# erturklab/delivr_cfos

Hardware: AMD Instinct MI355X
Metric: voxels/sec sliding-window 3D U-Net inference, 2048x2048x1024 vol @1/2/4/8 GPU (higher is better)
Workload: dtype f16; 1 GPU; c3: 1024x2048x2048 (Z,Y,X) uint16 synthetic brain, windows 128x128x128, overlap 0.5, 1 pass (no TTA), trained-like BasicUNet(32,32,64,128,256,32) weights, fp16 operands / fp32 accumulate, ellipsoid brain (background skipped); tta=False, windows=14415, windows_skipped=5400, lanes=3, mask_voxels=16658615, mask_checksum=17887483292235547, parallelism=1 GPU

## Files before the change

### delivr_cfos_amd/_lib.py

```python
from __future__ import annotations

import ctypes as C
import os

_HERE = os.path.dirname(os.path.abspath(__file__))
LIB_PATH = os.path.join(_HERE, "lib", "libdelivr_hip.so")
if os.environ.get("DLV_LIB"):
    _name = os.environ["DLV_LIB"]
    if os.path.basename(_name) != _name or not (_name.startswith("libdelivr_hip") and _name.endswith(".so")):
        raise ImportError(f"DLV_LIB={_name!r}: expected the bare name of a libdelivr_hip*.so under {os.path.dirname(LIB_PATH)}")
    if "_abl" in _name and os.environ.get("DLV_ALLOW_WRONG_RESULTS") != "1":
        raise ImportError(f"DLV_LIB={_name!r} is a timing-only ablation build (wrong results); set DLV_ALLOW_WRONG_RESULTS=1 "
                          "to time it (profiles/tools/zreg_abl.sh does)")
    LIB_PATH = os.path.join(os.path.dirname(LIB_PATH), _name)



def build_fingerprint(lib_path: str | None = None) -> dict:
    import glob
    import hashlib

    lib_path = lib_path or LIB_PATH
    out = {"lib": os.path.basename(lib_path), "lib_sha256": None, "src_sha256": None}
    if os.path.isfile(lib_path):
        h = hashlib.sha256()
        with open(lib_path, "rb") as f:
            for blk in iter(lambda: f.read(1 << 20), b""):
                h.update(blk)
        out["lib_sha256"] = h.hexdigest()
    csrc = os.path.join(_HERE, "csrc")
    files = sorted(glob.glob(os.path.join(csrc, "*.hip")) + glob.glob(os.path.join(csrc, "*.h")) + [os.path.join(csrc, "Makefile")]
                   + glob.glob(os.path.join(os.path.dirname(_HERE), "include", "*.h")))
    h = hashlib.sha256()
    for fn in files:
        if os.path.isfile(fn):
            h.update(os.path.basename(fn).encode() + b"\0")
            with open(fn, "rb") as f:
                h.update(f.read())
    out["src_sha256"] = h.hexdigest()
    return out


DLV_OK, DLV_EINVAL, DLV_EHIP, DLV_ENOMEM, DLV_ESTATE, DLV_EUNSUP, DLV_ERANGE = 0, -1, -2, -3, -4, -5, -6
ABI_VERSION = 2
PREC_F32, PREC_BF16, PREC_F16, PREC_BF16_ALL = 0, 1, 2, 3
N_CONV, N_DECONV = 18, 4
PROF_MAX = 64


class DelivrHipError(RuntimeError):
    def __init__(self, code: int, msg: str):
        super().__init__(f"libdelivr_hip error {code}: {msg}")
        self.code = code


class UnetWeights(C.Structure):
    _fields_ = [
        ("features", C.c_int * 6),
        ("conv_w", C.c_void_p * N_CONV),
        ("conv_b", C.c_void_p * N_CONV),
        ("norm_g", C.c_void_p * N_CONV),
        ("norm_b", C.c_void_p * N_CONV),
        ("deconv_w", C.c_void_p * N_DECONV),
        ("deconv_b", C.c_void_p * N_DECONV),
        ("final_w", C.c_void_p),
        ("final_b", C.c_void_p),
    ]


class DebugLayerArgs(C.Structure):
    _fields_ = [
        ("kind", C.c_int), ("op", C.c_int), ("index", C.c_int),
        ("in1", C.c_void_p), ("c1", C.c_int), ("ss1", C.c_void_p),
        ("in2", C.c_void_p), ("c2", C.c_int),
        ("vol", C.c_void_p), ("flip_dim", C.c_int),
        ("out", C.c_void_p),
        ("B", C.c_int), ("D", C.c_int), ("H", C.c_int), ("W", C.c_int),
        ("ran_zreg", C.c_int), ("ran_upconv", C.c_int), ("ran_stem", C.c_int), ("drops_bias", C.c_int),
        ("drops_fold_const", C.c_int), ("raw_scale", C.c_float),
    ]


PLAN_MAX_LABELS = 96
PLAN_CONV_KERNELS = ("ZREG", "DEEP", "ZMARCH", "GENERIC", "STEM_MFMA", "STEM_VALU")
PLAN_DECONV_KERNELS = ("DEEP", "REGW", "WST", "ROWS", "PARITY")


class PlanConv(C.Structure):
    _fields_ = [("kernel", C.c_int), ("level", C.c_int), ("cin", C.c_int), ("cout", C.c_int), ("folded", C.c_int),
                ("tile_rows", C.c_int), ("act_on_load", C.c_int), ("tx", C.c_int), ("ncb", C.c_int), ("wlds", C.c_int),
                ("max_parts", C.c_longlong)]


class PlanDeconv(C.Structure):
    _fields_ = [("kernel", C.c_int), ("norm_first", C.c_int), ("padded", C.c_int)]


class PlanPool(C.Structure):
    _fields_ = [("rows", C.c_int), ("writeback", C.c_int), ("norm_after", C.c_int), ("nt", C.c_int)]


class LayerPlan(C.Structure):
    _fields_ = [("conv", PlanConv * N_CONV), ("deconv", PlanDeconv * N_DECONV), ("pool", PlanPool * 4), ("n_labels", C.c_int),
                ("labels", (C.c_char * 48) * PLAN_MAX_LABELS), ("flops", C.c_double * PLAN_MAX_LABELS),
                ("bytes", C.c_double * PLAN_MAX_LABELS)]


class SwParams(C.Structure):
    _fields_ = [
        ("Zp", C.c_int), ("Yp", C.c_int), ("Xp", C.c_int),
        ("roi", C.c_int * 3),
        ("overlap", C.c_float),
        ("flip_dim", C.c_int),
        ("skip_threshold", C.c_int),
        ("precision", C.c_int),
        ("sw_batch", C.c_int),
        ("win_begin", C.c_int64),
        ("win_end", C.c_int64),
        ("z0", C.c_int), ("nz", C.c_int),
        ("repeat", C.c_int),
        ("blend_mode", C.c_int),
        ("sigma_scale", C.c_float),
        ("wsum_dev", C.c_void_p),
    ]


class SwStats(C.Structure):
    _fields_ = [("n_windows", C.c_int64), ("n_skipped", C.c_int64), ("n_forward_launches", C.c_int64)]


MAX_RANKS = 16


class ShardPlanC(C.Structure):
    _fields_ = [("world", C.c_int), ("n_windows", C.c_int64),
                ("win_begin", C.c_int64 * MAX_RANKS), ("win_end", C.c_int64 * MAX_RANKS),
                ("z_comp_lo", C.c_int * MAX_RANKS), ("z_comp_hi", C.c_int * MAX_RANKS),
                ("z_own_lo", C.c_int * MAX_RANKS), ("z_own_hi", C.c_int * MAX_RANKS)]


class ProfEntry(C.Structure):
    _fields_ = [("name", C.c_char * 48), ("launches", C.c_int64), ("total_ms", C.c_double),
                ("flops", C.c_double), ("bytes", C.c_double)]


_P = C.c_void_p
SIGNATURES = {
    "dlv_abi_version": (C.c_int, []),
    "dlv_ctx_create": (C.c_int, [C.c_int, _P, C.POINTER(_P)]),
    "dlv_ctx_destroy": (C.c_int, [_P]),
    "dlv_last_error": (C.c_char_p, [_P]),
    "dlv_sync": (C.c_int, [_P]),
    "dlv_stream": (_P, [_P]),
    "dlv_malloc": (C.c_int, [_P, C.c_size_t, C.POINTER(_P)]),
    "dlv_free": (C.c_int, [_P, _P]),
    "dlv_memset_dev": (C.c_int, [_P, _P, C.c_int, C.c_size_t]),
    "dlv_copy_h2d": (C.c_int, [_P, _P, _P, C.c_size_t]),
    "dlv_copy_d2h": (C.c_int, [_P, _P, _P, C.c_size_t]),
    "dlv_unet_load": (C.c_int, [_P, C.POINTER(UnetWeights)]),
    "dlv_unet_blob_size": (C.c_int, [_P, C.POINTER(C.c_size_t)]),
    "dlv_unet_blob_dev": (C.c_int, [_P, C.POINTER(_P)]),
    "dlv_unet_alloc_blob": (C.c_int, [_P, C.POINTER(C.c_int)]),
    "dlv_unet_forward_dev": (C.c_int, [_P, _P, _P, C.c_int, C.c_int, C.c_int, C.c_int, C.c_int]),
    "dlv_sw_num_windows": (C.c_int, [C.POINTER(SwParams), C.POINTER(C.c_int64)]),
    "dlv_sw_window_starts": (C.c_int, [C.POINTER(SwParams), C.POINTER(C.c_int64), C.c_int64]),
    "dlv_sw_window_max_dev": (C.c_int, [_P, C.POINTER(SwParams), _P, C.POINTER(C.c_int32), C.c_int64]),
    "dlv_sw_infer_dev": (C.c_int, [_P, C.POINTER(SwParams), _P, _P, _P, C.POINTER(SwStats)]),
    "dlv_shard_plan_make": (C.c_int, [C.POINTER(SwParams), C.c_int, C.POINTER(C.c_float), C.POINTER(ShardPlanC)]),
    "dlv_shard_slab": (C.c_int, [C.POINTER(ShardPlanC), C.c_int, C.c_int, C.c_int, C.c_int, C.POINTER(C.c_int), C.POINTER(C.c_int)]),
    "dlv_comm_init_all": (C.c_int, [C.c_int, C.POINTER(C.c_int), C.POINTER(_P)]),
    "dlv_comm_destroy": (C.c_int, [_P]),
    "dlv_comm_size": (C.c_int, [_P]),
    "dlv_comm_uses_rccl": (C.c_int, [_P]),
    "dlv_comm_selftest": (C.c_int, [_P, C.c_size_t]),
    "dlv_comm_ctx": (_P, [_P, C.c_int]),
    "dlv_comm_last_error": (C.c_char_p, [_P]),
    "dlv_bcast_weights": (C.c_int, [_P, C.c_int]),
    "dlv_sw_infer_sharded": (C.c_int, [_P, C.POINTER(SwParams), C.POINTER(ShardPlanC), C.POINTER(C.c_int), C.POINTER(C.c_int),
                                       C.POINTER(_P), C.POINTER(_P), C.POINTER(_P), C.POINTER(SwStats)]),
    "dlv_sw_infer_sharded_wsum": (C.c_int, [_P, C.POINTER(SwParams), C.POINTER(ShardPlanC), C.POINTER(C.c_int), C.POINTER(C.c_int),
                                            C.POINTER(_P), C.POINTER(_P), C.POINTER(_P), C.POINTER(_P), C.POINTER(SwStats)]),
    "dlv_finalize_slab_dev": (C.c_int, [_P, _P, _P, _P, C.c_int, C.c_int, C.c_int, C.c_int, C.c_int, C.c_int, C.c_float, C.c_int,
                                        C.c_int, _P, _P]),
    "dlv_finalize_dev": (C.c_int, [_P, _P, _P, _P, C.c_int, C.c_int, C.c_int, C.c_int, C.c_int, C.c_float, C.c_int,
                                   C.c_int, _P, _P]),
    "dlv_ccl26_dev": (C.c_int, [_P, _P, C.c_int, C.c_int, C.c_int, _P, C.POINTER(C.c_uint64)]),
    "dlv_cc_stats_dev": (C.c_int, [_P, _P, C.c_int, C.c_int, C.c_int, C.c_uint64, _P, _P, _P]),
    "dlv_block_mean_u16_dev": (C.c_int, [_P, _P, C.c_int, C.c_int, C.c_int, C.c_int, C.c_int, C.c_int, _P]),
    "dlv_zoom_spline2_u8_dev": (C.c_int, [_P, _P, C.c_int, C.c_int, C.c_int, _P, C.c_int, C.c_int, C.c_int]),
    "dlv_mask_pad_u16_dev": (C.c_int, [_P, _P, _P, C.c_int, C.c_int, C.c_int, C.c_int, _P, C.c_int, C.c_int, C.c_int]),
    "dlv_trilinear_u16_dev": (C.c_int, [_P, _P, C.c_int, C.c_int, C.c_int, _P, C.c_int, C.c_int, C.c_int]),
    "dlv_affine_warp_u16_dev": (C.c_int, [_P, _P, C.c_int, C.c_int, C.c_int, C.POINTER(C.c_double), _P, C.c_int, C.c_int, C.c_int]),
    "dlv_seam_pairs_dev": (C.c_int, [_P, _P, _P, C.c_int, C.c_int, _P, C.c_uint64, C.POINTER(C.c_uint64)]),
    "dlv_relabel_u32_dev": (C.c_int, [_P, _P, C.c_uint64, _P, C.c_uint64]),
    "dlv_cc_stats_raw_dev": (C.c_int, [_P, _P, C.c_int, C.c_int, C.c_int, C.c_uint64, _P, _P, _P, _P]),
    "dlv_cc_counts_dev": (C.c_int, [_P, _P, C.c_uint64, C.c_uint64, _P]),
    "dlv_cc_size_filter_dev": (C.c_int, [_P, _P, C.c_uint64, C.c_uint64, _P, C.c_int64, C.c_int64, C.POINTER(C.c_uint64)]),
    "dlv_cc_intensity_dev": (C.c_int, [_P, _P, _P, C.c_int, C.c_int, C.c_int, C.c_int64, C.c_int64, C.c_uint64, _P, _P, _P, _P]),
    "dlv_cc_shell_dev": (C.c_int, [_P, _P, _P, C.c_int, C.c_int, C.c_int, C.c_int64, C.c_int64, C.c_int, _P, _P]),
    "dlv_paint_owner_dev": (C.c_int, [_P, _P, C.c_int, C.c_int, C.c_int, _P, _P, C.c_uint64, _P]),
    "dlv_paint_apply_dev": (C.c_int, [_P, _P, _P, C.c_uint64, _P, C.c_int, _P]),
    "dlv_edt_u16_dev": (C.c_int, [_P, _P, C.c_int, C.c_int, C.c_int, C.POINTER(C.c_double), _P]),
    "dlv_heatmap_counts_dev": (C.c_int, [_P, _P, C.c_uint64, C.c_int, C.c_int, C.c_int, _P]),
    "dlv_gauss_blur_f32_dev": (C.c_int, [_P, _P, C.c_int, C.c_int, C.c_int, _P, C.c_int, _P]),
    "dlv_tiff_last_error": (C.c_char_p, []),
    "dlv_tiff_plane_size": (C.c_int, [C.c_char_p, C.POINTER(C.c_int), C.POINTER(C.c_int), C.POINTER(C.c_int)]),
    "dlv_tiff_read_plane_u16": (C.c_int, [C.c_char_p, _P, C.c_int, C.c_int]),
    "dlv_tiff_write_plane": (C.c_int, [C.c_char_p, _P, C.c_int, C.c_int, C.c_int, C.c_int]),
    "dlv_tiff_stack_to_device": (C.c_int, [_P, C.POINTER(C.c_char_p), C.c_int, C.c_int, C.c_int, _P, C.c_longlong,
                                            C.c_longlong, C.c_int]),
    "dlv_diag_set": (C.c_int, [_P, C.c_char_p, C.c_int]),
    "dlv_diag_plan": (C.c_int, [C.POINTER(C.c_int), C.POINTER(C.c_char_p), C.POINTER(C.c_int), C.c_int, C.c_int, C.c_int, C.c_int,
                                C.c_int, C.c_int, C.POINTER(LayerPlan)]),
    "dlv_cells_csv": (C.c_int, [_P, _P, C.c_uint64, _P, C.c_size_t, C.POINTER(C.c_size_t)]),
    "dlv_reserve_dev": (C.c_int, [_P, _P, C.c_int, C.c_int, C.c_int]),
    "dlv_debug_stamps": (C.c_int, [_P, _P]),
    "dlv_debug_set_zm_variant": (C.c_int, [_P, C.c_int]),
    "dlv_debug_set_format": (C.c_int, [_P, C.c_int]),
    "dlv_debug_layer_bf16": (C.c_int, [_P, C.c_int, C.c_int, _P, C.c_int, _P, C.c_int, _P, C.c_int, C.c_int, C.c_int,
                                       C.c_int]),
    "dlv_debug_layer16": (C.c_int, [_P, C.POINTER(DebugLayerArgs)]),
    "dlv_unet_set_conv_shift": (C.c_int, [_P, C.c_int, C.c_int]),
    "dlv_unet_get_conv_shift": (C.c_int, [_P, C.c_int, C.POINTER(C.c_int)]),
    "dlv_unet_note_conv_shifts": (C.c_int, [_P, C.POINTER(C.c_int)]),
    "dlv_range_report": (C.c_int, [_P, C.POINTER(C.c_int), C.POINTER(C.c_float)]),
    "dlv_range_next_shifts": (C.c_int, [C.c_int, C.POINTER(C.c_float), C.POINTER(C.c_int), C.POINTER(C.c_int)]),
    "dlv_range_recover": (C.c_int, [_P, C.POINTER(C.c_int)]),
    "dlv_comm_range_recover": (C.c_int, [_P, C.POINTER(C.c_int)]),
    "dlv_set_lanes": (C.c_int, [_P, C.c_int]),
    "dlv_prof_enable": (C.c_int, [_P, C.c_int]),
    "dlv_prof_reset": (C.c_int, [_P]),
    "dlv_prof_report": (C.c_int, [_P, C.POINTER(ProfEntry), C.c_int, C.POINTER(C.c_int)]),
}

_lib = None


def load() -> C.CDLL:
    global _lib
    if _lib is not None:
        return _lib
    if not os.path.isfile(LIB_PATH):
        raise ImportError(
            f"{LIB_PATH} not found - build it with `python -c 'import __graft_entry__ as g; g.build()'` "
            "or `make -C delivr_cfos_amd/csrc` (hipcc, --offload-arch=gfx950). There is no CPU fallback.")
    try:
        import torch
    except ImportError:
        pass
    lib = C.CDLL(LIB_PATH)
    for name, (res, args) in SIGNATURES.items():
        fn = getattr(lib, name)
        fn.restype = res
        fn.argtypes = args
    if lib.dlv_abi_version() != ABI_VERSION:
        raise ImportError(f"libdelivr_hip.so reports ABI version {lib.dlv_abi_version()}, this package binds version {ABI_VERSION} "
                          "(include/delivr_hip.h: DLV_ABI_VERSION): rebuild with make -C delivr_cfos_amd/csrc")
    _lib = lib
    return lib
```

### delivr_cfos_amd/csrc/api.hip

```cpp
#include <dlfcn.h>

#include <algorithm>
#include <charconv>
#include <cmath>
#include <cstdlib>
#include <mutex>

#include "common.h"

int dlv_fail(dlv_ctx* ctx, int code, const char* fmt, ...) {
    char buf[1024];
    va_list ap;
    va_start(ap, fmt);
    vsnprintf(buf, sizeof(buf), fmt, ap);
    va_end(ap);
    if (ctx) ctx->err = buf;
    return code;
}

int dlv_ws_get(dlv_ctx* ctx, int slot, size_t bytes, void** out) {
    if (slot < 0 || slot >= WS_N_SLOTS) return dlv_fail(ctx, DLV_EINVAL, "bad scratch slot %d", slot);
    if (ctx->ws_bytes[slot] < bytes) {
        if (ctx->ws[slot]) {
            DLV_TRY(dlv_sync_all(ctx));
// ... 559 lines not shown
    if (std::isnan(v)) return p + snprintf(p, (size_t)(end - p), "nan");
    if (std::isinf(v)) return p + snprintf(p, (size_t)(end - p), v < 0 ? "-inf" : "inf");
    const double a = std::fabs(v);
    if (a != 0.0 && (a < 1e-4 || a >= 1e16)) {
        const auto r = std::to_chars(p, end, v, std::chars_format::scientific);
        return r.ptr;
    }
    const auto r = std::to_chars(p, end, v, std::chars_format::fixed);
    char* q = r.ptr;
    bool dot = false;
    for (char* c = p; c < q; ++c) dot |= (*c == '.');
    if (!dot && q + 2 <= end) {
        *q++ = '.';
        *q++ = '0';
    }
    return q;
}

int dlv_cells_csv(const uint32_t* voxel_counts, const double* centroids, uint64_t n, char* out, size_t cap, size_t* len_out) {
    if (!voxel_counts || !centroids || !out || !len_out) return DLV_EINVAL;
    static const char header[] = ",Blob,Coords,Size\n";
    if (cap < sizeof(header)) return DLV_EINVAL;
    char* p = out;
    char* const end = out + cap;
    memcpy(p, header, sizeof(header) - 1);
    p += sizeof(header) - 1;
    for (uint64_t i = 1; i < n; ++i) {
        if ((size_t)(end - p) < 128) return DLV_EINVAL;
        p += snprintf(p, (size_t)(end - p), "0,%llu,\"[", (unsigned long long)i);
        for (int k = 0; k < 3; ++k) {
            p = py_float_repr(p, end, centroids[3 * i + k]);
            if (k < 2) {
                *p++ = ',';
                *p++ = ' ';
            }
        }
        p += snprintf(p, (size_t)(end - p), "]\",%u\n", voxel_counts[i]);
    }
    *len_out = (size_t)(p - out);
    return DLV_OK;
}

int dlv_diag_set(dlv_ctx* ctx, const char* name, int value) {
    if (!ctx || !name) return DLV_EINVAL;
    const std::string n(name);
    if (n == "zm_variant") return dlv_debug_set_zm_variant(ctx, value);
    if (dlv_plan_switch_set(ctx->sw, name, value)) return DLV_OK;
    if (n == "upconv_simple") ctx->upconv_simple = value ? 1 : 0;
    else if (n == "zreg_dbg") ctx->zreg_dbg = value;
    else if (n == "erode_xy_split") ctx->erode_xy_split = value != 0;
    else if (n == "erode_z_two_sweeps") ctx->erode_z_two_sweeps = value != 0;
    else if (n == "ccl_simple") ctx->ccl_simple = value != 0;
    else if (n == "resample_simple") ctx->resample_simple = value != 0;
    else if (n == "resample_run16") ctx->resample_run16 = value != 0;
    else if (n == "tiff_chunk") ctx->tiff_chunk = value > 0 ? value : 0;
    else return dlv_fail(ctx, DLV_EINVAL, "dlv_diag_set: unknown switch '%s'", name);
    return DLV_OK;
}

int dlv_debug_set_zm_variant(dlv_ctx* ctx, int variant) {
    if (!ctx) return DLV_EINVAL;
#ifndef DLV_DIAG
    if (variant != 0 && variant != 50 && variant != 51)
        return dlv_fail(ctx, DLV_EUNSUP, "z-march variant %d is a diagnostic build: load libdelivr_hip_diag.so (make -C delivr_cfos_amd/csrc diag)", variant);
#endif
    ctx->sw.zm_variant = variant;
    return DLV_OK;
}

int dlv_diag_plan(const int features[6], const char* const* names, const int* values, int n, int fmt16, int B, int d, int h, int w,
                  dlv_layer_plan* out) {
    if (!features || !out || n < 0 || (n > 0 && (!names || !values)) || fmt16 < 0 || fmt16 > 2) return DLV_EINVAL;
    DlvPlanSwitches sw;
    bool upconv_simple = false;
    for (int i = 0; i < n; ++i) {
        if (!names[i]) return DLV_EINVAL;
        if (strcmp(names[i], "upconv_simple") == 0) upconv_simple = values[i] != 0;
        else if (strcmp(names[i], "zreg_dbg") == 0) continue;
        else if (!dlv_plan_switch_set(sw, names[i], values[i])) return DLV_EINVAL;
    }
    return dlv_plan_forward(sw, upconv_simple, features, fmt16, B, d, h, w, out) ? DLV_OK : DLV_EUNSUP;
}

int dlv_debug_stamps(dlv_ctx* ctx, void* buf_dev) {
    if (!ctx) return DLV_EINVAL;
    ctx->stamp_buf = buf_dev;
    return DLV_OK;
}

int dlv_debug_set_format(dlv_ctx* ctx, int precision) {
    if (!ctx || (precision != DLV_PREC_BF16_ALL && precision != DLV_PREC_F16)) return DLV_EINVAL;
    ctx->debug_f16 = precision == DLV_PREC_F16;
    return DLV_OK;
}

int dlv_set_lanes(dlv_ctx* ctx, int lanes) {
    if (!ctx || lanes < 1 || lanes > DLV_MAX_LANES) return DLV_EINVAL;
    ctx->lanes_wanted = lanes;
    return DLV_OK;
}

int dlv_prof_enable(dlv_ctx* ctx, int on) {
    if (!ctx) return DLV_EINVAL;
    if (!on) DLV_TRY(prof_drain(ctx));
    ctx->prof_on = on != 0;
    return DLV_OK;
}
int dlv_prof_reset(dlv_ctx* ctx) {
    if (!ctx) return DLV_EINVAL;
    DLV_TRY(prof_drain(ctx));
    ctx->prof_slots.clear();
    return DLV_OK;
}
int dlv_prof_report(dlv_ctx* ctx, dlv_prof_entry* entries, int capacity, int* n_out) {
    if (!ctx || !n_out) return DLV_EINVAL;
    DLV_TRY(prof_drain(ctx));
    int n = (int)ctx->prof_slots.size();
    *n_out = n;
    for (int i = 0; i < n && i < capacity && entries; ++i) {
        memcpy(entries[i].name, ctx->prof_slots[i].name, sizeof(entries[i].name));
        entries[i].launches = ctx->prof_slots[i].launches;
        entries[i].total_ms = ctx->prof_slots[i].total_ms;
        entries[i].flops = ctx->prof_slots[i].flops;
        entries[i].bytes = ctx->prof_slots[i].bytes;
    }
    return DLV_OK;
}

}
```

### delivr_cfos_amd/csrc/common.h

```cpp
#pragma once
#include <hip/hip_runtime.h>

#include <atomic>
#include <cstdarg>
#include <cstdint>
#include <cstdio>
#include <cstring>
#include <string>
#include <vector>

#include "../../include/delivr_hip.h"
#include "../../include/delivr_hip_diag.h"
#include "layer_plan.h"

#define DLV_WAVE 64
#define DLV_MAX_LANES 6

struct DlvProfSlot {
    char name[48];
    int64_t launches = 0;
    double total_ms = 0.0, flops = 0.0, bytes = 0.0;
};
struct DlvProfPending {
    int slot;
    hipEvent_t a, b;
};

struct DlvConvLayer {
    int cin = 0, cout = 0;
    float* w_f32 = nullptr;
    float* bias = nullptr;
    float* bias16 = nullptr;
    int shift = 0;
    float* gamma = nullptr;
    float* beta = nullptr;
    uint16_t* w_bf16 = nullptr;
    uint16_t* w_f16 = nullptr;
    uint16_t* w16_bf16 = nullptr;
    uint16_t* w16_f16 = nullptr;
    uint16_t* wskip_bf16 = nullptr;
    uint16_t* wskip_f16 = nullptr;
    uint16_t* wup_bf16 = nullptr;
    uint16_t* wup_f16 = nullptr;
    float* up_corr = nullptr;
    int up_slices = 0;
};
struct DlvDeconvLayer {
    int cin = 0, cout = 0;
    float* w_f32 = nullptr;
    float* bias = nullptr;
    uint16_t* w_bf16 = nullptr;
    uint16_t* w_f16 = nullptr;
    uint16_t* w16_bf16 = nullptr;
    uint16_t* w16_f16 = nullptr;
};

enum DlvWsSlot {
    WS_F32_ACT = 0,
    WS_BF16_ACT,
    WS_STATS,
    WS_TILE_IN,
    WS_TILE_OUT,
    WS_TILE_META,
    WS_BLEND_W,
    WS_ERODE,
    WS_CCL,
    WS_MISC,
    WS_LANE_ACT0,
    WS_LANE_STATS0 = WS_LANE_ACT0 + DLV_MAX_LANES - 1,
    WS_N_SLOTS = WS_LANE_STATS0 + DLV_MAX_LANES - 1
};

struct dlv_ctx {
    int device = 0;
    hipStream_t stream = nullptr;
    hipStream_t main_stream = nullptr;
    hipStream_t aux_stream = nullptr;
    hipStream_t aux[DLV_MAX_LANES - 1] = {nullptr};
    hipEvent_t ev_lane[DLV_MAX_LANES + 1] = {nullptr};
    int lane = 0;
    int lanes_wanted = 3;
    bool own_stream = false;
    std::string err;
    bool weights_loaded = false;
    int features[6] = {0, 0, 0, 0, 0, 0};
    const float* blend_w = nullptr;
    float blend_min = 0.f;
    float* blend_wsum = nullptr;
    int upconv_dbg = 0;
    int upconv_simple = 0;
    void* stamp_buf = nullptr;
    int* range_flag = nullptr;
    int range_last = -1;
    float range_peak[DLV_N_CONV] = {0};
    bool range_seq = false;
    int range_base[DLV_N_CONV] = {0};
    int range_blind_layer = -1;
    void* zero_page = nullptr;
    void* blob = nullptr;
    size_t blob_bytes = 0;
    DlvConvLayer conv[DLV_N_CONV];
    DlvDeconvLayer deconv[DLV_N_DECONV];
    float* final_w = nullptr;
    float* final_b = nullptr;
    void* ws[WS_N_SLOTS] = {nullptr};
    size_t ws_bytes[WS_N_SLOTS] = {0};
    bool debug_f16 = false;
    DlvPlanSwitches sw;
    int zreg_dbg = 0;
    int ran_zreg = 0, ran_upconv = 0;
    bool erode_xy_split = false, erode_z_two_sweeps = false, ccl_simple = false;
    bool resample_simple = false, resample_run16 = false;
    int tiff_chunk = 0;
    bool prof_on = false;
    std::vector<DlvProfSlot> prof_slots;
    std::vector<DlvProfPending> prof_pending;
    std::vector<hipEvent_t> prof_free;
};

int dlv_fail(dlv_ctx* ctx, int code, const char* fmt, ...);

#define DLV_HIP(ctx, expr)                                                                          \
    do {                                                                                            \
        hipError_t _e = (expr);                                                                     \
        if (_e != hipSuccess)                                                                       \
            return dlv_fail((ctx), _e == hipErrorOutOfMemory ? DLV_ENOMEM : DLV_EHIP, "%s failed: %s (%s:%d)", \
                            #expr, hipGetErrorString(_e), __FILE__, __LINE__);                      \
    } while (0)

#define DLV_LAUNCH_CHECK(ctx, what)                                                                 \
    do {                                                                                            \
        hipError_t _e = hipGetLastError();                                                          \
        if (_e != hipSuccess)                                                                       \
            return dlv_fail((ctx), DLV_EHIP, "launch of %s failed: %s", (what), hipGetErrorString(_e)); \
    } while (0)

#define DLV_TRY(expr)                \
    do {                             \
        int _rc = (expr);            \
        if (_rc != DLV_OK) return _rc; \
    } while (0)

int dlv_ws_get(dlv_ctx* ctx, int slot, size_t bytes, void** out);
int dlv_sync_all(dlv_ctx* ctx);

struct DlvProf {
    dlv_ctx* ctx;
    int idx = -1;
    bool ranged = false;
    DlvProf(dlv_ctx* c, const char* name, double flops, double bytes);
    ~DlvProf();
    void end();
};

typedef std::atomic<unsigned long long> dlv_attr_bits;
static inline bool dlv_attr_is_set(const dlv_attr_bits& bits, int device) { return (bits.load(std::memory_order_acquire) >> (device & 63)) & 1ull; }
static inline void dlv_attr_mark(dlv_attr_bits& bits, int device) { bits.fetch_or(1ull << (device & 63), std::memory_order_release); }

#ifdef __HIPCC__
#ifndef DLV_NT
#define DLV_NT 1
#endif
typedef unsigned dlv_u32x4_t __attribute__((ext_vector_type(4)));
typedef unsigned dlv_u32x2_t __attribute__((ext_vector_type(2)));
template <bool NT>
__device__ __forceinline__ uint4 dlv_ld16(const uint4* p) {
    if constexpr (NT && DLV_NT) {
        const dlv_u32x4_t t = __builtin_nontemporal_load(reinterpret_cast<const dlv_u32x4_t*>(p));
        return make_uint4(t.x, t.y, t.z, t.w);
    } else {
        return *p;
    }
}
template <bool NT>
__device__ __forceinline__ void dlv_st16(uint4* p, uint4 v) {
    if constexpr (NT && DLV_NT) __builtin_nontemporal_store(dlv_u32x4_t{v.x, v.y, v.z, v.w}, reinterpret_cast<dlv_u32x4_t*>(p));
    else *p = v;
}
template <bool NT>
__device__ __forceinline__ void dlv_st8(uint2* p, uint2 v) {
    if constexpr (NT && DLV_NT) __builtin_nontemporal_store(dlv_u32x2_t{v.x, v.y}, reinterpret_cast<dlv_u32x2_t*>(p));
    else *p = v;
}
__device__ __forceinline__ int dlv_xcd_tile(unsigned bx, unsigned gx) {
    return (gx % 8 == 0) ? (int)((bx % 8) * (gx / 8) + bx / 8) : (int)bx;
}
#endif

int dlv_unet_forward_f32(dlv_ctx* ctx, const float* x, float* logits, int B, int d, int h, int w);
static inline int dlv_fmt16(int precision) { return precision == DLV_PREC_F16 ? 1 : (precision == DLV_PREC_BF16 ? 2 : 0); }
int dlv_unet_forward_bf16(dlv_ctx* ctx, const float* x, float* logits, int B, int d, int h, int w, int fmt16);
int dlv_unet_tiles_bf16(dlv_ctx* ctx, const uint16_t* vol, int Yp, int Xp, const int* starts_dev, int B, int d,
                        int h, int w, int flip_dim, float scale, float* acc, int fmt16);
int dlv_pack_weights_bf16(dlv_ctx* ctx);
int dlv_unet_reserve_16(dlv_ctx* ctx, int B, int d, int h, int w, int lanes);
int dlv_conv3_zmarch_launch(dlv_ctx* ctx, bool f16, int cin, int cout, const void* in1, int c1, const void* in2, int c2,
                            const void* wpk, const float* bias, void* out, float* partials, int B, int D, int H, int W,
                            int* nparts);
int dlv_conv3_deep_launch(dlv_ctx* ctx, bool f16, int cin, int cout, const void* in1, int c1, const void* in2, int c2, const void* wpk16,
                          void* out, float* partials, int B, int D, int H, int W, int* nparts);
int dlv_pack_deconv_w16(dlv_ctx* ctx, bool f16, const float* w_f32, uint16_t* out, int cin, int cout);
int dlv_deconv2_deep_launch(dlv_ctx* ctx, bool f16, int cin, int cout, const void* in, const void* wpk16, const float* bias, void* out, int B,
                            int D, int H, int W);
int dlv_conv3_zreg_launch(dlv_ctx* ctx, bool f16, int cin, int cout, const void* in1, int c1, const void* ss1, const void* in2,
                          int c2, const void* ss2, const void* wpk16, void* out, float* partials, int B, int D, int H, int W,
                          int* nparts, const void* addend = nullptr);
int dlv_pack_conv_w16(dlv_ctx* ctx, bool f16, const float* w_f32, uint16_t* out, int cout, int cin, int ctot = 0, int c0 = 0, float wscale = 1.f);
int dlv_pack_upconv(dlv_ctx* ctx, bool f16, const float* wc, int ctot, int cs, const float* wd, const float* bd, uint16_t* wpk, float* corr,
                    int ci0 = 0, int with_corr = 1, float wscale = 1.f);
bool dlv_upconv2_persistent(const dlv_ctx* ctx, int Dc, int Hc, int Wc);
int dlv_upconv2_launch(dlv_ctx* ctx, bool f16, const void* in, const void* wpk, const float* corr, void* out, int B, int Dc, int Hc, int Wc,
                       int cstride = 4, int c0 = 0);
int dlv_range_reset(dlv_ctx* ctx);
int dlv_range_check(dlv_ctx* ctx, int fmt16);
int dlv_unet_apply_conv_shifts(dlv_ctx* ctx, const int* shifts);
int dlv_range_step(dlv_ctx* ctx, int layer, const float* peaks, int* n_changed, const int* force_next );
int dlv_range_plan(dlv_ctx* ctx, int layer, const float* peaks, int* nxt, bool* blind);
size_t dlv_bf16_pack_bytes(const int features[6]);
#if defined(__HIPCC__)
__device__ __forceinline__ float dlv_half_sum32(float v) {
#define DLV_DPP_ADD(ctrl, rmask)                                                                                      \
    v += __builtin_bit_cast(float, __builtin_amdgcn_update_dpp(0, __builtin_bit_cast(int, v), ctrl, rmask, 0xf, true))
    DLV_DPP_ADD(0xB1, 0xf);
    DLV_DPP_ADD(0x4E, 0xf);
    DLV_DPP_ADD(0x141, 0xf);
    DLV_DPP_ADD(0x140, 0xf);
    DLV_DPP_ADD(0x142, 0xa);
#undef DLV_DPP_ADD
    return v;
}
#endif
```

### delivr_cfos_amd/csrc/layer_plan.h

```cpp
#pragma once
#include <cstdio>
#include <cstring>

#include "../../include/delivr_hip_diag.h"

struct DlvPlanSwitches {
    bool no_zmarch = false;
    int zm_variant = 0;
    int zreg_mask = 3;
    int deep_mask = 2;
    int deep_small = 1;
    int generic_ncb = 0;
    int fuse_layers = 1 << 17;
    int fuse_levels = 0;
    int fold_up = 1;
    bool pool_rows_off = false;
};

inline bool dlv_plan_switch_set(DlvPlanSwitches& s, const char* name, int value) {
    const auto is = [&](const char* n) { return strcmp(name, n) == 0; };
    if (is("no_zmarch")) s.no_zmarch = value != 0;
    else if (is("no_upconv")) s.fold_up = value ? 0 : 1;
    else if (is("zm_variant")) s.zm_variant = value;
    else if (is("fuse_levels")) s.fuse_levels = value;
    else if (is("fuse_layers")) s.fuse_layers = value;
    else if (is("zreg_mask")) s.zreg_mask = value;
    else if (is("deep_mask")) s.deep_mask = value;
    else if (is("generic_ncb")) s.generic_ncb = value;
    else if (is("deep_small")) s.deep_small = value;
    else if (is("pool_rows_off")) s.pool_rows_off = value != 0;
    else return false;
    return true;
}

static inline int dlv_cdiv(long long a, long long b) { return (int)((a + b - 1) / b); }

constexpr int kDlvConvLevel[DLV_N_CONV] = {0, 0, 1, 1, 2, 2, 3, 3, 4, 4, 3, 3, 2, 2, 1, 1, 0, 0};

inline void dlv_unet_channels(const int f[6], int cin[DLV_N_CONV], int cout[DLV_N_CONV], int dcin[DLV_N_DECONV], int dcout[DLV_N_DECONV]) {
    const int ci[DLV_N_CONV] = {1, f[0], f[0], f[1], f[1], f[2], f[2], f[3], f[3], f[4],
                                f[3] + f[4] / 2, f[3], f[2] + f[3] / 2, f[2], f[1] + f[2] / 2, f[1], f[0] + f[1], f[5]};
    const int co[DLV_N_CONV] = {f[0], f[0], f[1], f[1], f[2], f[2], f[3], f[3], f[4], f[4],
                                f[3], f[3], f[2], f[2], f[1], f[1], f[5], f[5]};
    const int di[DLV_N_DECONV] = {f[4], f[3], f[2], f[1]};
    const int dco[DLV_N_DECONV] = {f[4] / 2, f[3] / 2, f[2] / 2, f[1]};
    for (int i = 0; i < DLV_N_CONV; ++i) {
        cin[i] = ci[i];
        cout[i] = co[i];
    }
    for (int j = 0; j < DLV_N_DECONV; ++j) {
        dcin[j] = di[j];
        dcout[j] = dco[j];
    }
}
inline bool dlv_window_supported(int d, int h, int w) {
    return d >= 16 && h >= 16 && w >= 16 && (long long)(d >> 4) * (h >> 4) * (w >> 4) >= 2;
}

inline bool dlv_conv_has_fold_pack(int li, int cin, int cout, int dcin3, int dcout3) {
    return li == 16 && cin == 64 && cout == 32 && dcin3 == 32 && dcout3 == 32;
}
inline bool dlv_deconv_has_w16_pack(int cin) { return cin >= 128; }

inline bool dlv_conv3_zreg_supports(int cin, int cout, int c1, int c2, int W) {
    return cout % 32 == 0 && cout > 0 && W >= 32 &&
           ((cin == 32 && c1 == 32 && c2 == 0) || (cin == 64 && ((c1 == 32 && c2 == 32) || (c1 == 64 && c2 == 0))));
}
inline int dlv_conv3_zreg_tile_rows(int cin, int cout, int D, int H, int W) {
    return (cin == 32 && H % 16 == 0 && (long long)(H / 16) * dlv_cdiv(W, 32) * (cout / 32) * dlv_cdiv(D, 64) >= 16) ? 16 : 8;
}
inline bool dlv_conv3_deep_supports(int cin, int cout, int c1, int c2, int D, int H, int W) {
    return cin % 32 == 0 && c1 % 32 == 0 && c2 % 32 == 0 && c1 + c2 == cin && cout % 32 == 0 && cout >= 32 && W >= 2 && H >= 2 && D >= 2 &&
           (long long)D * H * W <= 32768;
}
inline bool dlv_deconv2_deep_supports(int cin, int cout, int D, int H, int W) {
    return (cin == 128 || cin == 256) && cout % 64 == 0 && cout > 0 && (long long)D * H * W <= 32768 && W >= 1;
}
inline bool dlv_upconv2_persistent_shape(int Dc, int Hc, int Wc) {
    return Dc > 0 && Dc % 4 == 0 && Hc % 8 == 0 && Wc % 16 == 0 && ((long long)5 * Hc + 10) * Wc * 16 < (1 << 24) &&
           (long long)Dc * Hc * Wc * 8 * 16 * 2 < (1LL << 31);
}

struct DlvConvPlan {
    int kernel = DLV_PLAN_GENERIC;
    int cin = 0, cout = 0;
    bool folded = false;
    int tile_rows = 0;
    int tx = 0, ncb = 0;
    bool wlds = false;
    bool act_on_load = false;
    bool norm_first = false;
    long long max_parts = 0;
};

inline bool dlv_plan_zreg_runs(const DlvPlanSwitches& sw, int cin, int cout, int c1, int c2, int D, int H, int W) {
    return (sw.zm_variant == 0 || sw.zm_variant == 50) && !sw.no_zmarch && (long long)D * H * W > 32768 &&
           dlv_conv3_zreg_supports(cin, cout, c1, c2, W) && ((cin == 32 ? 1 : 2) & sw.zreg_mask);
}
inline bool dlv_plan_fuses_first_input(const DlvPlanSwitches& sw, int li, int cin, int cout, int c1, int c2, int D, int H, int W) {
    return (((sw.fuse_levels >> kDlvConvLevel[li]) & 1) || ((sw.fuse_layers >> li) & 1)) && c1 == 32 &&
           dlv_plan_zreg_runs(sw, cin, cout, c1, c2, D, H, W);
}

inline DlvConvPlan plan_conv(const DlvPlanSwitches& sw, int li, int cin, int cout, int c1, int c2, bool raw1, int B, int D, int H, int W) {
    DlvConvPlan p;
    p.cin = cin;
    p.cout = cout;
    p.act_on_load = raw1 && dlv_plan_fuses_first_input(sw, li, cin, cout, c1, c2, D, H, W);
    p.norm_first = raw1 && !p.act_on_load;
    const long long zm_parts = (long long)dlv_cdiv(H, 8) * dlv_cdiv(W, 32) * dlv_cdiv(D, 16);
    if (dlv_plan_zreg_runs(sw, cin, cout, c1, c2, D, H, W)) {
        p.kernel = DLV_PLAN_ZREG;
        p.tile_rows = dlv_conv3_zreg_tile_rows(cin, cout, D, H, W);
        p.max_parts = zm_parts;
        return p;
    }
    const bool zmarch_ok = (cout == 32 || cout == 64) && (cin == 32 || cin == 64) && W >= 32;
    const bool deep_full = cout >= 64 && W >= 8 && H >= 8 && D >= 4;
    if (!sw.no_zmarch && ((zmarch_ok ? 1 : 2) & sw.deep_mask) && (deep_full || sw.deep_small) && dlv_conv3_deep_supports(cin, cout, c1, c2, D, H, W)) {
        p.kernel = DLV_PLAN_DEEP;
        p.max_parts = (long long)dlv_cdiv(D, 4) * dlv_cdiv(H, 8) * dlv_cdiv(W, 8);
        return p;
    }
    if (zmarch_ok && !sw.no_zmarch) {
        p.kernel = DLV_PLAN_ZMARCH;
        p.max_parts = zm_parts;
        return p;
    }
    p.kernel = DLV_PLAN_GENERIC;
    p.tx = W >= 16 ? 16 : 8;
    const long long ntiles = (long long)dlv_cdiv(D, 4) * dlv_cdiv(H, 64 / p.tx) * dlv_cdiv(W, p.tx);
    p.wlds = (long long)D * H * W <= 1024;
    p.ncb = p.wlds ? (cout >= 64 ? 2 : 1) : (cout >= 128 ? 4 : (cout >= 64 ? 2 : 1));
    while (p.ncb > 1 && (long long)B * ntiles * (cout / (32 * p.ncb)) < 512) p.ncb >>= 1;
    if (const int want = sw.generic_ncb)
        if ((want == 1 || want == 2 || (want == 4 && !p.wlds)) && cout % (32 * want) == 0) p.ncb = want;
    p.max_parts = ntiles;
    return p;
}

inline bool plan_folds_up(const DlvPlanSwitches& sw, bool has_pack, int cskip, int cout, int D, int H, int W) {
    return sw.fold_up && has_pack && cskip == 32 && (sw.zm_variant == 0 || sw.zm_variant == 50) && !sw.no_zmarch && (long long)D * H * W > 32768 &&
           dlv_conv3_zreg_supports(32, cout, 32, 0, W) && D % 2 == 0 && H % 2 == 0 && W % 2 == 0;
}
inline DlvConvPlan plan_conv_folded(const DlvPlanSwitches& sw, int li, int cout, bool raw1, int D, int H, int W) {
    DlvConvPlan p;
    p.kernel = DLV_PLAN_ZREG;
    p.folded = true;
    p.cin = 32;
    p.cout = cout;
    p.tile_rows = dlv_conv3_zreg_tile_rows(32, cout, D, H, W);
    p.act_on_load = raw1 && dlv_plan_fuses_first_input(sw, li, 64, cout, 32, 32, D, H, W);
    p.norm_first = raw1 && !p.act_on_load;
    p.max_parts = (long long)dlv_cdiv(H, 8) * dlv_cdiv(W, 32) * dlv_cdiv(D, 16);
    return p;
}

struct DlvDeconvPlan {
    int kernel = DLV_PLAN_DC_PARITY;
    bool norm_first = false;
};
constexpr int DLV_DC_IPW = 8;

inline DlvDeconvPlan plan_deconv(const DlvPlanSwitches& sw, int cin, int cout, bool raw, int D, int H, int W) {
    DlvDeconvPlan p;
    const bool rows = !sw.no_zmarch;
    p.norm_first = raw && (!rows || cin >= 128);
    const long long segs = dlv_cdiv(W, 16), vox = (long long)D * H * W;
    if (rows && sw.deep_mask != 0 && dlv_deconv_has_w16_pack(cin) && dlv_deconv2_deep_supports(cin, cout, D, H, W)) p.kernel = DLV_PLAN_DC_DEEP;
    else if (cin != 32 && cin != 64 && cin != 128 && cin != 256) p.kernel = DLV_PLAN_NONE;
    else if (!rows) p.kernel = DLV_PLAN_DC_PARITY;
    else if (cin >= 128) p.kernel = DLV_PLAN_DC_WST;
    else if (cout == 32 && (long long)D * H * segs >= 4 * DLV_DC_IPW * 64 && vox * 8 * 4 * 16 < (1ll << 32)) p.kernel = DLV_PLAN_DC_REGW;
    else p.kernel = DLV_PLAN_DC_ROWS;
    return p;
}

struct DlvNormPlan {
    bool rows = false;
    bool nt = false;
};
inline DlvNormPlan plan_norm_pass(const DlvPlanSwitches& sw, bool pooled, int B, int C, int D, int H, int W) {
    DlvNormPlan p;
    p.nt = (double)D * H * W * B * C * 2 > 768.0 * (1 << 20);
    p.rows = pooled && W % 64 == 0 && !sw.pool_rows_off;
    return p;
}
inline bool plan_stem_mfma(const DlvPlanSwitches& sw, bool from_volume) { return from_volume && !sw.no_zmarch; }

struct DlvLabel {
    char name[48];
    double flops, bytes;
};
inline const char* dlv_fmt_name(bool f16) { return f16 ? "f16" : "bf16"; }

inline DlvLabel dlv_label_conv(const DlvConvPlan& p, bool f16, int B, int D, int H, int W) {
    static const char* const family[4] = {"zreg", "deep", "zmarch", "mfma"};
    DlvLabel l;
    const double vox = (double)((long long)D * H * W);
    snprintf(l.name, sizeof(l.name), "conv3_%s_%s_c%dx%d_d%d%s%s", family[p.kernel], dlv_fmt_name(f16), p.cin, p.cout, D, p.folded ? "_add" : "",
             p.act_on_load ? "_act" : "");
    l.flops = 2.0 * 27 * p.cin * p.cout * vox * B;
    l.bytes = 2.0 * vox * B * (p.cin + (p.folded ? 2 : 1) * p.cout);
    if (p.kernel == DLV_PLAN_DEEP) l.bytes += 2.0 * 27 * p.cin * p.cout;
    return l;
}
inline DlvLabel dlv_label_upconv(bool persistent, bool f16, int B, int D, int H, int W) {
    DlvLabel l;
    const double vox = (double)((long long)D * H * W), voxc = (double)((long long)(D / 2) * (H / 2) * (W / 2));
    snprintf(l.name, sizeof(l.name), "upconv2%s_%s_c32x32_d%d", persistent ? "m" : "", dlv_fmt_name(f16), D / 2);
    l.flops = 2.0 * 8 * 32 * 32 * vox * B;
    l.bytes = 2.0 * 32 * (voxc + vox) * B;
    return l;
}
inline DlvLabel dlv_label_deconv(const DlvDeconvPlan& p, bool f16, int cin, int cout, int B, int D, int H, int W) {
    DlvLabel l;
    const double vox = (double)((long long)D * H * W);
    snprintf(l.name, sizeof(l.name), "deconv2_%s_%s_c%dx%d_d%d", p.kernel == DLV_PLAN_DC_DEEP ? "deep" : "mfma", dlv_fmt_name(f16), cin, cout, D);
    l.flops = 2.0 * 8 * cin * cout * vox * B;
    l.bytes = 2.0 * vox * B * (cin + 8.0 * cout);
    return l;
}
inline DlvLabel dlv_label_norm(bool pooled, bool writeback, bool f16, bool seam, int B, int C, int D, int H, int W) {
    DlvLabel l;
    const double vox = (double)((long long)D * H * W);
    snprintf(l.name, sizeof(l.name), "%s", pooled ? (writeback ? (f16 ? (seam ? "norm_mish_pool_f16_to_bf16" : "norm_mish_pool_f16") : "norm_mish_pool_bf16")
                                                               : (f16 ? "pool_act_f16" : "pool_act_bf16"))
                                                  : (f16 ? "norm_mish_f16" : (seam ? "norm_mish_bf16_to_f16" : "norm_mish_bf16")));
    l.flops = 0.0;
    l.bytes = vox * B * C * 2 * (writeback ? 2 : 1) + (pooled ? vox / 8 * B * C * 2 : 0.0);
    return l;
}
inline DlvLabel dlv_label_pad(bool f16, int cout, int B, long long vox_up, long long vox_skip) {
    DlvLabel l;
    snprintf(l.name, sizeof(l.name), "%s", f16 ? "replicate_pad_f16" : "replicate_pad_bf16");
    l.flops = 0.0;
    l.bytes = 16.0 * B * (cout / 8) * ((double)vox_up + (double)vox_skip);
    return l;
}
inline DlvLabel dlv_label_stem(bool mfma, int B, int D, int H, int W) {
    DlvLabel l;
    const double vox = (double)((long long)D * H * W);
    snprintf(l.name, sizeof(l.name), "%s", mfma ? "stem_mfma_u16" : "stem_conv_f32");
    l.flops = 2.0 * 27 * 32 * vox * B;
    l.bytes = vox * B * (2 + 64);
    return l;
}
inline DlvLabel dlv_label_final(bool blend, int B, int D, int H, int W) {
    DlvLabel l;
    const double vox = (double)((long long)D * H * W);
    snprintf(l.name, sizeof(l.name), "%s", blend ? "final_conv_blend" : "final_conv_logits");
    l.flops = 2.0 * 32 * vox * B;
    l.bytes = vox * B * (64 + (blend ? 8 : 4));
    return l;
}

inline bool dlv_plan_forward(const DlvPlanSwitches& sw, bool upconv_simple, const int f[6], int fmt16, int B, int d, int h, int w, dlv_layer_plan* out) {
    memset(out, 0, sizeof(*out));
    if (f[0] != 32 || f[5] != 32 || B < 1 || !dlv_window_supported(d, h, w)) return false;
    for (int i = 0; i < 6; ++i)
        if (f[i] <= 0 || f[i] % 32 || f[i] > 256) return false;
    int cin[DLV_N_CONV], cout[DLV_N_CONV], dcin[DLV_N_DECONV], dcout[DLV_N_DECONV];
    dlv_unet_channels(f, cin, cout, dcin, dcout);
    struct Dm {
        int D, H, W;
        long long vox() const { return (long long)D * H * W; }
    } dm[5];
    for (int l = 0; l < 5; ++l) dm[l] = Dm{d >> l, h >> l, w >> l};
    const bool mixed = fmt16 == 2;
    const auto f16_at = [&](int level) { return level == 0 ? fmt16 != 0 : fmt16 == 1; };
    const auto emit = [&](const DlvLabel& l) {
        if (out->n_labels >= DLV_PLAN_MAX_LABELS) return;
        memcpy(out->labels[out->n_labels], l.name, sizeof(l.name));
        out->flops[out->n_labels] = l.flops;
        out->bytes[out->n_labels] = l.bytes;
        ++out->n_labels;
    };
    struct T {
        int C;
        bool raw;
    };
    const auto materialise = [&](T& t, int level, int fl, bool seam) {
        if (!t.raw) return;
        emit(dlv_label_norm(false, true, f16_at(fl), seam, B, t.C, dm[level].D, dm[level].H, dm[level].W));
        t.raw = false;
    };
    const auto record = [&](int li, const DlvConvPlan& p, int level) {
        dlv_plan_conv& c = out->conv[li];
        c.kernel = p.kernel;
        c.level = level;
        c.cin = p.cin;
        c.cout = p.cout;
        c.folded = p.folded;
        c.tile_rows = p.tile_rows;
        c.act_on_load = p.act_on_load;
        c.tx = p.tx;
        c.ncb = p.ncb;
        c.wlds = p.wlds;
        c.max_parts = p.max_parts;
        emit(dlv_label_conv(p, f16_at(level), B, dm[level].D, dm[level].H, dm[level].W));
    };
    const auto conv = [&](int li, T& a1, int c2, int level) {
        const DlvConvPlan p = plan_conv(sw, li, cin[li], cout[li], a1.C, c2, a1.raw, B, dm[level].D, dm[level].H, dm[level].W);
        if (p.norm_first) materialise(a1, level, level, false);
        record(li, p, level);
        return T{cout[li], true};
    };
    const auto deconv_to = [&](int j, T& a, int l, int fl) {
        const Dm din = dm[l + 1], sk = dm[l];
        const DlvDeconvPlan p = plan_deconv(sw, dcin[j], dcout[j], a.raw, din.D, din.H, din.W);
        if (p.norm_first) materialise(a, l + 1, fl, false);
        out->deconv[j].kernel = p.kernel;
        out->deconv[j].norm_first = p.norm_first;
        emit(dlv_label_deconv(p, f16_at(fl), dcin[j], dcout[j], B, din.D, din.H, din.W));
        out->deconv[j].padded = 2 * din.D != sk.D || 2 * din.H != sk.H || 2 * din.W != sk.W;
        if (out->deconv[j].padded) emit(dlv_label_pad(f16_at(fl), dcout[j], B, 8 * din.vox(), sk.vox()));
    };

    const bool stem_mfma = plan_stem_mfma(sw, true);
    out->conv[0].kernel = stem_mfma ? DLV_PLAN_STEM_MFMA : DLV_PLAN_STEM_VALU;
    out->conv[0].cin = 1;
    out->conv[0].cout = 32;
    emit(dlv_label_stem(stem_mfma, B, d, h, w));
    T x0{32, !stem_mfma};
    T skip[5];
    skip[0] = conv(1, x0, 0, 0);
    for (int l = 1; l <= 4; ++l) {
        T& up = skip[l - 1];
        const int li_cat = 18 - 2 * l, c_up = dcout[4 - l];
        const Dm dp = dm[l - 1];
        const bool keep_raw = plan_conv(sw, li_cat, cin[li_cat], cout[li_cat], up.C, c_up, true, B, dp.D, dp.H, dp.W).act_on_load;
        const bool odd = ((dp.D | dp.H | dp.W) & 1) != 0;
        const DlvNormPlan np = plan_norm_pass(sw, true, B, up.C, dp.D, dp.H, dp.W);
        dlv_plan_pool& pl = out->pool[l - 1];
        pl.rows = np.rows;
        pl.nt = np.nt;
        pl.writeback = !keep_raw && !odd;
        pl.norm_after = odd && !keep_raw;
        emit(dlv_label_norm(true, pl.writeback, f16_at(l - 1), l == 1 && mixed, B, up.C, dp.D, dp.H, dp.W));
        if (pl.norm_after) emit(dlv_label_norm(false, true, f16_at(l - 1), false, B, up.C, dp.D, dp.H, dp.W));
        up.raw = keep_raw;
        T a{l == 1 ? 32 : f[l - 1], false};
        T b = conv(2 * l, a, 0, l);
        skip[l] = conv(2 * l + 1, b, 0, l);
    }
    T cur = skip[4];
    for (int j = 0; j < 4; ++j) {
        const int l = 3 - j, li = 10 + 2 * j;
        T b;
        if (l == 0 && mixed) materialise(cur, 1, 1, true);
        if (l == 0 && plan_folds_up(sw, dlv_conv_has_fold_pack(li, cin[li], cout[li], dcin[3], dcout[3]), skip[0].C, cout[li], d, h, w)) {
            const DlvConvPlan p = plan_conv_folded(sw, li, cout[li], skip[0].raw, d, h, w);
            materialise(cur, 1, 0, false);
            if (p.norm_first) materialise(skip[0], 0, 0, false);
            emit(dlv_label_upconv(!upconv_simple && dlv_upconv2_persistent_shape(dm[1].D, dm[1].H, dm[1].W), f16_at(0), B, d, h, w));
            record(li, p, 0);
            out->deconv[j].kernel = DLV_PLAN_NONE;
            b = T{cout[li], true};
        } else {
            deconv_to(j, cur, l, l);
            b = conv(li, skip[l], dcout[j], l);
        }
        cur = conv(li + 1, b, 0, l);
    }
    emit(dlv_label_final(true, B, d, h, w));
    return true;
}
```

### delivr_cfos_amd/csrc/sw_infer.hip

```cpp
#include <algorithm>

#include "common.h"
#include <cmath>

namespace {

struct Tiler {
    int n[3], roi[3], iv[3];
    std::vector<int> st[3];
    int ncol[3];
    std::vector<int> col[3];
    int64_t count() const { return (int64_t)st[0].size() * st[1].size() * st[2].size(); }
};

int build_tiler(dlv_ctx* ctx, const dlv_sw_params* p, Tiler& t) {
    t.n[0] = p->Zp;
    t.n[1] = p->Yp;
    t.n[2] = p->Xp;
    if (!(p->overlap >= 0.f && p->overlap < 1.f)) return dlv_fail(ctx, DLV_EINVAL, "overlap must be >= 0 and < 1");
    for (int k = 0; k < 3; ++k) {
        if (t.n[k] <= 0) return dlv_fail(ctx, DLV_EINVAL, "empty volume");
        int r = p->roi[k] > 0 ? p->roi[k] : t.n[k];
        if (r > t.n[k])
            return dlv_fail(ctx, DLV_EUNSUP, "roi[%d]=%d exceeds the padded volume (%d): pad the volume first "
                            "(downsample_and_mask.py:390-396 does)", k, r, t.n[k]);
        t.roi[k] = r;
        int iv = r == t.n[k] ? r : (int)((double)r * (1.0 - (double)p->overlap));
        if (iv <= 0) iv = 1;
        t.iv[k] = iv;
        const int num = (t.n[k] + iv - 1) / iv;
        int scan = num - 1;
        for (int dd = 0; dd < num; ++dd)
            if ((long long)dd * iv + r >= t.n[k]) {
                scan = dd;
                break;
            }
        t.st[k].clear();
        for (int i = 0; i <= scan; ++i) {
            int s = i * iv;
            s -= std::max(s + r - t.n[k], 0);
            t.st[k].push_back(s);
        }
        const int c = (r + iv - 1) / iv;
        const int kk = (int)t.st[k].size();
        t.col[k].assign(kk, 0);
        int ncol = std::min(c, kk);
        for (int i = 0; i < kk; ++i) t.col[k][i] = i % c;
        if (kk > 1 && t.st[k][kk - 1] != (kk - 1) * iv && kk > c) {
            t.col[k][kk - 1] = c;
            ncol = c + 1;
        }
        t.ncol[k] = ncol;
    }
    return DLV_OK;
}


__global__ void __launch_bounds__(256) window_max_kernel(const uint16_t* __restrict__ vol, int Yp, int Xp,
                                                         const int* __restrict__ starts, int d, int h, int w,
                                                         int* __restrict__ wmax) {
    const int win = blockIdx.y;
    const int z0 = starts[3 * win], y0 = starts[3 * win + 1], x0 = starts[3 * win + 2];
    const uint16_t* base = vol + ((long long)z0 * Yp + y0) * Xp + x0;
    unsigned m = 0;
    const bool vec = (w % 8 == 0) && (Xp % 8 == 0) && (x0 % 8 == 0);
    if (vec) {
        const int w8 = w / 8;
        const long long n8 = (long long)d * h * w8;
        for (long long i = (long long)blockIdx.x * blockDim.x + threadIdx.x; i < n8; i += (long long)gridDim.x * blockDim.x) {
            const int xx = (int)(i % w8), yy = (int)((i / w8) % h), zz = (int)(i / ((long long)w8 * h));
            const uint4 v = *reinterpret_cast<const uint4*>(base + ((long long)zz * Yp + yy) * Xp + xx * 8);
            const unsigned a = max(max(v.x & 0xffffu, v.x >> 16), max(v.y & 0xffffu, v.y >> 16));
            const unsigned b = max(max(v.z & 0xffffu, v.z >> 16), max(v.w & 0xffffu, v.w >> 16));
            m = max(m, max(a, b));
        }
    } else {
        const long long n = (long long)d * h * w;
        for (long long i = (long long)blockIdx.x * blockDim.x + threadIdx.x; i < n; i += (long long)gridDim.x * blockDim.x) {
            const int xx = (int)(i % w), yy = (int)((i / w) % h), zz = (int)(i / ((long long)w * h));
            m = max(m, (unsigned)base[((long long)zz * Yp + yy) * Xp + xx]);
        }
    }
    for (int o = 32; o > 0; o >>= 1) m = max(m, __shfl_down(m, o, 64));
    if ((threadIdx.x & 63) == 0 && m > 0) atomicMax(wmax + win, (int)m);
}

__global__ void __launch_bounds__(256) cell_max_kernel(const uint16_t* __restrict__ vol, int Yp, int Xp, int z_lo,
                                                       const int* __restrict__ zcell, const int* __restrict__ ybound, int ncy,
                                                       const int* __restrict__ xcell, int x_lo8, int x_hi8, int ncx,
                                                       int* __restrict__ cellmax) {
    extern __shared__ int lmax[];
    const int cy = blockIdx.x % ncy, z = z_lo + blockIdx.x / ncy;
    const int cz = zcell[z];
    if (cz < 0) return;
    for (int i = threadIdx.x; i < ncx; i += blockDim.x) lmax[i] = 0;
    __syncthreads();
    const int y0 = ybound[cy], y1 = ybound[cy + 1];
    for (int c = x_lo8 + threadIdx.x; c < x_hi8; c += blockDim.x) {
        unsigned m = 0;
        const uint16_t* col = vol + ((long long)z * Yp + y0) * Xp + 8 * c;
        for (int y = y0; y < y1; ++y, col += Xp) {
            const uint4 v = *reinterpret_cast<const uint4*>(col);
            const unsigned a = max(max(v.x & 0xffffu, v.x >> 16), max(v.y & 0xffffu, v.y >> 16));
            const unsigned b = max(max(v.z & 0xffffu, v.z >> 16), max(v.w & 0xffffu, v.w >> 16));
            m = max(m, max(a, b));
        }
        if (m) atomicMax(&lmax[xcell[c]], (int)m);
    }
    __syncthreads();
    for (int i = threadIdx.x; i < ncx; i += blockDim.x)
        if (lmax[i]) atomicMax(&cellmax[((long long)cz * ncy + cy) * ncx + i], lmax[i]);
// ... 150 lines not shown
        pr.end();
    }
    DLV_LAUNCH_CHECK(ctx, "window_max_kernel");
    DLV_HIP(ctx, hipMemcpyAsync(wmax, meta + n * 3, (size_t)n * sizeof(int), hipMemcpyDeviceToHost, ctx->stream));
    DLV_HIP(ctx, hipStreamSynchronize(ctx->stream));
    return DLV_OK;
}

extern "C" {

int dlv_sw_num_windows(const dlv_sw_params* p, int64_t* n_windows) {
    if (!p || !n_windows) return DLV_EINVAL;
    Tiler t;
    DLV_TRY(build_tiler(nullptr, p, t));
    *n_windows = t.count();
    return DLV_OK;
}

int dlv_sw_window_starts(const dlv_sw_params* p, int64_t* starts, int64_t capacity) {
    if (!p || !starts) return DLV_EINVAL;
    Tiler t;
    DLV_TRY(build_tiler(nullptr, p, t));
    if (capacity < t.count()) return DLV_EINVAL;
    int64_t i = 0;
    for (int z : t.st[0])
        for (int y : t.st[1])
            for (int x : t.st[2]) {
                starts[3 * i] = z;
                starts[3 * i + 1] = y;
                starts[3 * i + 2] = x;
                ++i;
            }
    return DLV_OK;
}

int dlv_sw_window_max_dev(dlv_ctx* ctx, const dlv_sw_params* p, const uint16_t* vol_dev, int32_t* wmax, int64_t capacity) {
    if (!ctx || !p || !vol_dev || !wmax) return DLV_EINVAL;
    DLV_HIP(ctx, hipSetDevice(ctx->device));
    Tiler t;
    DLV_TRY(build_tiler(ctx, p, t));
    const int64_t total = t.count();
    const int64_t wb = std::max<int64_t>(p->win_begin, 0);
    const int64_t we = p->win_end > 0 ? std::min<int64_t>(p->win_end, total) : total;
    const int64_t n = std::max<int64_t>(we - wb, 0);
    if (capacity < n) return dlv_fail(ctx, DLV_EINVAL, "wmax capacity %lld < %lld windows", (long long)capacity, (long long)n);
    if (n == 0) return DLV_OK;
    if (n > (int64_t)1 << 30) return dlv_fail(ctx, DLV_EUNSUP, "too many windows");
    const int z0 = p->nz > 0 ? p->z0 : 0, nz = p->nz > 0 ? p->nz : p->Zp;
    const int ny = (int)t.st[1].size(), nx = (int)t.st[2].size();
    std::vector<int> starts((size_t)n * 3);
    for (int64_t g = wb; g < we; ++g) {
        const int iz = (int)(g / ((int64_t)ny * nx)), iy = (int)((g / nx) % ny), ix = (int)(g % nx);
        const int z = t.st[0][iz];
        if (z < z0 || z + t.roi[0] > z0 + nz) return dlv_fail(ctx, DLV_EINVAL, "window %lld outside the slab", (long long)g);
        const int64_t i = g - wb;
        starts[3 * i] = z - z0;
        starts[3 * i + 1] = t.st[1][iy];
        starts[3 * i + 2] = t.st[2][ix];
    }
    return window_maxima(ctx, vol_dev, p->Yp, p->Xp, t.roi, starts, n, wmax);
}

static int default_sw_batch(long long tile_vox) {
    return (int)std::min<long long>(std::max<long long>(((long long)1 << 25) / tile_vox, 1), 64);
}

int dlv_reserve_dev(dlv_ctx* ctx, const dlv_sw_params* p, int Z, int Y, int X) {
    if (!ctx || !p) return DLV_EINVAL;
    if (p->roi[0] <= 0 || p->roi[1] <= 0 || p->roi[2] <= 0) return dlv_fail(ctx, DLV_EINVAL, "dlv_reserve_dev: window dimensions");
    DLV_HIP(ctx, hipSetDevice(ctx->device));
    const long long tile_vox = (long long)p->roi[0] * p->roi[1] * p->roi[2];
    const int B = p->sw_batch > 0 ? p->sw_batch : default_sw_batch(tile_vox);
    if (p->precision != DLV_PREC_F32) {
        const int lanes = ctx->aux[0] != nullptr ? std::max(1, std::min(ctx->lanes_wanted, DLV_MAX_LANES)) : 1;
        DLV_TRY(dlv_unet_reserve_16(ctx, B, p->roi[0], p->roi[1], p->roi[2], lanes));
    }
    if (Z > 0 && Y > 0 && X > 0) {
        void* q;
        DLV_TRY(dlv_ws_get(ctx, WS_ERODE, (size_t)Z * Y * X, &q));
    }
    return DLV_OK;
}

int dlv_sw_infer_dev(dlv_ctx* ctx, const dlv_sw_params* p, const uint16_t* vol_dev, float* acc_dev, uint8_t* cnt_dev,
                     dlv_sw_stats* stats) {
    if (!ctx || !p || !vol_dev || !acc_dev) return DLV_EINVAL;
    if (!ctx->weights_loaded) return dlv_fail(ctx, DLV_ESTATE, "dlv_sw_infer_dev before dlv_unet_load");
    if (p->precision != DLV_PREC_F32 && p->precision != DLV_PREC_BF16 && p->precision != DLV_PREC_F16 && p->precision != DLV_PREC_BF16_ALL)
        return dlv_fail(ctx, DLV_EINVAL, "unknown precision %d", p->precision);
    if (!(p->flip_dim == -1 || (p->flip_dim >= 2 && p->flip_dim <= 4)))
        return dlv_fail(ctx, DLV_EINVAL, "flip_dim must be -1, 2, 3 or 4");
    DLV_HIP(ctx, hipSetDevice(ctx->device));
    Tiler t;
    DLV_TRY(build_tiler(ctx, p, t));
    const int d = t.roi[0], h = t.roi[1], w = t.roi[2];
    if (!dlv_window_supported(d, h, w))
        return dlv_fail(ctx, DLV_EUNSUP, "window %dx%dx%d: every dimension must be at least 16 and level 4 (each dimension / 16, rounded down) must hold more "
                        "than one voxel - InstanceNorm3d has no statistics of a single value and torch raises there; any size from there on: "
                        "levels with an odd size are pooled and padded like MONAI's MaxPool3d / UpCat", d, h, w);
    const int64_t total = t.count();
    const int64_t wb = std::max<int64_t>(p->win_begin, 0);
    const int64_t we = p->win_end > 0 ? std::min<int64_t>(p->win_end, total) : total;
    const int z0 = p->nz > 0 ? p->z0 : 0;
    const int nz = p->nz > 0 ? p->nz : p->Zp;
    const int Yp = p->Yp, Xp = p->Xp;
    const int rep = p->repeat > 0 ? p->repeat : 1;
    ctx->blend_w = nullptr;
    ctx->blend_wsum = nullptr;
    ctx->blend_min = 0.f;
    if (p->blend_mode == DLV_BLEND_GAUSSIAN) {
        if (cnt_dev) return dlv_fail(ctx, DLV_EINVAL, "Gaussian blend: pass wsum_dev (fp32) instead of the uint8 count map");
        const float ss = p->sigma_scale > 0.f ? p->sigma_scale : 0.125f;
        std::vector<float> g((size_t)d + h + w);
        float gmin = 1.f;
        size_t off = 0;
        for (int k = 0; k < 3; ++k) {
            const int len = t.roi[k], center = len / 2;
            const float sigma = (float)len * ss;
            const int tail = (int)(std::max(sigma * 4.0f, 0.5f) + 0.5f);
            const float tt = 0.70710678f / std::fabs(sigma);
            float mx = 0.f, mn = 0.f;
            for (int i = 0; i < len; ++i) {
                const int x = i - center;
                float v = 0.f;
                if (x >= -tail && x <= tail) v = std::max(0.f, 0.5f * (std::erf(tt * ((float)x + 0.5f)) - std::erf(tt * ((float)x - 0.5f))));
                g[off + i] = v;
                mx = std::max(mx, v);
            }
            for (int i = 0; i < len; ++i) {
                g[off + i] /= mx;
                if (g[off + i] > 0.f && (mn == 0.f || g[off + i] < mn)) mn = g[off + i];
            }
            gmin *= mn;
            off += len;
        }
        float* gw;
        DLV_TRY(dlv_ws_get(ctx, WS_BLEND_W, g.size() * sizeof(float), (void**)&gw));
        DLV_HIP(ctx, hipMemcpyAsync(gw, g.data(), g.size() * sizeof(float), hipMemcpyHostToDevice, ctx->stream));
        DLV_HIP(ctx, hipStreamSynchronize(ctx->stream));
        ctx->blend_w = gw;
        ctx->blend_min = gmin;
        ctx->blend_wsum = p->wsum_dev;
    } else if (p->blend_mode != DLV_BLEND_CONSTANT) {
        return dlv_fail(ctx, DLV_EINVAL, "unknown blend_mode %d", p->blend_mode);
    }
    if (cnt_dev) {
        long long mult = 1;
        for (int k = 0; k < 3; ++k) {
            std::vector<int> cov((size_t)t.n[k] + 1, 0);
            for (int st : t.st[k]) {
                cov[st] += 1;
                cov[st + t.roi[k]] -= 1;
            }
            int run = 0, mx = 0;
            for (int i = 0; i < t.n[k]; ++i) {
                run += cov[i];
                mx = std::max(mx, run);
            }
            mult *= mx;
        }
        if (mult * rep > 255)
            return dlv_fail(ctx, DLV_EUNSUP, "uint8 count map would wrap: up to %lld windows cover a voxel, x repeat %d > 255", mult, rep);
    }
    if (stats) {
        stats->n_windows = std::max<int64_t>(we - wb, 0);
        stats->n_skipped = 0;
        stats->n_forward_launches = 0;
    }
    if (we <= wb) return DLV_OK;
    const int64_t nwin = we - wb;
    if (nwin > (int64_t)1 << 30) return dlv_fail(ctx, DLV_EUNSUP, "too many windows in one shard");

    const int ny = (int)t.st[1].size(), nx = (int)t.st[2].size();
    const int ncolors = t.ncol[0] * t.ncol[1] * t.ncol[2];
    std::vector<std::vector<int>> by_color(ncolors);
    std::vector<int> starts((size_t)nwin * 3);
    for (int64_t g = wb; g < we; ++g) {
        const int iz = (int)(g / ((int64_t)ny * nx)), iy = (int)((g / nx) % ny), ix = (int)(g % nx);
        const int i = (int)(g - wb);
        const int sz = t.st[0][iz], sy = t.st[1][iy], sx = t.st[2][ix];
        if (sz < z0 || sz + d > z0 + nz)
            return dlv_fail(ctx, DLV_EINVAL, "window %lld (z %d..%d) lies outside the slab [%d,%d)", (long long)g, sz,
                            sz + d, z0, z0 + nz);
        starts[3 * i] = sz - z0;
        starts[3 * i + 1] = sy;
        starts[3 * i + 2] = sx;
        const int c = (t.col[0][iz] * t.ncol[1] + t.col[1][iy]) * t.ncol[2] + t.col[2][ix];
        by_color[c].push_back(i);
    }

    int* meta;
    DLV_TRY(dlv_ws_get(ctx, WS_TILE_META, (size_t)nwin * 3 * sizeof(int), (void**)&meta));
    int* list_dev = meta;
    const long long tile_vox = (long long)d * h * w;
    std::vector<int> wmax((size_t)nwin);
    DLV_TRY(window_maxima(ctx, vol_dev, Yp, Xp, t.roi, starts, nwin, wmax.data()));

    std::vector<int> list;
    list.reserve((size_t)nwin * 3);
    struct Seg { size_t off; int n_active, n_skipped; };
    std::vector<Seg> segs;
    int64_t n_skipped = 0;
    for (int c = 0; c < ncolors; ++c) {
        Seg s{list.size() / 3, 0, 0};
        for (int pass = 0; pass < 2; ++pass)
            for (int i : by_color[c]) {
                const bool skip = wmax[i] <= p->skip_threshold;
                if ((pass == 0) == skip) continue;
                list.push_back(starts[3 * i]);
                list.push_back(starts[3 * i + 1]);
                list.push_back(starts[3 * i + 2]);
                if (skip) ++s.n_skipped; else ++s.n_active;
            }
        n_skipped += s.n_skipped;
        segs.push_back(s);
    }
    DLV_HIP(ctx, hipMemcpyAsync(list_dev, list.data(), list.size() * sizeof(int), hipMemcpyHostToDevice, ctx->stream));

    int sw_batch = p->sw_batch;
    if (sw_batch <= 0) sw_batch = default_sw_batch(tile_vox);
    int64_t launches = 0;
    const int bchunks = (int)std::min<long long>(std::max<long long>(tile_vox / (256 * 16), 1), 256);
    const int nlanes = (p->precision != DLV_PREC_F32 && ctx->aux[0] != nullptr) ? std::max(1, std::min(ctx->lanes_wanted, DLV_MAX_LANES)) : 1;
    const bool two_lanes = nlanes > 1;
    auto lane_stream = [&](int l) { return l == 0 ? ctx->main_stream : ctx->aux[l - 1]; };
    std::vector<hipStream_t> parts;
    for (int l = 0; l < nlanes; ++l) parts.push_back(lane_stream(l));
    auto join_lanes = [&]() -> int {
        if (!two_lanes) return DLV_OK;
        for (size_t l = 0; l < parts.size(); ++l) DLV_HIP(ctx, hipEventRecord(ctx->ev_lane[l], parts[l]));
        for (size_t l = 0; l < parts.size(); ++l)
            for (size_t m = 0; m < parts.size(); ++m)
                if (m != l) DLV_HIP(ctx, hipStreamWaitEvent(parts[l], ctx->ev_lane[m], 0));
        return DLV_OK;
    };
    if (p->precision != DLV_PREC_F32) DLV_TRY(dlv_range_reset(ctx));
    int rc = join_lanes();
    int lane = 0;
    for (const Seg& s : segs) {
        if (rc != DLV_OK) break;
        for (int b0 = 0; b0 < s.n_active && rc == DLV_OK; b0 += sw_batch) {
            const int B = std::min(sw_batch, s.n_active - b0);
            const int* st_dev = list_dev + (s.off + b0) * 3;
            if (p->precision != DLV_PREC_F32) {
                ctx->lane = two_lanes ? lane : 0;
                ctx->stream = lane_stream(ctx->lane);
                rc = dlv_unet_tiles_bf16(ctx, vol_dev, Yp, Xp, st_dev, B, d, h, w, p->flip_dim, (float)rep, acc_dev, dlv_fmt16(p->precision));
                if (rc == DLV_OK && cnt_dev) {
                    hipLaunchKernelGGL(fill_add_kernel, dim3(bchunks, B), dim3(256), 0, ctx->stream, st_dev, d, h, w, Yp,
                                       Xp, 0.0f, rep, acc_dev, cnt_dev, nullptr, 0.f, nullptr);
                    if (hipGetLastError() != hipSuccess) rc = dlv_fail(ctx, DLV_EHIP, "launch of fill_add_kernel(count) failed");
                }
                lane = (lane + 1) % nlanes;
            } else {
                float *tin, *tout;
                rc = dlv_ws_get(ctx, WS_TILE_IN, (size_t)sw_batch * tile_vox * 4, (void**)&tin);
                if (rc == DLV_OK) rc = dlv_ws_get(ctx, WS_TILE_OUT, (size_t)sw_batch * tile_vox * 4, (void**)&tout);
                if (rc != DLV_OK) break;
                hipLaunchKernelGGL(gather_f32_kernel, dim3(bchunks, B), dim3(256), 0, ctx->stream, vol_dev, Yp, Xp,
                                   st_dev, d, h, w, p->flip_dim, tin);
                rc = dlv_unet_forward_f32(ctx, tin, tout, B, d, h, w);
                if (rc != DLV_OK) break;
                hipLaunchKernelGGL(blend_add_kernel, dim3(bchunks, B), dim3(256), 0, ctx->stream, tout, st_dev, d, h, w,
                                   p->flip_dim, Yp, Xp, (float)rep, rep, acc_dev, cnt_dev, ctx->blend_w, ctx->blend_min, ctx->blend_wsum);
                if (hipGetLastError() != hipSuccess) rc = dlv_fail(ctx, DLV_EHIP, "launch of gather/blend kernel failed");
            }
            ++launches;
        }
        ctx->stream = ctx->main_stream;
        ctx->lane = 0;
        if (rc == DLV_OK && s.n_skipped > 0) {
            const int* st_dev = list_dev + (s.off + s.n_active) * 3;
            DlvProf pr(ctx, "skip_fill_f32", 0.0, 8.0 * tile_vox * s.n_skipped);
            hipLaunchKernelGGL(fill_add_kernel, dim3(bchunks, s.n_skipped), dim3(256), 0, ctx->stream, st_dev, d, h, w,
                               Yp, Xp, -1000.0f * rep, rep, acc_dev, cnt_dev, ctx->blend_w, ctx->blend_min, ctx->blend_wsum);
            pr.end();
            if (hipGetLastError() != hipSuccess) rc = dlv_fail(ctx, DLV_EHIP, "launch of fill_add_kernel failed");
        }
        if (rc == DLV_OK) rc = join_lanes();
    }
    ctx->stream = ctx->main_stream;
    ctx->lane = 0;
    if (rc != DLV_OK) return rc;
    if (stats) {
        stats->n_skipped = n_skipped;
        stats->n_forward_launches = launches;
    }
    if (p->precision != DLV_PREC_F32 && launches > 0) return dlv_range_check(ctx, dlv_fmt16(p->precision));
    return DLV_OK;
}

}
```

### delivr_cfos_amd/csrc/unet16_norm.h

```cpp
#pragma once
namespace {

__global__ void __launch_bounds__(64) stats_finalize_kernel(const float* __restrict__ partials, int nparts, int C,
                                                            double inv_count, float eps, const float* __restrict__ gamma,
                                                            const float* __restrict__ beta, float2* __restrict__ ss,
                                                            int* __restrict__ range_flag, int layer) {
    const int c = blockIdx.x % C, n = blockIdx.x / C;
    double s = 0.0, q = 0.0;
    for (int i = threadIdx.x; i < nparts; i += 64) {
        const float2 v = *reinterpret_cast<const float2*>(partials + (((long long)n * nparts + i) * C + c) * 2);
        s += v.x;
        q += v.y;
    }
    for (int o = 32; o > 0; o >>= 1) {
        s += __shfl_down(s, o, 64);
        q += __shfl_down(q, o, 64);
    }
    if (threadIdx.x == 0) {
        if (!(fabs(s) <= 1.0e300 && fabs(q) <= 1.0e300)) atomicMax(range_flag, 100 - layer);
        const double mean = s * inv_count;
        double var = q * inv_count - mean * mean;
        if (var < 0.0) var = 0.0;
        const float peak = (float)(fabs(mean) + 8.0 * sqrt(var));
        if (peak > 0.f && peak < 3.0e38f && __float_as_int(peak) > __builtin_nontemporal_load(range_flag + 1 + layer))
            atomicMax(range_flag + 1 + layer, __float_as_int(peak));
        const float rstd = (float)(1.0 / sqrt(var + (double)eps));
        const float sc = rstd * gamma[c];
        ss[n * C + c] = make_float2(sc, beta[c] - (float)mean * sc);
    }
}

template <class P, class PO = P>
__device__ __forceinline__ uint4 norm_mish8(uint4 u, const float* sc, const float* sh, float* mx) {
    float v[8] = {P::lo(u.x), P::hi(u.x), P::lo(u.y), P::hi(u.y), P::lo(u.z), P::hi(u.z), P::lo(u.w), P::hi(u.w)};
#pragma unroll
    for (int k = 0; k < 8; k += 2) {
        const f32x2_t m = mish_fast2(fma2(f32x2_t{v[k], v[k + 1]}, f32x2_t{sc[k], sc[k + 1]}, f32x2_t{sh[k], sh[k + 1]}));
        v[k] = m.x;
        v[k + 1] = m.y;
        if (mx) {
            mx[k] = fmaxf(mx[k], v[k]);
            mx[k + 1] = fmaxf(mx[k + 1], v[k + 1]);
        }
    }
    uint4 r;
    r.x = PO::pack2(v[0], v[1]);
    r.y = PO::pack2(v[2], v[3]);
    r.z = PO::pack2(v[4], v[5]);
    r.w = PO::pack2(v[6], v[7]);
    return r;
}

template <class P, bool POOL, bool WB, bool NT = false, class PW = P, class PQ = P>
__global__ void __launch_bounds__(256) norm_mish_kernel(uint4* __restrict__ x, const float2* __restrict__ ss, int C,
                                                        int D, int H, int W, uint4* __restrict__ pooled) {
    const int c8 = blockIdx.y, n = blockIdx.z;
    float sc[8], sh[8];
#pragma unroll
    for (int k = 0; k < 8; ++k) {
        const float2 v = ss[n * C + c8 * 8 + k];
        sc[k] = v.x;
        sh[k] = v.y;
    }
    const long long vox = (long long)D * H * W;
    uint4* p = x + ((long long)n * (C / 8) + c8) * vox;
    if (!POOL) {
        for (long long i = (long long)blockIdx.x * 256 + threadIdx.x; i < vox; i += (long long)gridDim.x * 256)
            dlv_st16<NT>(p + i, norm_mish8<P, PW>(dlv_ld16<NT>(p + i), sc, sh, nullptr));
    } else {
        const int d2 = D / 2, h2 = H / 2, w2 = W / 2;
        const long long pv = (long long)d2 * h2 * w2;
        uint4* q = pooled + ((long long)n * (C / 8) + c8) * pv;
        for (long long i = (long long)blockIdx.x * 256 + threadIdx.x; i < pv; i += (long long)gridDim.x * 256) {
            const int xx = (int)(i % w2), yy = (int)((i / w2) % h2), zz = (int)(i / ((long long)w2 * h2));
            float mx[8];
#pragma unroll
            for (int k = 0; k < 8; ++k) mx[k] = -INFINITY;
#pragma unroll
            for (int a = 0; a < 2; ++a)
#pragma unroll
                for (int b = 0; b < 2; ++b) {
                    const long long o = ((long long)(2 * zz + a) * H + (2 * yy + b)) * W + 2 * xx;
                    const uint4 r0 = norm_mish8<P, PW>(p[o], sc, sh, mx), r1 = norm_mish8<P, PW>(p[o + 1], sc, sh, mx);
                    if (WB) {
                        p[o] = r0;
                        p[o + 1] = r1;
                    }
                }
            uint4 r;
            r.x = PQ::pack2(mx[0], mx[1]);
            r.y = PQ::pack2(mx[2], mx[3]);
            r.z = PQ::pack2(mx[4], mx[5]);
            r.w = PQ::pack2(mx[6], mx[7]);
            q[i] = r;
        }
    }
}

template <class P, bool WB, bool NT, class PQ = P>
__global__ void __launch_bounds__(256) norm_mish_pool_rows_kernel(uint4* __restrict__ x, const float2* __restrict__ ss, int C, int D, int H,
                                                                  int W, uint4* __restrict__ pooled) {
    const int c8 = blockIdx.y, n = blockIdx.z;
    float sc[8], sh[8];
#pragma unroll
    for (int k = 0; k < 8; ++k) {
        const float2 v = ss[n * C + c8 * 8 + k];
        sc[k] = v.x;
        sh[k] = v.y;
    }
    const long long vox = (long long)D * H * W;
    const int d2 = D / 2, h2 = H / 2, w2 = W / 2, nseg = W / 64;
    uint4* p = x + ((long long)n * (C / 8) + c8) * vox;
// ... 32 lines not shown
```

### delivr_cfos_amd/csrc/unet16_stem.h

```cpp
#pragma once
namespace {

constexpr int STEM_ZR = 4;

template <class P, bool FROM_VOLUME>
__global__ void __launch_bounds__(256) stem_conv_kernel(const float* __restrict__ xf, const uint16_t* __restrict__ vol,
                                                        int Yp, int Xp, const int* __restrict__ starts, int flip_dim,
                                                        const float* __restrict__ w, const float* __restrict__ bias,
                                                        uint4* __restrict__ out, float* __restrict__ partials, int D,
                                                        int H, int W, float oscale) {
    __shared__ float wl[27 * 32];
    __shared__ float red[4][64];
    for (int i = threadIdx.x; i < 27 * 32; i += 256) {
        const int t = i >> 5, co = i & 31;
        wl[i] = w[co * 27 + t];
    }
    __syncthreads();
    const int n = blockIdx.z;
    const int hw = H * W;
    const int p = blockIdx.x * 256 + threadIdx.x;
    const bool pvalid = p < hw;
    const int y = pvalid ? p / W : 0, x = pvalid ? p % W : 0;
    const int zb = blockIdx.y * STEM_ZR;
    int z0 = 0, y0 = 0, x0 = 0;
// ... 13 lines not shown
        return xf[(long long)n * D * hw + ((long long)zz * H + yy) * W + xx];
    };
    float s[32], q[32];
#pragma unroll
    for (int c = 0; c < 32; ++c) s[c] = q[c] = 0.f;
#pragma unroll 1
    for (int zi = 0; zi < STEM_ZR; ++zi) {
        const int z = zb + zi;
        if (z >= D || !pvalid) continue;
        float acc[32];
#pragma unroll
        for (int c = 0; c < 32; ++c) acc[c] = bias[c];
#pragma unroll 1
        for (int dz = 0; dz < 3; ++dz)
#pragma unroll 1
            for (int dy = 0; dy < 3; ++dy)
#pragma unroll
                for (int dx = 0; dx < 3; ++dx) {
                    const float v = fetch(z + dz - 1, y + dy - 1, x + dx - 1);
                    const float4* wr = reinterpret_cast<const float4*>(wl + ((dz * 3 + dy) * 3 + dx) * 32);
#pragma unroll
                    for (int c4 = 0; c4 < 8; ++c4) {
                        const float4 ww = wr[c4];
                        acc[4 * c4 + 0] = fmaf(v, ww.x, acc[4 * c4 + 0]);
                        acc[4 * c4 + 1] = fmaf(v, ww.y, acc[4 * c4 + 1]);
                        acc[4 * c4 + 2] = fmaf(v, ww.z, acc[4 * c4 + 2]);
                        acc[4 * c4 + 3] = fmaf(v, ww.w, acc[4 * c4 + 3]);
                    }
                }
        if (oscale != 1.0f) {
#pragma unroll
            for (int c = 0; c < 32; ++c) acc[c] *= oscale;
        }
        const long long vox = (long long)D * hw;
        const long long o = (long long)z * hw + p;
#pragma unroll
        for (int c8 = 0; c8 < 4; ++c8) {
            uint4 u;
            u.x = P::pack2(acc[8 * c8 + 0], acc[8 * c8 + 1]);
            u.y = P::pack2(acc[8 * c8 + 2], acc[8 * c8 + 3]);
            u.z = P::pack2(acc[8 * c8 + 4], acc[8 * c8 + 5]);
            u.w = P::pack2(acc[8 * c8 + 6], acc[8 * c8 + 7]);
            out[((long long)n * 4 + c8) * vox + o] = u;
        }
#pragma unroll
        for (int c = 0; c < 32; ++c) {
            s[c] += acc[c];
            q[c] = fmaf(acc[c], acc[c], q[c]);
        }
    }
    const int lane = threadIdx.x & 63, wave = threadIdx.x >> 6;
#pragma unroll
    for (int c = 0; c < 32; ++c) {
        float a = s[c], b = q[c];
        for (int o = 32; o > 0; o >>= 1) {
            a += __shfl_xor(a, o, 64);
            b += __shfl_xor(b, o, 64);
        }
        if (lane == 0) {
            red[wave][2 * c] = a;
            red[wave][2 * c + 1] = b;
        }
    }
    __syncthreads();
    if (threadIdx.x < 64) {
        const float v = red[0][threadIdx.x] + red[1][threadIdx.x] + red[2][threadIdx.x] + red[3][threadIdx.x];
        const long long blk = (long long)blockIdx.y * gridDim.x + blockIdx.x;
        const long long nblk = (long long)gridDim.x * gridDim.y;
        partials[((long long)n * nblk + blk) * 64 + threadIdx.x] = v;
    }
}

constexpr int SM_TZ = 4, SM_TY = 8, SM_TX = 32, SM_HZ = 6, SM_HY = 10, SM_HX = 34;
constexpr int SM_ZC = 8;
constexpr int SM_NT = SM_HZ * SM_HY * SM_HX;
constexpr int SM_NS = (SM_NT + 255) / 256;

template <class P, int MODE>
__global__ void __launch_bounds__(256) stem_mfma_kernel(const uint16_t* __restrict__ vol, int Yp, int Xp,
                                                        const int* __restrict__ starts, int flip_dim,
                                                        const uint4* __restrict__ wpk, const float* __restrict__ bias,
                                                        uint4* __restrict__ out, float* __restrict__ partials,
                                                        const float2* __restrict__ ss, int D, int H, int W, int tilesY,
                                                        int tilesX) {
    __shared__ unsigned tile[2][SM_NT];
    __shared__ float red[4 * 64];
    const int n = blockIdx.z;
    const int t = dlv_xcd_tile(blockIdx.x, gridDim.x);
    const int tx = t % tilesX, ty = (t / tilesX) % tilesY, tg = t / (tilesX * tilesY);
    const int zbase = tg * (SM_ZC * SM_TZ), y0 = ty * SM_TY, x0 = tx * SM_TX;
    const int nzc = min(SM_ZC, (D - zbase + SM_TZ - 1) / SM_TZ);
    const int wz = starts[3 * n], wy = starts[3 * n + 1], wx = starts[3 * n + 2];
    int soff[SM_NS], szh[SM_NS];
#pragma unroll
    for (int k = 0; k < SM_NS; ++k) {
        const int i = threadIdx.x + 256 * k;
        const int xh = i % SM_HX, yh = (i / SM_HX) % SM_HY, zh = i / (SM_HX * SM_HY);
        int gy = y0 + yh - 1, gx = x0 + xh - 1;
        const bool ok = i < SM_NT && (unsigned)gy < (unsigned)H && (unsigned)gx < (unsigned)W;
        if (flip_dim == 3) gy = H - 1 - gy;
        if (flip_dim == 4) gx = W - 1 - gx;
        soff[k] = ok ? (wy + gy) * Xp + (wx + gx) : -1;
        szh[k] = zh - 1;
    }
    const long long plane = (long long)Yp * Xp;
    unsigned sv[SM_NS];
    auto stage_load = [&](int zc) __attribute__((always_inline)) {
#pragma unroll
        for (int k = 0; k < SM_NS; ++k) {
            int gz = zbase + zc * SM_TZ + szh[k];
            const bool ok = soff[k] >= 0 && (unsigned)gz < (unsigned)D;
            if (flip_dim == 2) gz = D - 1 - gz;
            sv[k] = ok ? (unsigned)vol[(long long)(wz + gz) * plane + soff[k]] : 0u;
        }
    };
    auto stage_store = [&](int buf) __attribute__((always_inline)) {
#pragma unroll
        for (int k = 0; k < SM_NS; ++k) {
            const int i = threadIdx.x + 256 * k;
            if (i < SM_NT) tile[buf][i] = P::pack2((float)(sv[k] & 255u), (float)(sv[k] >> 8));
        }
    };
    stage_load(0);
    const int lane = threadIdx.x & 63, wave = threadIdx.x >> 6;
    const int h = lane >> 5, col = lane & 31;
    uint4 a[4];
#pragma unroll
    for (int s = 0; s < 4; ++s) a[s] = AS_FRAG(wpk[s * 64 + lane]);
    const f32x16 bsv = {};
    float ssum[16], ssq[16];
#pragma unroll
    for (int r = 0; r < 16; ++r) ssum[r] = ssq[r] = 0.f;
    float nsc[16], nsh[16];
    if (MODE == 2) {
#pragma unroll
        for (int r = 0; r < 16; ++r) {
            const float2 v = ss[n * 32 + (r & 3) + 8 * (r >> 2) + 4 * h];
            nsc[r] = v.x;
            nsh[r] = v.y;
        }
    }
    stage_store(0);
    __syncthreads();
    const long long vox = (long long)D * H * W;
    int tap_off[16];
#pragma unroll
    for (int i = 0; i < 16; ++i) {
        const int tp = 8 * (i >> 2) + 4 * h + (i & 3);
        const int tt = tp < 27 ? tp : 0;
        tap_off[i] = (wave * SM_HY * SM_HX + col) + ((tt / 9) * SM_HY + (tt / 3) % 3) * SM_HX + tt % 3;
    }
#pragma unroll 1
    for (int zc = 0; zc < nzc; ++zc) {
        if (zc + 1 < nzc) stage_load(zc + 1);
        const unsigned* tl = tile[zc & 1];
        const int oz = zbase + zc * SM_TZ + wave;
#pragma unroll
        for (int row = 0; row < SM_TY; ++row) {
            unsigned b[16];
#pragma unroll
            for (int i = 0; i < 16; ++i) b[i] = tl[tap_off[i] + row * SM_HX];
            f32x16 acc = P::mfma(a[0], AS_FRAG(make_uint4(b[0], b[1], b[2], b[3])), bsv, 0, 0, 0);
            acc = P::mfma(a[1], AS_FRAG(make_uint4(b[4], b[5], b[6], b[7])), acc, 0, 0, 0);
            acc = P::mfma(a[2], AS_FRAG(make_uint4(b[8], b[9], b[10], b[11])), acc, 0, 0, 0);
            acc = P::mfma(a[3], AS_FRAG(make_uint4(b[12], b[13], b[14], b[15])), acc, 0, 0, 0);
            const int oy = y0 + row, ox = x0 + col;
            const bool ok = oz < D && oy < H && ox < W;
            float val[16];
#pragma unroll
            for (int r = 0; r < 16; ++r) val[r] = acc[r];
            if (MODE != 2 && ok) {
#pragma unroll
                for (int r = 0; r < 16; ++r) {
                    ssum[r] += val[r];
                    ssq[r] = fmaf(val[r], val[r], ssq[r]);
                }
            }
            if (MODE == 2) {
#pragma unroll
                for (int r = 0; r < 16; r += 2) {
                    const f32x2_t m = mish_fast2(fma2(f32x2_t{val[r], val[r + 1]}, f32x2_t{nsc[r], nsc[r + 1]}, f32x2_t{nsh[r], nsh[r + 1]}));
                    val[r] = m.x;
                    val[r + 1] = m.y;
                }
            }
            if (MODE != 1 && ok) {
                const long long o = ((long long)oz * H + oy) * W + ox;
#pragma unroll
                for (int g = 0; g < 4; ++g) {
                    uint2 u;
                    u.x = P::pack2(val[4 * g + 0], val[4 * g + 1]);
                    u.y = P::pack2(val[4 * g + 2], val[4 * g + 3]);
                    uint2* dst = reinterpret_cast<uint2*>(out + ((long long)n * 4 + g) * vox + o);
                    dlv_st8<true>(dst + h, u);
                }
            }
        }
        if (zc + 1 < nzc) stage_store((zc + 1) & 1);
        __syncthreads();
    }
    if (MODE == 2) return;
#pragma unroll
    for (int r = 0; r < 16; ++r) {
        float sa = ssum[r], sb = ssq[r];
        sa = dlv_half_sum32(sa);
        sb = dlv_half_sum32(sb);
        if (col == 31) {
            const int co = (r & 3) + 8 * (r >> 2) + 4 * h;
            red[(wave * 32 + co) * 2] = sa;
            red[(wave * 32 + co) * 2 + 1] = sb;
        }
    }
    __syncthreads();
    if (threadIdx.x < 64) {
        const int i = threadIdx.x;
        partials[((long long)n * gridDim.x + t) * 64 + i] = red[i] + red[64 + i] + red[128 + i] + red[192 + i];
    }
}

}
```

### delivr_cfos_amd/csrc/unet_bf16.hip

```cpp
#include <algorithm>
#include <type_traits>

#include "common.h"
#include "prec16.h"

namespace {

#define AS_FRAG(x) (x)

__device__ __forceinline__ float mish_fast(float y) {
    const float n = __builtin_amdgcn_exp2f(y * 1.44269504f);
    const float d = fmaf(n, n + 2.f, 2.f);
    return fmaf(-2.f * y, __builtin_amdgcn_rcpf(d), y);
}

__device__ __forceinline__ f32x2_t mish_fast2(f32x2_t y) {
    const f32x2_t l2e = {1.44269504f, 1.44269504f}, two = {2.f, 2.f}, m2 = {-2.f, -2.f};
    const f32x2_t e = y * l2e;
    const f32x2_t n = {__builtin_amdgcn_exp2f(e.x), __builtin_amdgcn_exp2f(e.y)};
    const f32x2_t d = __builtin_elementwise_fma(n, n + two, two);
    const f32x2_t r = {__builtin_amdgcn_rcpf(d.x), __builtin_amdgcn_rcpf(d.y)};
    return __builtin_elementwise_fma(m2 * y, r, y);
}
__device__ __forceinline__ f32x2_t fma2(f32x2_t a, f32x2_t b, f32x2_t c) { return __builtin_elementwise_fma(a, b, c); }
// ... 214 lines not shown
        }
        if (kernel == DLV_PLAN_DC_ROWS)
            hipLaunchKernelGGL((deconv2_rows_kernel<P, KP>), dim3(dlv_cdiv(rowsegs, 4), B), dim3(256), 0, ctx->stream, in, w, L.bias, out, L.cout, din.D, din.H,
                               din.W, segs, ssin);
        else
            hipLaunchKernelGGL((deconv2_mfma_kernel<P, KP>), dim3(dlv_cdiv(din.vox(), 128), B), dim3(256), 0, ctx->stream, in, w, L.bias, out, L.cout, din.D,
                               din.H, din.W);
        return DLV_OK;
    }

    int deconv(int j, Act& a, uint4* out, Dims din) {
        const DlvDeconvLayer& L = ctx->deconv[j];
        const DlvDeconvPlan plan = plan_deconv(ctx->sw, L.cin, L.cout, a.ss != nullptr, din.D, din.H, din.W);
        if (plan.kernel == DLV_PLAN_NONE) return dlv_fail(ctx, DLV_EUNSUP, "deconv %d: Cin=%d not in {32,64,128,256}", j, L.cin);
        if (plan.norm_first) DLV_TRY(materialise(a, din));
        const DlvLabel lb = dlv_label_deconv(plan, P::IS_F16, L.cin, L.cout, B, din.D, din.H, din.W);
        DlvProf pr(ctx, lb.name, lb.flops, lb.bytes);
        if (plan.kernel == DLV_PLAN_DC_DEEP) {
            DLV_TRY(dlv_deconv2_deep_launch(ctx, P::IS_F16, L.cin, L.cout, a.p, P::IS_F16 ? L.w16_f16 : L.w16_bf16, L.bias, out, B, din.D, din.H, din.W));
            pr.end();
            return DLV_OK;
        }
        switch (L.cin / 16) {
            case 2: DLV_TRY(launch_deconv<2>(plan.kernel, L, a.p, a.ss, out, din)); break;
            case 4: DLV_TRY(launch_deconv<4>(plan.kernel, L, a.p, a.ss, out, din)); break;
            case 8: DLV_TRY(launch_deconv<8>(plan.kernel, L, a.p, a.ss, out, din)); break;
            default: DLV_TRY(launch_deconv<16>(plan.kernel, L, a.p, a.ss, out, din)); break;
        }
        pr.end();
        DLV_LAUNCH_CHECK(ctx, "deconv2 kernel");
        return DLV_OK;
    }
};

struct Ws16 {
    size_t act, stats, pfloats;
};
static Ws16 ws16_bytes(const int* f, int B, int d, int h, int w, size_t (*offs)[4]) {
    const int lvlC[5] = {32, f[1], f[2], f[3], f[4]};
    size_t off = 0;
    for (int l = 0; l < 5; ++l)
        for (int k = 0; k < 4; ++k) {
            if (offs) offs[l][k] = off;
            off += (size_t)B * lvlC[l] * ((size_t)(d >> l) * (h >> l) * (w >> l)) * 2;
            off = (off + 255) & ~(size_t)255;
        }
    const long long max_tiles = (long long)dlv_cdiv(d, 4) * dlv_cdiv(h, 4) * dlv_cdiv(w, 8) + 64;
    const size_t pfloats = (size_t)B * max_tiles * 64 * 2;
    return Ws16{off, pfloats * 4 + (size_t)DLV_N_CONV * B * 256 * sizeof(float2) + 256, pfloats};
}

template <class P0, class PD = P0>
int forward_16(dlv_ctx* ctx, const float* xf, const uint16_t* vol, int Yp, int Xp, const int* starts_dev, int flip_dim,
                 float scale, float* logits, float* acc, int B, int d, int h, int w) {
    const int* f = ctx->features;
    if (f[0] != 32 || f[5] != 32)
        return dlv_fail(ctx, DLV_EUNSUP, "bf16 path: features[0] and features[5] must be 32 (got %d, %d)", f[0], f[5]);
    if ((long long)d * h * w >= (1ll << 31)) return dlv_fail(ctx, DLV_EUNSUP, "16-bit path: a window of %d x %d x %d voxels exceeds the 2^31 voxel index range", d, h, w);
    Dims dm[5];
    for (int l = 0; l < 5; ++l) dm[l] = Dims{d >> l, h >> l, w >> l};
    size_t offs[5][4];
    Ws16 wsz = ws16_bytes(f, B, d, h, w, offs);
    const size_t off = wsz.act, pfloats = wsz.pfloats;
    char* base;
    DLV_TRY(dlv_ws_get(ctx, ctx->lane ? WS_LANE_ACT0 + (ctx->lane - 1) : WS_BF16_ACT, off, (void**)&base));
    char* sbase;
    DLV_TRY(dlv_ws_get(ctx, ctx->lane ? WS_LANE_STATS0 + (ctx->lane - 1) : WS_STATS, wsz.stats, (void**)&sbase));
    Net16<P0> net{ctx, B, (float*)sbase, pfloats, (float2*)(sbase + ((pfloats * 4 + 255) & ~(size_t)255))};
    Net16<PD> netd{ctx, B, net.partials, pfloats, net.ss_base};
    constexpr bool mixed = !std::is_same<P0, PD>::value;
    using P = P0;
    using Act = Act16;
    auto buf = [&](int l, int k) { return (uint4*)(base + offs[l][k]); };
    enum { A = 0, Bf = 1, S = 2, U = 3 };

    Act x0{buf(0, A), 32, nullptr};
    {
        dim3 grid(dlv_cdiv((long long)h * w, 256), dlv_cdiv(d, STEM_ZR), B);
        int nblk = grid.x * grid.y;
        bool two_pass_stem = false;
        if ((size_t)B * nblk * 64 > pfloats) return dlv_fail(ctx, DLV_ESTATE, "partials buffer too small (stem)");
        const DlvConvLayer& L = ctx->conv[0];
        const bool stem_mfma = plan_stem_mfma(ctx->sw, vol != nullptr);
        const DlvLabel lb = dlv_label_stem(stem_mfma, B, d, h, w);
        DlvProf pr(ctx, lb.name, lb.flops, lb.bytes);
        if (stem_mfma) {
            const int tY = dlv_cdiv(h, SM_TY), tX = dlv_cdiv(w, SM_TX), tZ = dlv_cdiv(d, SM_TZ * SM_ZC);
            grid = dim3(tZ * tY * tX, 1, B);
            nblk = grid.x;
            if ((size_t)B * nblk * 64 > pfloats) return dlv_fail(ctx, DLV_ESTATE, "partials buffer too small (stem)");
            const uint4* wst = reinterpret_cast<const uint4*>(wpack<P>(L));
            hipLaunchKernelGGL((stem_mfma_kernel<P, 1>), grid, dim3(256), 0, ctx->stream, vol, Yp, Xp, starts_dev, flip_dim, wst,
                               L.bias16, buf(0, A), net.partials, (const float2*)nullptr, d, h, w, tY, tX);
            DLV_LAUNCH_CHECK(ctx, "stem_mfma_kernel<1>");
            DLV_TRY(net.stats(nblk, 0, dm[0]));
            hipLaunchKernelGGL((stem_mfma_kernel<P, 2>), grid, dim3(256), 0, ctx->stream, vol, Yp, Xp, starts_dev, flip_dim, wst,
                               L.bias16, buf(0, A), net.partials, (const float2*)net.ss_of(0), d, h, w, tY, tX);
            two_pass_stem = true;
        } else if (vol)
            hipLaunchKernelGGL((stem_conv_kernel<P, true>), grid, dim3(256), 0, ctx->stream, nullptr, vol, Yp, Xp, starts_dev,
                               flip_dim, L.w_f32, L.bias, buf(0, A), net.partials, d, h, w, P::STEM_SCALE * exp2f(-(float)L.shift));
        else
            hipLaunchKernelGGL((stem_conv_kernel<P, false>), grid, dim3(256), 0, ctx->stream, xf, nullptr, 0, 0, nullptr, -1,
                               L.w_f32, L.bias, buf(0, A), net.partials, d, h, w, P::STEM_SCALE * exp2f(-(float)L.shift));
        pr.end();
        DLV_LAUNCH_CHECK(ctx, "stem_conv_kernel");
        if (!two_pass_stem) {
            DLV_TRY(net.stats(nblk, 0, dm[0]));
            x0.ss = net.ss_of(0);
        }
    }
    const int encC[5] = {32, f[1], f[2], f[3], f[4]};
    Act skip[5];
    {
        Act s0{buf(0, S), 32, nullptr};
        DLV_TRY(net.conv(1, x0, nullptr, s0.p, dm[0]));
        s0.ss = net.ss_of(1);
        skip[0] = s0;
    }
    for (int l = 1; l <= 4; ++l) {
        Act& up = skip[l - 1];
        const int li_cat = 18 - 2 * l;
        const int c_up = ctx->deconv[4 - l].cout;
        const DlvConvLayer& Lcat = ctx->conv[li_cat];
        const bool keep_raw = plan_conv(ctx->sw, li_cat, Lcat.cin, Lcat.cout, up.C, c_up, true, B, dm[l - 1].D, dm[l - 1].H, dm[l - 1].W).act_on_load;
        const bool odd = ((dm[l - 1].D | dm[l - 1].H | dm[l - 1].W) & 1) != 0;
        if (l == 1) {
            DLV_TRY((net.template norm_mish<P0, PD>(up.p, up.C, dm[0], buf(1, A), up.ss, !keep_raw && !odd)));
            if (odd && !keep_raw) DLV_TRY(net.norm_mish(up.p, up.C, dm[0], nullptr, up.ss, true));
        } else {
            DLV_TRY(netd.norm_mish(up.p, up.C, dm[l - 1], buf(l, A), up.ss, !keep_raw && !odd));
            if (odd && !keep_raw) DLV_TRY(netd.norm_mish(up.p, up.C, dm[l - 1], nullptr, up.ss, true));
        }
        if (!keep_raw) up.ss = nullptr;
        Act a{buf(l, A), encC[l - 1], nullptr};
        Act b{buf(l, Bf), encC[l], nullptr};
        DLV_TRY(netd.conv(2 * l, a, nullptr, b.p, dm[l]));
        b.ss = net.ss_of(2 * l);
        Act s{buf(l, S), encC[l], nullptr};
        DLV_TRY(netd.conv(2 * l + 1, b, nullptr, s.p, dm[l]));
        s.ss = net.ss_of(2 * l + 1);
        skip[l] = s;
    }
    Act cur = skip[4];
    for (int j = 0; j < 4; ++j) {
        const int l = 3 - j;
        const int li = 10 + 2 * j;
        Act b{buf(l, Bf), ctx->conv[li].cout, nullptr};
        if (l >= 1) {
            DLV_TRY(netd.deconv_to(j, cur, buf(l, U), buf(l, A), dm[l + 1], dm[l]));
            Act u{buf(l, U), ctx->deconv[j].cout, nullptr};
            DLV_TRY(netd.conv(li, skip[l], &u, b.p, dm[l]));
            b.ss = net.ss_of(li);
            Act o{buf(l, A), ctx->conv[li + 1].cout, nullptr};
            DLV_TRY(netd.conv(li + 1, b, nullptr, o.p, dm[l]));
            o.ss = net.ss_of(li + 1);
            cur = o;
            continue;
        }
        if (mixed) DLV_TRY((netd.template materialise<P0>(cur, dm[1])));
        if (net.plan_fold(li, skip[l].C, dm[l])) {
            DLV_TRY(net.conv_folded(li, skip[l], cur, buf(l, U), b.p, dm[l], dm[l + 1]));
        } else {
            DLV_TRY(net.deconv_to(j, cur, buf(l, U), buf(l, A), dm[l + 1], dm[l]));
            Act u{buf(l, U), ctx->deconv[j].cout, nullptr};
            DLV_TRY(net.conv(li, skip[l], &u, b.p, dm[l]));
        }
        b.ss = net.ss_of(li);
        Act o{buf(l, A), ctx->conv[li + 1].cout, nullptr};
        DLV_TRY(net.conv(li + 1, b, nullptr, o.p, dm[l]));
        o.ss = net.ss_of(li + 1);
        cur = o;
    }
    {
        dim3 grid(std::min(net.grid1d(dm[0].vox()), 512), B);
        const DlvLabel lb = dlv_label_final(acc != nullptr, B, d, h, w);
        DlvProf pr(ctx, lb.name, lb.flops, lb.bytes);
        if (acc)
            hipLaunchKernelGGL((final_conv_kernel<P, true>), grid, dim3(256), 0, ctx->stream, cur.p, cur.ss, ctx->final_w,
                               ctx->final_b, nullptr, starts_dev, flip_dim, Yp, Xp, scale, acc, d, h, w, ctx->blend_w, ctx->blend_min,
// ... 41 lines not shown
}

template <class P>
int debug_layer_16(dlv_ctx* ctx, dlv_debug_layer_args& a) {
    const int B = a.B, D = a.D, H = a.H, W = a.W;
    const Dims d{D, H, W};
    const long long vox = d.vox();
    a.ran_zreg = a.ran_upconv = a.ran_stem = a.drops_bias = a.drops_fold_const = 0;
    a.raw_scale = 1.f;
    ctx->ran_zreg = ctx->ran_upconv = 0;
    if (B < 1 || D < 1 || H < 1 || W < 1) return dlv_fail(ctx, DLV_EINVAL, "debug layer: empty shape");
    const int kind = a.kind;
    if (kind == 1) {
        if (a.op != DLV_DBG_CONV) return dlv_fail(ctx, DLV_EINVAL, "kind 1 (deconv) runs as op 0 only");
        const int index = a.index, c1 = a.c1;
        if (index < 0 || index >= DLV_N_DECONV) return dlv_fail(ctx, DLV_EINVAL, "deconv index must be 0..3");
        const DlvDeconvLayer& L = ctx->deconv[index];
        if (!a.in1 || c1 != L.cin || a.c2 != 0 || a.ss1) return dlv_fail(ctx, DLV_EINVAL, "bad channels");
        const size_t b1 = (size_t)B * c1 * vox * 2, bo = (size_t)B * L.cout * vox * 8 * 2;
        char* base;
        DLV_TRY(dlv_ws_get(ctx, WS_BF16_ACT, b1 + bo + 1024, (void**)&base));
        uint4 *i1 = (uint4*)base, *o = (uint4*)(base + ((b1 + 255) & ~(size_t)255));
        Net16<P> net{ctx, B, nullptr, 0, nullptr};
        hipLaunchKernelGGL(f32_to_cp_kernel<P>, dim3(net.grid1d(vox), c1 / 8, B), dim3(256), 0, ctx->stream, a.in1, i1, c1, vox);
        typename Net16<P>::Act t1{i1, c1, nullptr};
        DLV_TRY(net.deconv(index, t1, o, d));
        hipLaunchKernelGGL(cp_to_f32_kernel<P>, dim3(net.grid1d(vox * 8), L.cout / 8, B), dim3(256), 0, ctx->stream, o, a.out,
                           L.cout, vox * 8);
        DLV_LAUNCH_CHECK(ctx, "debug deconv");
        return DLV_OK;
    }
    if (kind != 0 && kind != 2 && kind != 3) return dlv_fail(ctx, DLV_EINVAL, "kind must be 0 (final), 1 (deconv), 2 (raw) or 3 (scale/shift)");
    const int li = a.op == DLV_DBG_STEM ? 0 : a.index;
    if (a.op == DLV_DBG_FOLDED && li != 16) return dlv_fail(ctx, DLV_EINVAL, "the folded conv is block 16");
    if (a.op == DLV_DBG_CONV && (li < 1 || li >= DLV_N_CONV)) return dlv_fail(ctx, DLV_EINVAL, "conv index must be 1..17");
    if (a.op < DLV_DBG_CONV || a.op > DLV_DBG_STEM) return dlv_fail(ctx, DLV_EINVAL, "op must be 0 (conv), 1 (folded) or 2 (stem)");
    const DlvConvLayer& L = ctx->conv[li];
    int c1 = a.c1, c2 = a.c2;
    long long vox2 = vox;
    if (a.op == DLV_DBG_STEM) {
        if (!a.vol) return dlv_fail(ctx, DLV_EINVAL, "the stem reads vol");
        if (a.flip_dim != -1 && (a.flip_dim < 2 || a.flip_dim > 4)) return dlv_fail(ctx, DLV_EINVAL, "flip_dim must be -1 or 2..4");
        c1 = c2 = 0;
    } else {
        if (!a.in1) return dlv_fail(ctx, DLV_EINVAL, "in1 missing");
        if (a.op == DLV_DBG_FOLDED) {
            if (c1 != 32 || c2 != 32 || !a.in2 || D % 2 || H % 2 || W % 2) return dlv_fail(ctx, DLV_EINVAL, "folded conv: 32 fine + 32 coarse channels, even sizes");
            vox2 = vox / 8;
        } else if (c1 + c2 != L.cin || c1 % 32 || c2 % 32 || (c2 && !a.in2)) {
            return dlv_fail(ctx, DLV_EINVAL, "bad channel split");
        }
    }
    const bool folded = a.op == DLV_DBG_FOLDED;
    auto al = [](size_t b) { return (b + 255) & ~(size_t)255; };
    const size_t b1 = (size_t)B * c1 * vox * 2, b2 = (size_t)B * c2 * vox2 * 2, bp = folded ? (size_t)B * 32 * vox * 2 : 0,
                 bo = (size_t)B * L.cout * vox * 2, bst = (size_t)B * 3 * sizeof(int);
    const long long tiles = (long long)dlv_cdiv(D, 4) * dlv_cdiv(H, 4) * dlv_cdiv(W, 8) + 64;
    const size_t pf = (size_t)B * tiles * std::max(L.cout, 64) * 2;
    char* base;
    DLV_TRY(dlv_ws_get(ctx, WS_BF16_ACT, al(b1) + al(b2) + al(bp) + al(bo) + al(bst) + 1024, (void**)&base));
    char* sbase;
    DLV_TRY(dlv_ws_get(ctx, WS_STATS, al(pf * 4) + Net16<P>::ss_bytes(B) + 256, (void**)&sbase));
    uint4 *i1 = (uint4*)base, *i2 = (uint4*)(base + al(b1)), *pb = (uint4*)(base + al(b1) + al(b2)),
          *o = (uint4*)(base + al(b1) + al(b2) + al(bp));
    int* starts = (int*)(base + al(b1) + al(b2) + al(bp) + al(bo));
    Net16<P> net{ctx, B, (float*)sbase, pf, (float2*)(sbase + al(pf * 4))};
    const int g = net.grid1d(vox);
    if (c1) hipLaunchKernelGGL(f32_to_cp_kernel<P>, dim3(g, c1 / 8, B), dim3(256), 0, ctx->stream, a.in1, i1, c1, vox);
    if (c2) hipLaunchKernelGGL(f32_to_cp_kernel<P>, dim3(net.grid1d(vox2), c2 / 8, B), dim3(256), 0, ctx->stream, a.in2, i2, c2, vox2);
    DLV_LAUNCH_CHECK(ctx, "debug layer: f32_to_cp_kernel");
    bool final_written = false;
    if (a.op == DLV_DBG_STEM) {
        std::vector<int> st(3 * (size_t)B, 0);
        for (int n = 0; n < B; ++n) st[3 * n] = n * D;
        DLV_HIP(ctx, hipMemcpyAsync(starts, st.data(), bst, hipMemcpyHostToDevice, ctx->stream));
        DLV_HIP(ctx, hipStreamSynchronize(ctx->stream));
        const int tY = dlv_cdiv(H, SM_TY), tX = dlv_cdiv(W, SM_TX), tZ = dlv_cdiv(D, SM_TZ * SM_ZC);
        const dim3 grid(tZ * tY * tX, 1, B);
        if ((size_t)B * grid.x * 64 > pf) return dlv_fail(ctx, DLV_ESTATE, "partials buffer too small (stem)");
        const uint4* wst = reinterpret_cast<const uint4*>(wpack<P>(L));
        const uint16_t* vol = reinterpret_cast<const uint16_t*>(a.vol);
        if (kind == 2)
            hipLaunchKernelGGL((stem_mfma_kernel<P, 0>), grid, dim3(256), 0, ctx->stream, vol, H, W, starts, a.flip_dim, wst,
                               L.bias16, o, net.partials, (const float2*)nullptr, D, H, W, tY, tX);
        else
            hipLaunchKernelGGL((stem_mfma_kernel<P, 1>), grid, dim3(256), 0, ctx->stream, vol, H, W, starts, a.flip_dim, wst,
                               L.bias16, o, net.partials, (const float2*)nullptr, D, H, W, tY, tX);
        DLV_LAUNCH_CHECK(ctx, "debug stem_mfma_kernel");
        DLV_TRY(net.stats((int)grid.x, 0, d));
        if (kind == 0) {
            hipLaunchKernelGGL((stem_mfma_kernel<P, 2>), grid, dim3(256), 0, ctx->stream, vol, H, W, starts, a.flip_dim, wst,
                               L.bias16, o, net.partials, (const float2*)net.ss_of(0), D, H, W, tY, tX);
            DLV_LAUNCH_CHECK(ctx, "debug stem_mfma_kernel<2>");
            final_written = true;
        }
        a.ran_stem = 1;
        a.drops_bias = 1;
        a.raw_scale = P::STEM_SCALE * exp2f(-(float)L.shift);
    } else {
        typename Net16<P>::Act t1{i1, c1, reinterpret_cast<const float2*>(a.ss1)}, t2{i2, c2, nullptr};
        if (folded) {
            if (!net.plan_fold(16, 32, d)) return dlv_fail(ctx, DLV_EUNSUP, "debug layer: a forward does not fold block 16 at %dx%dx%d", D, H, W);
            DLV_TRY(net.conv_folded(16, t1, t2, pb, o, d, Dims{D / 2, H / 2, W / 2}));
            a.drops_fold_const = 1;
        } else {
            DLV_TRY(net.conv(li, t1, c2 ? &t2 : nullptr, o, d));
        }
        a.raw_scale = exp2f(-(float)L.shift);
    }
    a.ran_zreg = ctx->ran_zreg;
    a.ran_upconv = ctx->ran_upconv;
    a.drops_bias |= a.ran_zreg != 0;
    if (kind == 3) {
        DLV_HIP(ctx, hipMemcpyAsync(a.out, net.ss_of(li), (size_t)B * L.cout * sizeof(float2), hipMemcpyDeviceToDevice, ctx->stream));
        return DLV_OK;
    }
    if (kind == 0 && !final_written) DLV_TRY(net.norm_mish(o, L.cout, d, nullptr, net.ss_of(li), true));
    hipLaunchKernelGGL(cp_to_f32_kernel<P>, dim3(g, L.cout / 8, B), dim3(256), 0, ctx->stream, o, a.out, L.cout, vox);
    DLV_LAUNCH_CHECK(ctx, "debug layer");
    return DLV_OK;
}

}

int dlv_pack_weights_bf16(dlv_ctx* ctx) {
    DLV_TRY(pack_weights_16<PBf16>(ctx));
    return pack_weights_16<PF16>(ctx);
}

int dlv_unet_reserve_16(dlv_ctx* ctx, int B, int d, int h, int w, int lanes) {
    if (!ctx->weights_loaded && ctx->features[1] == 0) return DLV_OK;
    const Ws16 wsz = ws16_bytes(ctx->features, B, d, h, w, nullptr);
    void* p;
    for (int lane = 0; lane < std::max(1, std::min(lanes, DLV_MAX_LANES)); ++lane) {
        DLV_TRY(dlv_ws_get(ctx, lane ? WS_LANE_ACT0 + (lane - 1) : WS_BF16_ACT, wsz.act, &p));
        DLV_TRY(dlv_ws_get(ctx, lane ? WS_LANE_STATS0 + (lane - 1) : WS_STATS, wsz.stats, &p));
    }
    return DLV_OK;
}

int dlv_range_reset(dlv_ctx* ctx) {
    DLV_HIP(ctx, hipMemsetAsync(ctx->range_flag, 0, sizeof(int) * (1 + DLV_N_CONV), ctx->main_stream));
    return DLV_OK;
}

int dlv_range_check(dlv_ctx* ctx, int fmt16) {
    const bool f16 = fmt16 != 0;
    int words[1 + DLV_N_CONV] = {0};
    DLV_HIP(ctx, hipMemcpyAsync(words, ctx->range_flag, sizeof(words), hipMemcpyDeviceToHost, ctx->main_stream));
    DLV_HIP(ctx, hipStreamSynchronize(ctx->main_stream));
    const int flag = words[0];
    for (int i = 0; i < DLV_N_CONV; ++i) memcpy(&ctx->range_peak[i], &words[1 + i], sizeof(float));
    ctx->range_last = flag == 0 ? -1 : 100 - flag;
    if (flag == 0) {
        ctx->range_seq = false;
        ctx->range_blind_layer = -1;
        return DLV_OK;
    }
    const int layer = 100 - flag;
    static const char* const names[DLV_N_CONV] = {"conv_0.conv_0", "conv_0.conv_1", "down_1.conv_0", "down_1.conv_1", "down_2.conv_0",
                                                  "down_2.conv_1", "down_3.conv_0", "down_3.conv_1", "down_4.conv_0", "down_4.conv_1",
                                                  "upcat_4.conv_0", "upcat_4.conv_1", "upcat_3.conv_0", "upcat_3.conv_1", "upcat_2.conv_0",
                                                  "upcat_2.conv_1", "upcat_1.conv_0", "upcat_1.conv_1"};
    if (layer >= 0 && layer < DLV_N_CONV)
        return dlv_fail(ctx, DLV_ERANGE, "%s range exceeded: the InstanceNorm sums of conv block %d (%s) are not finite - a value of its input "
                        "(the block before it or the transposed conv feeding it) left the format%s", fmt16 == 2 ? "fp16 (level 0 of DLV_PREC_BF16)" : (f16 ? "fp16" : "bf16"), layer, names[layer],
                        f16 ? "; use dlv_unet_set_conv_shift on the producing block (dlv_range_report) or DLV_PREC_BF16_ALL (8 exponent bits) for this checkpoint" : "");
    return dlv_fail(ctx, DLV_ERANGE, "%s range exceeded: non-finite logits (raw output of the last conv block, upcat_1.conv_1)%s",
                    fmt16 == 2 ? "fp16 (level 0 of DLV_PREC_BF16)" : (f16 ? "fp16" : "bf16"), f16 ? "; use dlv_unet_set_conv_shift on upcat_1.conv_1 (dlv_range_report) or DLV_PREC_BF16_ALL (8 exponent bits) for this checkpoint" : "");
}

int dlv_unet_forward_bf16(dlv_ctx* ctx, const float* x, float* logits, int B, int d, int h, int w, int fmt16) {
    DLV_TRY(dlv_range_reset(ctx));
    if (fmt16 == 1) DLV_TRY(forward_16<PF16>(ctx, x, nullptr, 0, 0, nullptr, -1, 1.f, logits, nullptr, B, d, h, w));
    else if (fmt16 == 2) DLV_TRY((forward_16<PF16, PBf16>(ctx, x, nullptr, 0, 0, nullptr, -1, 1.f, logits, nullptr, B, d, h, w)));
    else DLV_TRY(forward_16<PBf16>(ctx, x, nullptr, 0, 0, nullptr, -1, 1.f, logits, nullptr, B, d, h, w));
    return dlv_range_check(ctx, fmt16);
}

int dlv_unet_tiles_bf16(dlv_ctx* ctx, const uint16_t* vol, int Yp, int Xp, const int* starts_dev, int B, int d, int h,
                        int w, int flip_dim, float scale, float* acc, int fmt16) {
    if (fmt16 == 1) return forward_16<PF16>(ctx, nullptr, vol, Yp, Xp, starts_dev, flip_dim, scale, nullptr, acc, B, d, h, w);
    if (fmt16 == 2) return forward_16<PF16, PBf16>(ctx, nullptr, vol, Yp, Xp, starts_dev, flip_dim, scale, nullptr, acc, B, d, h, w);
    return forward_16<PBf16>(ctx, nullptr, vol, Yp, Xp, starts_dev, flip_dim, scale, nullptr, acc, B, d, h, w);
}

extern "C" int dlv_debug_layer16(dlv_ctx* ctx, dlv_debug_layer_args* args) {
    if (!ctx || !args || !args->out) return DLV_EINVAL;
    if (!ctx->weights_loaded) return dlv_fail(ctx, DLV_ESTATE, "no weights");
    DLV_HIP(ctx, hipSetDevice(ctx->device));
    if (ctx->debug_f16) return debug_layer_16<PF16>(ctx, *args);
    return debug_layer_16<PBf16>(ctx, *args);
}

extern "C" int dlv_debug_layer_bf16(dlv_ctx* ctx, int kind, int index, const float* in1_dev, int c1, const float* in2_dev,
                                    int c2, float* out_dev, int B, int D, int H, int W) {
    if (!in1_dev) return DLV_EINVAL;
    dlv_debug_layer_args a{};
    a.kind = kind;
    a.op = DLV_DBG_CONV;
    a.index = index;
    a.in1 = in1_dev;
    a.c1 = c1;
    a.in2 = in2_dev;
    a.c2 = c2;
// ... 9 lines not shown
```

### delivr_cfos_amd/engine.py

```python
from __future__ import annotations

import ctypes as C
from typing import Dict, Optional, Sequence, Tuple

import numpy as np

from . import _lib
from ._lib import PREC_BF16, PREC_BF16_ALL, PREC_F16, PREC_F32, DelivrHipError

PRECISIONS = {"fp32": PREC_F32, "f32": PREC_F32, "bf16": PREC_BF16, "fp16": PREC_F16, "f16": PREC_F16, "bf16_all": PREC_BF16_ALL}
RANGE_GUARDED = ("fp16", "f16", "bf16")

CONV_BLOCKS = (
    ["conv_0.conv_0", "conv_0.conv_1"]
    + [f"down_{k}.convs.conv_{j}" for k in (1, 2, 3, 4) for j in (0, 1)]
    + [f"upcat_{k}.convs.conv_{j}" for k in (4, 3, 2, 1) for j in (0, 1)]
)
DECONV_BLOCKS = [f"upcat_{k}.upsample.deconv" for k in (4, 3, 2, 1)]


def strip_state_dict(checkpoint) -> Dict[str, "np.ndarray"]:
    sd = checkpoint
    if isinstance(sd, dict):
        for key in ("state_dict", "model_state"):
# ... 29 lines not shown

    def close(self):
        if getattr(self, "handle", None):
            self.lib.dlv_comm_destroy(self.handle)
            self.handle = None
            for e in self.engines:
                e.ctx = None

    def _check(self, rc: int):
        if rc != 0:
            raise DelivrHipError(rc, self.lib.dlv_comm_last_error(self.handle).decode(errors="replace"))

    @property
    def uses_rccl(self) -> bool:
        return bool(self.lib.dlv_comm_uses_rccl(self.handle))

    def selftest(self, nbytes: int = 64 << 20) -> None:
        self._check(self.lib.dlv_comm_selftest(self.handle, int(nbytes)))

    def bcast_weights(self, root: int = 0):
        self._check(self.lib.dlv_bcast_weights(self.handle, int(root)))
        for e in self.engines:
            e.features = self.engines[root].features

    def range_recover(self) -> int:
        n = C.c_int()
        self._check(self.lib.dlv_comm_range_recover(self.handle, C.byref(n)))
        return n.value

    def make_plan(self, params, weights=None):
        from .parallel import plan_from_params

        return plan_from_params(params, len(self.devices), weights)

    def sw_infer_sharded(self, params, plan, slabs, vols, accs, cnts=None, wsums=None):
        n = len(self.devices)
        pc = _lib.ShardPlanC()
        pc.world, pc.n_windows = n, plan.n_windows
        for r in range(n):
            pc.win_begin[r], pc.win_end[r] = plan.win_ranges[r]
            pc.z_comp_lo[r], pc.z_comp_hi[r] = plan.z_computed[r]
            pc.z_own_lo[r], pc.z_own_hi[r] = plan.z_owned[r]
        z0 = (C.c_int * n)(*[int(s[0]) for s in slabs])
        nz = (C.c_int * n)(*[int(s[1]) for s in slabs])
        torch = self.torch
        vp = (C.c_void_p * n)(*[self.engines[r]._dev(vols[r], torch.uint16, "vol").value for r in range(n)])
        ap = (C.c_void_p * n)(*[self.engines[r]._dev(accs[r], torch.float32, "acc").value for r in range(n)])
        cp = None
        if cnts is not None:
            cp = (C.c_void_p * n)(*[self.engines[r]._dev(cnts[r], torch.uint8, "cnt").value for r in range(n)])
        st = (_lib.SwStats * n)()
        for d in set(self.devices):
            torch.cuda.synchronize(d)
        if wsums is None:
            self._check(self.lib.dlv_sw_infer_sharded(self.handle, C.byref(params), C.byref(pc), z0, nz, vp, ap, cp, st))
        else:
            wp = (C.c_void_p * n)(*[self.engines[r]._dev(wsums[r], torch.float32, "wsum").value for r in range(n)])
            self._check(self.lib.dlv_sw_infer_sharded_wsum(self.handle, C.byref(params), C.byref(pc), z0, nz, vp, ap, cp, wp, st))
        return [{"n_windows": s.n_windows, "n_skipped": s.n_skipped, "n_forward_launches": s.n_forward_launches} for s in st]


_shared_engines: Dict[int, "HipEngine"] = {}
_shared_comms: Dict[Tuple[int, ...], HipComm] = {}


def shared_comm(devices: Sequence[int]) -> HipComm:
    key = tuple(int(d) for d in devices)
    comm = _shared_comms.get(key)
    if comm is None or comm.handle is None:
        comm = HipComm(key)
        _shared_comms[key] = comm
    return comm


def shared_engine(device: int = 0) -> "HipEngine":
    eng = _shared_engines.get(int(device))
    if eng is None or eng.ctx is None:
        eng = HipEngine(int(device))
        eng.shared = True
        _shared_engines[int(device)] = eng
    return eng


def layer_plan(window, switches=None, precision="fp16", batch=1, features=(32, 32, 64, 128, 256, 32)):
    lib = _lib.load()
    sw = dict(switches or {})
    names = (C.c_char_p * max(1, len(sw)))(*[k.encode() for k in sw])
    values = (C.c_int * max(1, len(sw)))(*[int(v) for v in sw.values()])
    out = _lib.LayerPlan()
    rc = lib.dlv_diag_plan((C.c_int * 6)(*features), names, values, len(sw), {"bf16_all": 0, "fp16": 1, "bf16": 2}[precision], int(batch),
                           *(int(v) for v in window), C.byref(out))
    if rc != 0:
        raise DelivrHipError(rc, f"dlv_diag_plan: window {tuple(window)}, switches {sw}")

    def fields(st, kernels):
        d = {name: getattr(st, name) for name, _ in st._fields_}
        d["kernel"] = None if st.kernel < 0 else kernels[st.kernel]
        return d

    return {"conv": [fields(c, _lib.PLAN_CONV_KERNELS) for c in out.conv],
            "deconv": [fields(c, _lib.PLAN_DECONV_KERNELS) for c in out.deconv],
            "pool": [{name: getattr(p, name) for name, _ in p._fields_} for p in out.pool],
            "labels": [(out.labels[i].value.decode(), out.flops[i], out.bytes[i]) for i in range(out.n_labels)]}


class HipEngine:
    shared = False

    def __init__(self, device: int = 0, _ctx=None):
        import torch

        if not torch.cuda.is_available():
            raise RuntimeError("delivr_cfos_amd needs an MI355X (torch.cuda.is_available() is False); "
                               "there is no CPU fallback for the HIP path")
        self.torch = torch
        self.lib = _lib.load()
        self.device_index = int(device)
        self.device = torch.device("cuda", self.device_index)
        self.features: Optional[Tuple[int, ...]] = None
        self._keep = []
        self._owns_ctx = _ctx is None
        if _ctx is not None:
            self.ctx = _ctx
            self.tstream = torch.cuda.ExternalStream(self.lib.dlv_stream(_ctx), device=self.device)
            return
        self.tstream = torch.cuda.Stream(device=self.device)
        ctx = C.c_void_p()
        rc = self.lib.dlv_ctx_create(self.device_index, C.c_void_p(self.tstream.cuda_stream), C.byref(ctx))
        if rc != 0:
            raise DelivrHipError(rc, "dlv_ctx_create failed")
        self.ctx = ctx

    def close(self):
        if getattr(self, "ctx", None) and getattr(self, "_owns_ctx", True):
            self.lib.dlv_ctx_destroy(self.ctx)
        self.ctx = None

    def __del__(self):
        try:
            self.close()
        except Exception:
            pass

    def _check(self, rc: int):
        if rc != 0:
            raise DelivrHipError(rc, self.lib.dlv_last_error(self.ctx).decode(errors="replace"))

    def _enter(self):
        self.tstream.wait_stream(self.torch.cuda.current_stream(self.device))

    def _leave(self):
        self.torch.cuda.current_stream(self.device).wait_stream(self.tstream)

    def sync(self):
        self._check(self.lib.dlv_sync(self.ctx))

    def _dev(self, t, dtype, name):
        torch = self.torch
        if not isinstance(t, torch.Tensor) or t.device != self.device:
            raise TypeError(f"{name}: expected a torch tensor on {self.device}, got {type(t)} on "
                            f"{getattr(t, 'device', None)}")
        if t.dtype != dtype:
            raise TypeError(f"{name}: expected dtype {dtype}, got {t.dtype}")
        if not t.is_contiguous():
            raise ValueError(f"{name}: tensor must be contiguous")
        return C.c_void_p(t.data_ptr())

    def to_device(self, arr, dtype=None):
        torch = self.torch
        if isinstance(arr, torch.Tensor):
            t = arr
        else:
            a = np.ascontiguousarray(arr)
            if not a.flags.writeable:
                a = np.array(a)
            t = torch.from_numpy(a)
        if dtype is not None and t.dtype != dtype:
            t = t.to(dtype)
        return t.to(self.device).contiguous()

    def upload_volume(self, arr, z_lo: int = 0, z_hi: Optional[int] = None, chunk_bytes: int = 64 << 20):
        from . import hostio

        a = arr if isinstance(arr, np.ndarray) else np.asarray(arr)
        lead = a.shape[:-3]
# ... 132 lines not shown
        a.B, a.D, a.H, a.W = int(B), int(D), int(H), int(W)
        self._check(self.lib.dlv_debug_set_format(self.ctx, PREC_F16 if precision in ("fp16", "f16") else PREC_BF16_ALL))
        self._enter()
        self._check(self.lib.dlv_debug_layer16(self.ctx, C.byref(a)))
        self._leave()
        zr = a.ran_zreg
        report = {
            "zreg": None if not zr else "{}_c{}_t{}_{}".format("f16" if zr & 2 else "bf16", 64 if zr & 4 else 32, 16 if zr & 8 else 8,
                                                              ("adda1" if zr & 16 else "add") if zr & 32 else ("a1" if zr & 16 else "a0")),
            "upconv": {0: None, 1: "upconv2", 2: "upconv2m"}[a.ran_upconv],
            "stem": bool(a.ran_stem),
            "drops_bias": bool(a.drops_bias),
            "drops_fold_const": bool(a.drops_fold_const),
            "raw_scale": float(a.raw_scale),
        }
        return out, report

    def make_sw_params(self, padded_shape, roi, overlap=0.5, flip_dim=None, skip_threshold=0, precision="fp16",
                       sw_batch=0, win_range=None, slab=None, repeat=1, blend="constant", sigma_scale=0.125,
                       wsum=None) -> _lib.SwParams:
        p = _lib.SwParams()
        p.Zp, p.Yp, p.Xp = (int(v) for v in padded_shape)
        for k in range(3):
            p.roi[k] = int(roi[k])
        p.overlap = float(overlap)
        p.flip_dim = -1 if flip_dim is None else int(flip_dim)
        p.skip_threshold = int(skip_threshold)
        p.precision = PRECISIONS[precision]
        p.sw_batch = int(sw_batch)
        p.win_begin, p.win_end = (0, 0) if win_range is None else (int(win_range[0]), int(win_range[1]))
        p.z0, p.nz = (0, 0) if slab is None else (int(slab[0]), int(slab[1]))
        p.repeat = int(repeat)
        p.blend_mode = {"constant": 0, "gaussian": 1}[blend]
        p.sigma_scale = float(sigma_scale)
        if wsum is not None:
            if blend != "gaussian":
                raise ValueError("wsum is the float count map of the Gaussian blend")
            p.wsum_dev = self._dev(wsum, self.torch.float32, "wsum").value
            p._keep = wsum
        return p

    def num_windows(self, params) -> int:
        n = C.c_int64()
        rc = self.lib.dlv_sw_num_windows(C.byref(params), C.byref(n))
        if rc != 0:
            raise DelivrHipError(rc, "dlv_sw_num_windows: bad geometry")
        return n.value

    def window_starts(self, params) -> np.ndarray:
        n = self.num_windows(params)
        buf = np.zeros((n, 3), dtype=np.int64)
        rc = self.lib.dlv_sw_window_starts(C.byref(params), buf.ctypes.data_as(C.POINTER(C.c_int64)), n)
        if rc != 0:
            raise DelivrHipError(rc, "dlv_sw_window_starts failed")
        return buf

    def window_max(self, params, vol) -> np.ndarray:
        n = self.num_windows(params)
        if params.win_end > 0 or params.win_begin > 0:
            n = max(min(int(params.win_end) if params.win_end > 0 else n, n) - max(int(params.win_begin), 0), 0)
        out = np.zeros(n, dtype=np.int32)
        if n == 0:
            return out
        self._enter()
        self._check(self.lib.dlv_sw_window_max_dev(self.ctx, C.byref(params), self._dev(vol, self.torch.uint16, "vol"),
                                                   out.ctypes.data_as(C.POINTER(C.c_int32)), n))
        self._leave()
        return out

    def reserve(self, params, stack_shape=None) -> None:
        Z, Y, X = (int(v) for v in stack_shape) if stack_shape is not None else (0, 0, 0)
        self._check(self.lib.dlv_reserve_dev(self.ctx, C.byref(params), Z, Y, X))

    def sw_infer(self, params, vol, acc, cnt=None) -> dict:
        torch = self.torch
        st = _lib.SwStats()
        self._enter()
        self._check(self.lib.dlv_sw_infer_dev(
            self.ctx, C.byref(params), self._dev(vol, torch.uint16, "vol"), self._dev(acc, torch.float32, "acc"),
            self._dev(cnt, torch.uint8, "cnt") if cnt is not None else None, C.byref(st)))
        self._leave()
        return {"n_windows": st.n_windows, "n_skipped": st.n_skipped, "n_forward_launches": st.n_forward_launches}

    def finalize(self, acc, cnt, raw, stack_shape, threshold=0.5, erode_iters=30, zblock=0, want_prob=False, out=None):
        torch = self.torch
        Z, Y, X = (int(v) for v in stack_shape)
        Yp, Xp = int(acc.shape[-2]), int(acc.shape[-1])
        if cnt is not None and cnt.dtype == torch.float32:
            acc = acc / cnt.clamp_min(torch.finfo(torch.float32).tiny)
            cnt = None
        if out is None:
            out = torch.empty((Z, Y, X), dtype=torch.uint8, device=self.device)
        elif tuple(out.shape) != (Z, Y, X):
            raise ValueError(f"finalize: out has shape {tuple(out.shape)}, the stack {(Z, Y, X)}")
        prob = torch.empty((Z, Y, X), dtype=torch.float32, device=self.device) if want_prob else None
        self._enter()
        self._check(self.lib.dlv_finalize_dev(
            self.ctx, self._dev(acc, torch.float32, "acc"),
            self._dev(cnt, torch.uint8, "cnt") if cnt is not None else None, self._dev(raw, torch.uint16, "raw"),
            Yp, Xp, Z, Y, X, float(threshold), int(erode_iters), int(zblock),
            self._dev(out, torch.uint8, "out"), self._dev(prob, torch.float32, "prob") if want_prob else None))
        self._leave()
        return (out, prob) if want_prob else out

    def finalize_slab(self, acc, cnt, raw, z_abs0: int, stack_yx, threshold=0.5, erode_iters=30, zblock=0, want_prob=False):
        torch = self.torch
        nz = int(acc.shape[0])
        Y, X = (int(v) for v in stack_yx)
        Yp, Xp = int(acc.shape[-2]), int(acc.shape[-1])
        if cnt is not None and cnt.dtype == torch.float32:
            acc = acc / cnt.clamp_min(torch.finfo(torch.float32).tiny)
            cnt = None
        out = torch.empty((nz, Y, X), dtype=torch.uint8, device=self.device)
        prob = torch.empty((nz, Y, X), dtype=torch.float32, device=self.device) if want_prob else None
        self._enter()
        self._check(self.lib.dlv_finalize_slab_dev(
            self.ctx, self._dev(acc, torch.float32, "acc"), self._dev(cnt, torch.uint8, "cnt") if cnt is not None else None,
            self._dev(raw, torch.uint16, "raw"), Yp, Xp, int(z_abs0), nz, Y, X, float(threshold), int(erode_iters), int(zblock),
            self._dev(out, torch.uint8, "out"), self._dev(prob, torch.float32, "prob") if want_prob else None))
        self._leave()
        return (out, prob) if want_prob else out

    def ccl26(self, mask):
        torch = self.torch
        Z, Y, X = (int(v) for v in mask.shape)
        labels = torch.empty((Z, Y, X), dtype=torch.int32, device=self.device)
        n = C.c_uint64()
        self._enter()
        self._check(self.lib.dlv_ccl26_dev(self.ctx, self._dev(mask, torch.uint8, "mask"), Z, Y, X,
                                           C.c_void_p(labels.data_ptr()), C.byref(n)))
        self._leave()
        return labels, int(n.value)

    def cc_stats(self, labels, n: int) -> dict:
        Z, Y, X = (int(v) for v in labels.shape)
        counts = np.zeros(n + 1, dtype=np.uint32)
        bbox = np.zeros((n + 1, 6), dtype=np.uint16)
        cent = np.zeros((n + 1, 3), dtype=np.float64)
        self._enter()
        self._check(self.lib.dlv_cc_stats_dev(self.ctx, C.c_void_p(labels.data_ptr()), Z, Y, X, n,
                                              counts.ctypes.data_as(C.c_void_p), bbox.ctypes.data_as(C.c_void_p),
                                              cent.ctypes.data_as(C.c_void_p)))
        self._leave()
        return {"voxel_counts": counts, "bounding_boxes": bbox, "centroids": cent}

    def cc_stats_raw(self, labels, n: int) -> dict:
        Z, Y, X = (int(v) for v in labels.shape)
        counts = np.zeros(n + 1, dtype=np.uint32)
        bbmin = np.zeros((n + 1, 3), dtype=np.uint32)
        bbmax = np.zeros((n + 1, 3), dtype=np.uint32)
        sums = np.zeros((n + 1, 3), dtype=np.uint64)
        self._enter()
        self._check(self.lib.dlv_cc_stats_raw_dev(self.ctx, C.c_void_p(labels.data_ptr()), Z, Y, X, n,
                                                  counts.ctypes.data_as(C.c_void_p), bbmin.ctypes.data_as(C.c_void_p),
                                                  bbmax.ctypes.data_as(C.c_void_p), sums.ctypes.data_as(C.c_void_p)))
        self._leave()
        return {"counts": counts, "bbmin": bbmin, "bbmax": bbmax, "sums": sums}

    def seam_pairs(self, plane_a, plane_b) -> np.ndarray:
        torch = self.torch
        Y, X = (int(v) for v in plane_a.shape)
        a = self._dev(plane_a, torch.int32, "plane_a")
        b = self._dev(plane_b, torch.int32, "plane_b")
        cnt = C.c_uint64()
        self._enter()
        self._check(self.lib.dlv_seam_pairs_dev(self.ctx, a, b, Y, X, None, 0, C.byref(cnt)))
# ... 290 lines not shown
```

### include/delivr_hip_diag.h

```cpp
#ifndef DELIVR_HIP_DIAG_H
#define DELIVR_HIP_DIAG_H
#include "delivr_hip.h"
#ifdef __cplusplus
extern "C" {
#endif

int dlv_diag_set(dlv_ctx* ctx, const char* name, int value);

int dlv_debug_set_zm_variant(dlv_ctx* ctx, int variant);
int dlv_debug_stamps(dlv_ctx* ctx, void* buf_dev);
int dlv_debug_set_format(dlv_ctx* ctx, int precision);
int dlv_debug_layer_bf16(dlv_ctx* ctx, int kind, int index, const float* in1_dev, int c1, const float* in2_dev,
                         int c2, float* out_dev, int B, int D, int H, int W);

#define DLV_DBG_CONV 0
#define DLV_DBG_FOLDED 1
#define DLV_DBG_STEM 2
#define DLV_DBG_ZR_RAN 1
#define DLV_DBG_ZR_F16 2
#define DLV_DBG_ZR_C64 4
#define DLV_DBG_ZR_T16 8
#define DLV_DBG_ZR_ACT 16
#define DLV_DBG_ZR_ADD 32
typedef struct dlv_debug_layer_args {
    int kind, op, index;
    const float* in1;
    int c1;
    const float* ss1;
    const float* in2;
    int c2;
    const unsigned short* vol;
    int flip_dim;
    float* out;
    int B, D, H, W;
    int ran_zreg, ran_upconv, ran_stem, drops_bias, drops_fold_const;
    float raw_scale;
} dlv_debug_layer_args;
int dlv_debug_layer16(dlv_ctx* ctx, dlv_debug_layer_args* args);

#define DLV_PLAN_NONE (-1)
#define DLV_PLAN_ZREG 0
#define DLV_PLAN_DEEP 1
#define DLV_PLAN_ZMARCH 2
#define DLV_PLAN_GENERIC 3
#define DLV_PLAN_STEM_MFMA 4
#define DLV_PLAN_STEM_VALU 5
#define DLV_PLAN_DC_DEEP 0
#define DLV_PLAN_DC_REGW 1
#define DLV_PLAN_DC_WST 2
#define DLV_PLAN_DC_ROWS 3
#define DLV_PLAN_DC_PARITY 4
#define DLV_PLAN_MAX_LABELS 96
typedef struct dlv_plan_conv {
    int kernel, level, cin, cout;
    int folded;
    int tile_rows;
    int act_on_load;
    int tx, ncb, wlds;
    long long max_parts;
} dlv_plan_conv;
typedef struct dlv_plan_deconv {
    int kernel;
    int norm_first;
    int padded;
} dlv_plan_deconv;
typedef struct dlv_plan_pool {
    int rows;
    int writeback;
    int norm_after;
    int nt;
} dlv_plan_pool;
typedef struct dlv_layer_plan {
    dlv_plan_conv conv[DLV_N_CONV];
    dlv_plan_deconv deconv[DLV_N_DECONV];
    dlv_plan_pool pool[4];
    int n_labels;
    char labels[DLV_PLAN_MAX_LABELS][48];
    double flops[DLV_PLAN_MAX_LABELS], bytes[DLV_PLAN_MAX_LABELS];
} dlv_layer_plan;
int dlv_diag_plan(const int features[6], const char* const* names, const int* values, int n, int fmt16, int B, int d, int h, int w,
                  dlv_layer_plan* out);

#ifdef __cplusplus
}
#endif
#endif
```

Baseline: 819.0 million voxels/s.

## Share stem norm statistics across overlapping windows via per-cell precomputed sums

Adds a pre-pass that splits the volume into scan-interval cells, computes the stem conv's per-channel sum and sum-of-squares once per cell, and lets each window assemble its instance-norm statistics from its cells. This replaces the separate per-window statistics pass of the two-pass MFMA stem. Windows overlap by half, so each cell is otherwise recomputed by up to eight windows. Window-boundary face voxels still need a small correction pass. The change adds host-side cell bookkeeping, a new scratch slot and a debug hook, and the double-precision reassembly risks small numeric differences.

```diff
diff --git a/delivr_cfos_amd/_lib.py b/delivr_cfos_amd/_lib.py
--- a/delivr_cfos_amd/_lib.py
+++ b/delivr_cfos_amd/_lib.py
@@ -103,7 +103,7 @@
 class LayerPlan(C.Structure):
     _fields_ = [("conv", PlanConv * N_CONV), ("deconv", PlanDeconv * N_DECONV), ("pool", PlanPool * 4), ("n_labels", C.c_int),
                 ("labels", (C.c_char * 48) * PLAN_MAX_LABELS), ("flops", C.c_double * PLAN_MAX_LABELS),
-                ("bytes", C.c_double * PLAN_MAX_LABELS)]
+                ("bytes", C.c_double * PLAN_MAX_LABELS), ("stem_stats_pass", C.c_int)]
 
 
 class SwParams(C.Structure):
@@ -212,6 +212,9 @@
     "dlv_diag_set": (C.c_int, [_P, C.c_char_p, C.c_int]),
     "dlv_diag_plan": (C.c_int, [C.POINTER(C.c_int), C.POINTER(C.c_char_p), C.POINTER(C.c_int), C.c_int, C.c_int, C.c_int, C.c_int,
                                 C.c_int, C.c_int, C.POINTER(LayerPlan)]),
+    "dlv_diag_plan_sw": (C.c_int, [C.POINTER(C.c_int), C.POINTER(C.c_char_p), C.POINTER(C.c_int), C.c_int, C.c_int, C.c_int, C.POINTER(C.c_int),
+                                   C.POINTER(C.c_int), C.c_float, C.POINTER(LayerPlan)]),
+    "dlv_debug_sw_stem_stats": (C.c_int, [_P, _P, _P, _P, C.POINTER(C.c_int)]),
     "dlv_cells_csv": (C.c_int, [_P, _P, C.c_uint64, _P, C.c_size_t, C.POINTER(C.c_size_t)]),
     "dlv_reserve_dev": (C.c_int, [_P, _P, C.c_int, C.c_int, C.c_int]),
     "dlv_debug_stamps": (C.c_int, [_P, _P]),
diff --git a/delivr_cfos_amd/csrc/api.hip b/delivr_cfos_amd/csrc/api.hip
--- a/delivr_cfos_amd/csrc/api.hip
+++ b/delivr_cfos_amd/csrc/api.hip
@@ -665,6 +665,21 @@
     return dlv_plan_forward(sw, upconv_simple, features, fmt16, B, d, h, w, out) ? DLV_OK : DLV_EUNSUP;
 }
 
+int dlv_diag_plan_sw(const int features[6], const char* const* names, const int* values, int n, int fmt16, int B, const int roi[3],
+                     const int volume[3], float overlap, dlv_layer_plan* out) {
+    if (!features || !out || !roi || !volume || n < 0 || (n > 0 && (!names || !values)) || fmt16 < 0 || fmt16 > 2) return DLV_EINVAL;
+    DlvPlanSwitches sw;
+    bool upconv_simple = false;
+    for (int i = 0; i < n; ++i) {
+        if (!names[i]) return DLV_EINVAL;
+        if (strcmp(names[i], "upconv_simple") == 0) upconv_simple = values[i] != 0;
+        else if (strcmp(names[i], "zreg_dbg") == 0) continue;
+        else if (!dlv_plan_switch_set(sw, names[i], values[i])) return DLV_EINVAL;
+    }
+    const bool shared = plan_stem_shared(sw, plan_stem_mfma(sw, true), volume, roi, overlap).on;
+    return dlv_plan_forward(sw, upconv_simple, features, fmt16, B, roi[0], roi[1], roi[2], out, shared) ? DLV_OK : DLV_EUNSUP;
+}
+
 int dlv_debug_stamps(dlv_ctx* ctx, void* buf_dev) {
     if (!ctx) return DLV_EINVAL;
     ctx->stamp_buf = buf_dev;
diff --git a/delivr_cfos_amd/csrc/common.h b/delivr_cfos_amd/csrc/common.h
--- a/delivr_cfos_amd/csrc/common.h
+++ b/delivr_cfos_amd/csrc/common.h
@@ -66,9 +66,19 @@
     WS_ERODE,
     WS_CCL,
     WS_MISC,
+    WS_STEM_SHARED,
     WS_LANE_ACT0,
     WS_LANE_STATS0 = WS_LANE_ACT0 + DLV_MAX_LANES - 1,
     WS_N_SLOTS = WS_LANE_STATS0 + DLV_MAX_LANES - 1
+};
+
+struct DlvStemShared {
+    const double* cell_sums = nullptr;
+    const int* win_cells = nullptr;
+    int ncw = 0;
+    int Zv = 0;
+    float2* capture = nullptr;
+    const int* capture_idx = nullptr;
 };
 
 struct dlv_ctx {
@@ -107,6 +117,7 @@
     size_t ws_bytes[WS_N_SLOTS] = {0};
     bool debug_f16 = false;
     DlvPlanSwitches sw;
+    DlvStemShared stem;
     int zreg_dbg = 0;
     int ran_zreg = 0, ran_upconv = 0;
     bool erode_xy_split = false, erode_z_two_sweeps = false, ccl_simple = false;
@@ -192,6 +203,9 @@
 int dlv_unet_forward_bf16(dlv_ctx* ctx, const float* x, float* logits, int B, int d, int h, int w, int fmt16);
 int dlv_unet_tiles_bf16(dlv_ctx* ctx, const uint16_t* vol, int Yp, int Xp, const int* starts_dev, int B, int d,
                         int h, int w, int flip_dim, float scale, float* acc, int fmt16);
+int dlv_stem_cell_stats(dlv_ctx* ctx, const uint16_t* vol, int Zv, int Yp, int Xp, const int* origins_dev, int ncells, const int cell[3],
+                        int flip_dim, int fmt16, float* scratch, size_t scratch_floats, double* sums_dev);
+size_t dlv_stem_cell_scratch_floats(int ncells, const int cell[3]);
 int dlv_pack_weights_bf16(dlv_ctx* ctx);
 int dlv_unet_reserve_16(dlv_ctx* ctx, int B, int d, int h, int w, int lanes);
 int dlv_conv3_zmarch_launch(dlv_ctx* ctx, bool f16, int cin, int cout, const void* in1, int c1, const void* in2, int c2,
diff --git a/delivr_cfos_amd/csrc/layer_plan.h b/delivr_cfos_amd/csrc/layer_plan.h
--- a/delivr_cfos_amd/csrc/layer_plan.h
+++ b/delivr_cfos_amd/csrc/layer_plan.h
@@ -15,6 +15,7 @@
     int fuse_levels = 0;
     int fold_up = 1;
     bool pool_rows_off = false;
+    bool stem_shared_stats = true;
 };
 
 inline bool dlv_plan_switch_set(DlvPlanSwitches& s, const char* name, int value) {
@@ -29,6 +30,7 @@
     else if (is("generic_ncb")) s.generic_ncb = value;
     else if (is("deep_small")) s.deep_small = value;
     else if (is("pool_rows_off")) s.pool_rows_off = value != 0;
+    else if (is("stem_shared_stats")) s.stem_shared_stats = value != 0;
     else return false;
     return true;
 }
@@ -188,6 +190,36 @@
 }
 inline bool plan_stem_mfma(const DlvPlanSwitches& sw, bool from_volume) { return from_volume && !sw.no_zmarch; }
 
+inline int dlv_sw_scan_interval(int roi, int n, float overlap) {
+    int iv = roi == n ? roi : (int)((double)roi * (1.0 - (double)overlap));
+    return iv <= 0 ? 1 : iv;
+}
+struct DlvStemSharedPlan {
+    bool on = false;
+    int cell[3] = {0, 0, 0};
+    int per_win[3] = {0, 0, 0};
+    int ncell[3] = {0, 0, 0};
+};
+inline DlvStemSharedPlan plan_stem_shared(const DlvPlanSwitches& sw, bool stem_mfma, const int n[3], const int roi[3], float overlap) {
+    DlvStemSharedPlan p;
+    if (!sw.stem_shared_stats || !stem_mfma) return p;
+    bool shared = false;
+    for (int k = 0; k < 3; ++k) {
+        if (roi[k] < 2 || n[k] < roi[k]) return p;
+        const int iv = dlv_sw_scan_interval(roi[k], n[k], overlap);
+        if (roi[k] % iv != 0 || (n[k] - roi[k]) % iv != 0) return p;
+        p.cell[k] = iv;
+        p.per_win[k] = roi[k] / iv;
+        p.ncell[k] = n[k] / iv;
+        shared = shared || (n[k] > roi[k] && iv < roi[k]);
+    }
+    p.on = shared;
+    return p;
+}
+inline long long dlv_window_face_voxels(int D, int H, int W) {
+    return (long long)D * H * W - (long long)(D - 2) * (H - 2) * (W - 2);
+}
+
 struct DlvLabel {
     char name[48];
     double flops, bytes;
@@ -246,6 +278,14 @@
     l.bytes = vox * B * (2 + 64);
     return l;
 }
+inline DlvLabel dlv_label_stem_faces(int B, int D, int H, int W) {
+    DlvLabel l;
+    const double fv = (double)dlv_window_face_voxels(D, H, W);
+    snprintf(l.name, sizeof(l.name), "stem_face_stats_u16");
+    l.flops = 2.0 * 2.0 * 27 * 32 * fv * B;
+    l.bytes = 2.0 * fv * B;
+    return l;
+}
 inline DlvLabel dlv_label_final(bool blend, int B, int D, int H, int W) {
     DlvLabel l;
     const double vox = (double)((long long)D * H * W);
@@ -255,7 +295,8 @@
     return l;
 }
 
-inline bool dlv_plan_forward(const DlvPlanSwitches& sw, bool upconv_simple, const int f[6], int fmt16, int B, int d, int h, int w, dlv_layer_plan* out) {
+inline bool dlv_plan_forward(const DlvPlanSwitches& sw, bool upconv_simple, const int f[6], int fmt16, int B, int d, int h, int w, dlv_layer_plan* out,
+                             bool stem_shared = false) {
     memset(out, 0, sizeof(*out));
     if (f[0] != 32 || f[5] != 32 || B < 1 || !dlv_window_supported(d, h, w)) return false;
     for (int i = 0; i < 6; ++i)
@@ -321,6 +362,8 @@
     out->conv[0].kernel = stem_mfma ? DLV_PLAN_STEM_MFMA : DLV_PLAN_STEM_VALU;
     out->conv[0].cin = 1;
     out->conv[0].cout = 32;
+    out->stem_stats_pass = !(stem_shared && stem_mfma);
+    if (!out->stem_stats_pass) emit(dlv_label_stem_faces(B, d, h, w));
     emit(dlv_label_stem(stem_mfma, B, d, h, w));
     T x0{32, !stem_mfma};
     T skip[5];
diff --git a/delivr_cfos_amd/csrc/sw_infer.hip b/delivr_cfos_amd/csrc/sw_infer.hip
--- a/delivr_cfos_amd/csrc/sw_infer.hip
+++ b/delivr_cfos_amd/csrc/sw_infer.hip
@@ -25,8 +25,7 @@
             return dlv_fail(ctx, DLV_EUNSUP, "roi[%d]=%d exceeds the padded volume (%d): pad the volume first "
                             "(downsample_and_mask.py:390-396 does)", k, r, t.n[k]);
         t.roi[k] = r;
-        int iv = r == t.n[k] ? r : (int)((double)r * (1.0 - (double)p->overlap));
-        if (iv <= 0) iv = 1;
+        const int iv = dlv_sw_scan_interval(r, t.n[k], p->overlap);
         t.iv[k] = iv;
         const int num = (t.n[k] + iv - 1) / iv;
         int scan = num - 1;
@@ -343,9 +342,10 @@
     return DLV_OK;
 }
 
-int dlv_sw_infer_dev(dlv_ctx* ctx, const dlv_sw_params* p, const uint16_t* vol_dev, float* acc_dev, uint8_t* cnt_dev,
-                     dlv_sw_stats* stats) {
-    if (!ctx || !p || !vol_dev || !acc_dev) return DLV_EINVAL;
+}
+
+static int sw_infer_pass(dlv_ctx* ctx, const dlv_sw_params* p, const uint16_t* vol_dev, float* acc_dev, uint8_t* cnt_dev, dlv_sw_stats* stats,
+                         float2* capture, int* shared_out) {
     if (!ctx->weights_loaded) return dlv_fail(ctx, DLV_ESTATE, "dlv_sw_infer_dev before dlv_unet_load");
     if (p->precision != DLV_PREC_F32 && p->precision != DLV_PREC_BF16 && p->precision != DLV_PREC_F16 && p->precision != DLV_PREC_BF16_ALL)
         return dlv_fail(ctx, DLV_EINVAL, "unknown precision %d", p->precision);
@@ -457,8 +457,9 @@
     std::vector<int> wmax((size_t)nwin);
     DLV_TRY(window_maxima(ctx, vol_dev, Yp, Xp, t.roi, starts, nwin, wmax.data()));
 
-    std::vector<int> list;
+    std::vector<int> list, list_win;
     list.reserve((size_t)nwin * 3);
+    list_win.reserve((size_t)nwin);
     struct Seg { size_t off; int n_active, n_skipped; };
     std::vector<Seg> segs;
     int64_t n_skipped = 0;
@@ -471,12 +472,85 @@
                 list.push_back(starts[3 * i]);
                 list.push_back(starts[3 * i + 1]);
                 list.push_back(starts[3 * i + 2]);
+                list_win.push_back(i);
                 if (skip) ++s.n_skipped; else ++s.n_active;
             }
         n_skipped += s.n_skipped;
         segs.push_back(s);
     }
     DLV_HIP(ctx, hipMemcpyAsync(list_dev, list.data(), list.size() * sizeof(int), hipMemcpyHostToDevice, ctx->stream));
+
+    struct StemReset {
+        dlv_ctx* c;
+        ~StemReset() { c->stem = DlvStemShared(); }
+    } stem_reset{ctx};
+    ctx->stem = DlvStemShared();
+    const bool stem16 = p->precision != DLV_PREC_F32 && plan_stem_mfma(ctx->sw, true);
+    const DlvStemSharedPlan ssp = plan_stem_shared(ctx->sw, stem16, t.n, t.roi, p->overlap);
+    if (capture && !stem16) return dlv_fail(ctx, DLV_EUNSUP, "the stem statistics hook needs the MFMA stem of a 16-bit precision");
+    if (shared_out) *shared_out = ssp.on ? 1 : 0;
+    const int ncw = ssp.on ? ssp.per_win[0] * ssp.per_win[1] * ssp.per_win[2] : 0;
+    const int* win_cells_dev = nullptr;
+    const int* list_win_dev = nullptr;
+    std::vector<int> stem_host;
+    if (ssp.on || capture) {
+        const size_t n_list = list_win.size();
+        std::vector<int> cell_id, origins;
+        std::vector<int> wcells(n_list * (size_t)ncw, 0);
+        int ncells = 0;
+        if (ssp.on) {
+            cell_id.assign((size_t)ssp.ncell[0] * ssp.ncell[1] * ssp.ncell[2], -1);
+            const auto cell_at = [&](size_t e, int a, int b, int c) {
+                const int cz = (list[3 * e] + z0) / ssp.cell[0] + a, cy = list[3 * e + 1] / ssp.cell[1] + b, cx = list[3 * e + 2] / ssp.cell[2] + c;
+                return ((size_t)cz * ssp.ncell[1] + cy) * ssp.ncell[2] + cx;
+            };
+            size_t e = 0;
+            for (const Seg& sg : segs)
+                for (int k = 0; k < sg.n_active + sg.n_skipped; ++k, ++e) {
+                    if (k >= sg.n_active) continue;
+                    for (int a = 0; a < ssp.per_win[0]; ++a)
+                        for (int b = 0; b < ssp.per_win[1]; ++b)
+                            for (int c = 0; c < ssp.per_win[2]; ++c) cell_id[cell_at(e, a, b, c)] = 0;
+                }
+            for (size_t i = 0; i < cell_id.size(); ++i)
+                if (cell_id[i] == 0) {
+                    cell_id[i] = ncells++;
+                    const int cx = (int)(i % ssp.ncell[2]), cy = (int)((i / ssp.ncell[2]) % ssp.ncell[1]), cz = (int)(i / ((size_t)ssp.ncell[2] * ssp.ncell[1]));
+                    origins.push_back(cz * ssp.cell[0] - z0);
+                    origins.push_back(cy * ssp.cell[1]);
+                    origins.push_back(cx * ssp.cell[2]);
+                }
+            e = 0;
+            for (const Seg& sg : segs)
+                for (int k = 0; k < sg.n_active + sg.n_skipped; ++k, ++e) {
+                    if (k >= sg.n_active) continue;
+                    int m = 0;
+                    for (int a = 0; a < ssp.per_win[0]; ++a)
+                        for (int b = 0; b < ssp.per_win[1]; ++b)
+                            for (int c = 0; c < ssp.per_win[2]; ++c) wcells[e * ncw + m++] = cell_id[cell_at(e, a, b, c)];
+                }
+        }
+        stem_host = origins;
+        stem_host.insert(stem_host.end(), wcells.begin(), wcells.end());
+        stem_host.insert(stem_host.end(), list_win.begin(), list_win.end());
+        const size_t sums_bytes = (size_t)ncells * 64 * sizeof(double);
+        const size_t scratch_floats = ncells ? dlv_stem_cell_scratch_floats(ncells, ssp.cell) : 0;
+        const size_t scratch_bytes = (scratch_floats * sizeof(float) + 255) & ~(size_t)255;
+        char* sb;
+        DLV_TRY(dlv_ws_get(ctx, WS_STEM_SHARED, sums_bytes + scratch_bytes + stem_host.size() * sizeof(int) + 256, (void**)&sb));
+        int* ints = (int*)(sb + sums_bytes + scratch_bytes);
+        DLV_HIP(ctx, hipMemcpyAsync(ints, stem_host.data(), stem_host.size() * sizeof(int), hipMemcpyHostToDevice, ctx->stream));
+        win_cells_dev = ints + origins.size();
+        list_win_dev = win_cells_dev + wcells.size();
+        if (ncells > 0) {
+            DLV_TRY(dlv_stem_cell_stats(ctx, vol_dev, nz, Yp, Xp, ints, ncells, ssp.cell, p->flip_dim, dlv_fmt16(p->precision),
+                                        (float*)(sb + sums_bytes), scratch_floats, (double*)sb));
+            ctx->stem.cell_sums = (const double*)sb;
+            ctx->stem.ncw = ncw;
+            ctx->stem.Zv = nz;
+        }
+        ctx->stem.capture = capture;
+    }
 
     int sw_batch = p->sw_batch;
     if (sw_batch <= 0) sw_batch = default_sw_batch(tile_vox);
@@ -506,6 +580,8 @@
             if (p->precision != DLV_PREC_F32) {
                 ctx->lane = two_lanes ? lane : 0;
                 ctx->stream = lane_stream(ctx->lane);
+                ctx->stem.win_cells = win_cells_dev ? win_cells_dev + (s.off + b0) * (size_t)ncw : nullptr;
+                ctx->stem.capture_idx = list_win_dev ? list_win_dev + (s.off + b0) : nullptr;
                 rc = dlv_unet_tiles_bf16(ctx, vol_dev, Yp, Xp, st_dev, B, d, h, w, p->flip_dim, (float)rep, acc_dev, dlv_fmt16(p->precision));
                 if (rc == DLV_OK && cnt_dev) {
                     hipLaunchKernelGGL(fill_add_kernel, dim3(bchunks, B), dim3(256), 0, ctx->stream, st_dev, d, h, w, Yp,
@@ -530,7 +606,7 @@
         }
         ctx->stream = ctx->main_stream;
         ctx->lane = 0;
-        if (rc == DLV_OK && s.n_skipped > 0) {
+        if (rc == DLV_OK && s.n_skipped > 0 && !capture) {
             const int* st_dev = list_dev + (s.off + s.n_active) * 3;
             DlvProf pr(ctx, "skip_fill_f32", 0.0, 8.0 * tile_vox * s.n_skipped);
             hipLaunchKernelGGL(fill_add_kernel, dim3(bchunks, s.n_skipped), dim3(256), 0, ctx->stream, st_dev, d, h, w,
@@ -551,4 +627,20 @@
     return DLV_OK;
 }
 
-}
+extern "C" {
+
+int dlv_sw_infer_dev(dlv_ctx* ctx, const dlv_sw_params* p, const uint16_t* vol_dev, float* acc_dev, uint8_t* cnt_dev,
+                     dlv_sw_stats* stats) {
+    if (!ctx || !p || !vol_dev || !acc_dev) return DLV_EINVAL;
+    return sw_infer_pass(ctx, p, vol_dev, acc_dev, cnt_dev, stats, nullptr, nullptr);
+}
+
+int dlv_debug_sw_stem_stats(dlv_ctx* ctx, const dlv_sw_params* p, const unsigned short* vol_dev, float* ss_dev, int* shared_out) {
+    if (!ctx || !p || !vol_dev || !ss_dev) return DLV_EINVAL;
+    if (p->precision == DLV_PREC_F32) return dlv_fail(ctx, DLV_EUNSUP, "the stem statistics hook runs the 16-bit precisions");
+    dlv_sw_params q = *p;
+    q.blend_mode = DLV_BLEND_CONSTANT;
+    return sw_infer_pass(ctx, &q, vol_dev, nullptr, nullptr, nullptr, reinterpret_cast<float2*>(ss_dev), shared_out);
+}
+
+}
diff --git a/delivr_cfos_amd/csrc/unet16_norm.h b/delivr_cfos_amd/csrc/unet16_norm.h
--- a/delivr_cfos_amd/csrc/unet16_norm.h
+++ b/delivr_cfos_amd/csrc/unet16_norm.h
@@ -1,5 +1,19 @@
 #pragma once
 namespace {
+
+__device__ __forceinline__ void stats_write(double s, double q, int c, double inv_count, float eps, const float* __restrict__ gamma,
+                                            const float* __restrict__ beta, float2* __restrict__ ss, int* __restrict__ range_flag, int layer) {
+    if (!(fabs(s) <= 1.0e300 && fabs(q) <= 1.0e300)) atomicMax(range_flag, 100 - layer);
+    const double mean = s * inv_count;
+    double var = q * inv_count - mean * mean;
+    if (var < 0.0) var = 0.0;
+    const float peak = (float)(fabs(mean) + 8.0 * sqrt(var));
+    if (peak > 0.f && peak < 3.0e38f && __float_as_int(peak) > __builtin_nontemporal_load(range_flag + 1 + layer))
+        atomicMax(range_flag + 1 + layer, __float_as_int(peak));
+    const float rstd = (float)(1.0 / sqrt(var + (double)eps));
+    const float sc = rstd * gamma[c];
+    *ss = make_float2(sc, beta[c] - (float)mean * sc);
+}
 
 __global__ void __launch_bounds__(64) stats_finalize_kernel(const float* __restrict__ partials, int nparts, int C,
                                                             double inv_count, float eps, const float* __restrict__ gamma,
@@ -16,18 +30,34 @@
         s += __shfl_down(s, o, 64);
         q += __shfl_down(q, o, 64);
     }
-    if (threadIdx.x == 0) {
-        if (!(fabs(s) <= 1.0e300 && fabs(q) <= 1.0e300)) atomicMax(range_flag, 100 - layer);
-        const double mean = s * inv_count;
-        double var = q * inv_count - mean * mean;
-        if (var < 0.0) var = 0.0;
-        const float peak = (float)(fabs(mean) + 8.0 * sqrt(var));
-        if (peak > 0.f && peak < 3.0e38f && __float_as_int(peak) > __builtin_nontemporal_load(range_flag + 1 + layer))
-            atomicMax(range_flag + 1 + layer, __float_as_int(peak));
-        const float rstd = (float)(1.0 / sqrt(var + (double)eps));
-        const float sc = rstd * gamma[c];
-        ss[n * C + c] = make_float2(sc, beta[c] - (float)mean * sc);
+    if (threadIdx.x == 0) stats_write(s, q, c, inv_count, eps, gamma, beta, ss + n * C + c, range_flag, layer);
+}
+
+__global__ void __launch_bounds__(64) stem_combine_kernel(const double* __restrict__ cell_sums, const int* __restrict__ win_cells, int ncw,
+                                                          const float* __restrict__ fparts, int nfp, double inv_count, float eps,
+                                                          const float* __restrict__ gamma, const float* __restrict__ beta,
+                                                          float2* __restrict__ ss, int* __restrict__ range_flag) {
+    const int c = blockIdx.x % 32, n = blockIdx.x / 32;
+    double s = 0.0, q = 0.0;
+    for (int k = threadIdx.x; k < ncw; k += 64) {
+        const double* v = cell_sums + ((long long)win_cells[(long long)n * ncw + k] * 32 + c) * 2;
+        s += v[0];
+        q += v[1];
     }
+    for (int i = threadIdx.x; i < nfp; i += 64) {
+        const float2 v = *reinterpret_cast<const float2*>(fparts + (((long long)n * nfp + i) * 32 + c) * 2);
+        s += v.x;
+        q += v.y;
+    }
+    for (int o = 32; o > 0; o >>= 1) {
+        s += __shfl_down(s, o, 64);
+        q += __shfl_down(q, o, 64);
+    }
+    if (threadIdx.x == 0) stats_write(s, q, c, inv_count, eps, gamma, beta, ss + n * 32 + c, range_flag, 0);
+}
+
+__global__ void __launch_bounds__(64) stem_capture_kernel(const float2* __restrict__ ss, const int* __restrict__ idx, float2* __restrict__ out) {
+    if (threadIdx.x < 32) out[(long long)idx[blockIdx.x] * 32 + threadIdx.x] = ss[blockIdx.x * 32 + threadIdx.x];
 }
 
 template <class P, class PO = P>
diff --git a/delivr_cfos_amd/csrc/unet16_stem.h b/delivr_cfos_amd/csrc/unet16_stem.h
--- a/delivr_cfos_amd/csrc/unet16_stem.h
+++ b/delivr_cfos_amd/csrc/unet16_stem.h
@@ -119,7 +119,7 @@
                                                         const uint4* __restrict__ wpk, const float* __restrict__ bias,
                                                         uint4* __restrict__ out, float* __restrict__ partials,
                                                         const float2* __restrict__ ss, int D, int H, int W, int tilesY,
-                                                        int tilesX) {
+                                                        int tilesX, int Zv) {
     __shared__ unsigned tile[2][SM_NT];
     __shared__ float red[4 * 64];
     const int n = blockIdx.z;
@@ -134,9 +134,10 @@
         const int i = threadIdx.x + 256 * k;
         const int xh = i % SM_HX, yh = (i / SM_HX) % SM_HY, zh = i / (SM_HX * SM_HY);
         int gy = y0 + yh - 1, gx = x0 + xh - 1;
-        const bool ok = i < SM_NT && (unsigned)gy < (unsigned)H && (unsigned)gx < (unsigned)W;
+        bool ok = i < SM_NT && (unsigned)gy < (unsigned)H && (unsigned)gx < (unsigned)W;
         if (flip_dim == 3) gy = H - 1 - gy;
         if (flip_dim == 4) gx = W - 1 - gx;
+        if (MODE == 3) ok = i < SM_NT && (unsigned)(wy + gy) < (unsigned)Yp && (unsigned)(wx + gx) < (unsigned)Xp;
         soff[k] = ok ? (wy + gy) * Xp + (wx + gx) : -1;
         szh[k] = zh - 1;
     }
@@ -146,8 +147,9 @@
 #pragma unroll
         for (int k = 0; k < SM_NS; ++k) {
             int gz = zbase + zc * SM_TZ + szh[k];
-            const bool ok = soff[k] >= 0 && (unsigned)gz < (unsigned)D;
+            bool ok = soff[k] >= 0 && (unsigned)gz < (unsigned)D;
             if (flip_dim == 2) gz = D - 1 - gz;
+            if (MODE == 3) ok = soff[k] >= 0 && (unsigned)(wz + gz) < (unsigned)Zv;
             sv[k] = ok ? (unsigned)vol[(long long)(wz + gz) * plane + soff[k]] : 0u;
         }
     };
@@ -221,7 +223,7 @@
                     val[r + 1] = m.y;
                 }
             }
-            if (MODE != 1 && ok) {
+            if (MODE != 1 && MODE != 3 && ok) {
                 const long long o = ((long long)oz * H + oy) * W + ox;
 #pragma unroll
                 for (int g = 0; g < 4; ++g) {
@@ -255,4 +257,140 @@
     }
 }
 
-}
+__global__ void __launch_bounds__(64) stem_cell_reduce_kernel(const float* __restrict__ partials, int nblk, double* __restrict__ sums) {
+    const long long cell = blockIdx.x;
+    double s = 0.0;
+    for (int b = 0; b < nblk; ++b) s += (double)partials[(cell * nblk + b) * 64 + threadIdx.x];
+    sums[cell * 64 + threadIdx.x] = s;
+}
+
+constexpr int SF_SEGS_PER_WAVE = 4;
+constexpr int SF_YSEG = 30;
+inline int stem_face_segments(int D, int H, int W) {
+    return 2 * H * ((W + 31) / 32) + 2 * (D - 2) * ((W + 31) / 32) + 2 * (D - 2) * ((H - 2 + SF_YSEG - 1) / SF_YSEG);
+}
+inline int stem_face_blocks(int D, int H, int W) { return (stem_face_segments(D, H, W) + 4 * SF_SEGS_PER_WAVE - 1) / (4 * SF_SEGS_PER_WAVE); }
+
+template <class P>
+__global__ void __launch_bounds__(256) stem_face_kernel(const uint16_t* __restrict__ vol, int Zv, int Yp, int Xp,
+                                                        const int* __restrict__ starts, int flip_dim,
+                                                        const uint4* __restrict__ wpk, float* __restrict__ partials, int D, int H,
+                                                        int W) {
+    const int n = blockIdx.y;
+    const int lane = threadIdx.x & 63, wave = threadIdx.x >> 6;
+    const int h = lane >> 5, col = lane & 31;
+    const int wz = starts[3 * n], wy = starts[3 * n + 1], wx = starts[3 * n + 2];
+    const long long plane = (long long)Yp * Xp;
+    uint4 a[4];
+#pragma unroll
+    for (int s = 0; s < 4; ++s) a[s] = AS_FRAG(wpk[s * 64 + lane]);
+    int toff[16], tbit[16];
+    const int fz = flip_dim == 2 ? -1 : 1, fy = flip_dim == 3 ? -1 : 1, fx = flip_dim == 4 ? -1 : 1;
+#pragma unroll
+    for (int i = 0; i < 16; ++i) {
+        const int tp = 8 * (i >> 2) + 4 * h + (i & 3);
+        const int tt = tp < 27 ? tp : 13;
+        const int oz = (tt / 9 - 1) * fz, oy = ((tt / 3) % 3 - 1) * fy, ox = (tt % 3 - 1) * fx;
+        toff[i] = (oz * Yp + oy) * Xp + ox;
+        tbit[i] = tp < 27 ? (oz + 1) | ((oy + 4) << 8) | ((ox + 7) << 16) : -1;
+    }
+    float ds[16], dq[16];
+#pragma unroll
+    for (int r = 0; r < 16; ++r) ds[r] = dq[r] = 0.f;
+    const int sx = (W + 31) / 32, sy = (H - 2 + SF_YSEG - 1) / SF_YSEG;
+    const int nA = 2 * H * sx, nB = 2 * (D - 2) * sx, nC = 2 * (D - 2) * sy;
+    const f32x16 zero = {};
+#pragma unroll 1
+    for (int j = blockIdx.x * 4 + wave; j < nA + nB + nC; j += gridDim.x * 4) {
+        unsigned bg[16], bz[16];
+        if (j < nA + nB) {
+            int z, y;
+            if (j < nA) {
+                const int r = j % (H * sx);
+                z = j / (H * sx) ? D - 1 : 0;
+                y = r / sx;
+            } else {
+                const int k = j - nA, r = k % ((D - 2) * sx);
+                y = k / ((D - 2) * sx) ? H - 1 : 0;
+                z = 1 + r / sx;
+            }
+            const int x = (j % sx) * 32 + col;
+            unsigned win = 0, hld = 0;
+#pragma unroll
+            for (int o = -1; o <= 1; ++o) {
+                win |= ((unsigned)(z + o) < (unsigned)D ? 1u : 0u) << (o + 1);
+                win |= ((unsigned)(y + o) < (unsigned)H ? 1u : 0u) << (o + 4);
+                win |= ((unsigned)(x + o) < (unsigned)W ? 1u : 0u) << (o + 7);
+                hld |= ((unsigned)(wz + z + o) < (unsigned)Zv ? 1u : 0u) << (o + 1);
+                hld |= ((unsigned)(wy + y + o) < (unsigned)Yp ? 1u : 0u) << (o + 4);
+                hld |= ((unsigned)(wx + x + o) < (unsigned)Xp ? 1u : 0u) << (o + 7);
+            }
+            if (x >= W) win = hld = 0;
+            const uint16_t* ctr = vol + ((long long)(wz + z) * plane + (long long)(wy + y) * Xp + (wx + x));
+#pragma unroll
+            for (int i = 0; i < 16; ++i) {
+                const int tb = tbit[i];
+                const unsigned m = tb < 0 ? 0u : (1u << (tb & 255)) | (1u << ((tb >> 8) & 255)) | (1u << (tb >> 16));
+                unsigned v = 0;
+                if ((hld & m) == m && tb >= 0) v = ctr[toff[i]];
+                bg[i] = P::pack2((float)(v & 255u), (float)(v >> 8));
+                bz[i] = (win & m) == m && tb >= 0 ? bg[i] : 0u;
+            }
+        } else {
+            const int k = j - nA - nB, r = k % ((D - 2) * sy);
+            const int x = k / ((D - 2) * sy) ? W - 1 : 0;
+            const int z = 1 + r / sy;
+            const int y = (r % sy) * SF_YSEG + col;
+            const bool on = col >= 1 && col <= SF_YSEG && y < H - 1;
+            unsigned nb[3][3];
+            bool cin[3];
+#pragma unroll
+            for (int c3 = 0; c3 < 3; ++c3) cin[c3] = (unsigned)(x + fx * (c3 - 1)) < (unsigned)W;
+#pragma unroll
+            for (int a3 = 0; a3 < 3; ++a3)
+#pragma unroll
+                for (int c3 = 0; c3 < 3; ++c3) {
+                    const int gz = wz + z + fz * (a3 - 1), gx = wx + x + fx * (c3 - 1);
+                    unsigned v = 0;
+                    if (y < H && (unsigned)gz < (unsigned)Zv && (unsigned)gx < (unsigned)Xp) v = vol[(long long)gz * plane + (long long)(wy + y) * Xp + gx];
+                    nb[a3][c3] = P::pack2((float)(v & 255u), (float)(v >> 8));
+                }
+#pragma unroll
+            for (int i = 0; i < 16; ++i) {
+                const int t0 = 8 * (i >> 2) + (i & 3) < 27 ? 8 * (i >> 2) + (i & 3) : 13;
+                const int t1 = 8 * (i >> 2) + 4 + (i & 3) < 27 ? 8 * (i >> 2) + 4 + (i & 3) : 13;
+                const unsigned mine = h ? nb[t1 / 9][t1 % 3] : nb[t0 / 9][t0 % 3];
+                const int oy = (h ? (t1 / 3) % 3 : (t0 / 3) % 3) - 1;
+                const unsigned v = (unsigned)__shfl((int)mine, lane + fy * oy, 64);
+                bg[i] = on ? v : 0u;
+                bz[i] = on && (h ? cin[t1 % 3] : cin[t0 % 3]) ? v : 0u;
+            }
+        }
+        f32x16 g = P::mfma(a[0], AS_FRAG(make_uint4(bg[0], bg[1], bg[2], bg[3])), zero, 0, 0, 0);
+        g = P::mfma(a[1], AS_FRAG(make_uint4(bg[4], bg[5], bg[6], bg[7])), g, 0, 0, 0);
+        g = P::mfma(a[2], AS_FRAG(make_uint4(bg[8], bg[9], bg[10], bg[11])), g, 0, 0, 0);
+        g = P::mfma(a[3], AS_FRAG(make_uint4(bg[12], bg[13], bg[14], bg[15])), g, 0, 0, 0);
+        f32x16 zp = P::mfma(a[0], AS_FRAG(make_uint4(bz[0], bz[1], bz[2], bz[3])), zero, 0, 0, 0);
+        zp = P::mfma(a[1], AS_FRAG(make_uint4(bz[4], bz[5], bz[6], bz[7])), zp, 0, 0, 0);
+        zp = P::mfma(a[2], AS_FRAG(make_uint4(bz[8], bz[9], bz[10], bz[11])), zp, 0, 0, 0);
+        zp = P::mfma(a[3], AS_FRAG(make_uint4(bz[12], bz[13], bz[14], bz[15])), zp, 0, 0, 0);
+#pragma unroll
+        for (int r = 0; r < 16; ++r) {
+            const float df = zp[r] - g[r];
+            ds[r] += df;
+            dq[r] = fmaf(df, zp[r] + g[r], dq[r]);
+        }
+    }
+    float* row = partials + (((long long)n * gridDim.x + blockIdx.x) * 4 + wave) * 64;
+#pragma unroll
+    for (int r = 0; r < 16; ++r) {
+        const float sa = dlv_half_sum32(ds[r]), sb = dlv_half_sum32(dq[r]);
+        if (col == 31) {
+            const int co = (r & 3) + 8 * (r >> 2) + 4 * h;
+            row[2 * co] = sa;
+            row[2 * co + 1] = sb;
+        }
+    }
+}
+
+}
diff --git a/delivr_cfos_amd/csrc/unet_bf16.hip b/delivr_cfos_amd/csrc/unet_bf16.hip
--- a/delivr_cfos_amd/csrc/unet_bf16.hip
+++ b/delivr_cfos_amd/csrc/unet_bf16.hip
@@ -320,6 +320,23 @@
         if ((size_t)B * nblk * 64 > pfloats) return dlv_fail(ctx, DLV_ESTATE, "partials buffer too small (stem)");
         const DlvConvLayer& L = ctx->conv[0];
         const bool stem_mfma = plan_stem_mfma(ctx->sw, vol != nullptr);
+        const bool stem_shared = stem_mfma && ctx->stem.cell_sums != nullptr;
+        if (stem_shared) {
+            const uint4* wst = reinterpret_cast<const uint4*>(wpack<P>(L));
+            const DlvLabel lf = dlv_label_stem_faces(B, d, h, w);
+            DlvProf pf(ctx, lf.name, lf.flops, lf.bytes);
+            const int fblk = stem_face_blocks(d, h, w), nfp = fblk * 4;
+            if ((size_t)B * nfp * 64 > pfloats) return dlv_fail(ctx, DLV_ESTATE, "partials buffer too small (stem faces)");
+            hipLaunchKernelGGL((stem_face_kernel<P>), dim3(fblk, B), dim3(256), 0, ctx->stream, vol, ctx->stem.Zv, Yp, Xp, starts_dev,
+                               flip_dim, wst, net.partials, d, h, w);
+            DLV_LAUNCH_CHECK(ctx, "stem_face_kernel");
+            const float eps = 1e-5f * P::STEM_SCALE * P::STEM_SCALE * exp2f(-2.f * (float)L.shift);
+            hipLaunchKernelGGL(stem_combine_kernel, dim3(B * 32), dim3(64), 0, ctx->stream, ctx->stem.cell_sums, ctx->stem.win_cells,
+                               ctx->stem.ncw, (const float*)net.partials, nfp, 1.0 / (double)dm[0].vox(), eps, L.gamma, L.beta, net.ss_of(0),
+                               ctx->range_flag);
+            DLV_LAUNCH_CHECK(ctx, "stem_combine_kernel");
+            pf.end();
+        }
         const DlvLabel lb = dlv_label_stem(stem_mfma, B, d, h, w);
         DlvProf pr(ctx, lb.name, lb.flops, lb.bytes);
         if (stem_mfma) {
@@ -328,12 +345,21 @@
             nblk = grid.x;
             if ((size_t)B * nblk * 64 > pfloats) return dlv_fail(ctx, DLV_ESTATE, "partials buffer too small (stem)");
             const uint4* wst = reinterpret_cast<const uint4*>(wpack<P>(L));
-            hipLaunchKernelGGL((stem_mfma_kernel<P, 1>), grid, dim3(256), 0, ctx->stream, vol, Yp, Xp, starts_dev, flip_dim, wst,
-                               L.bias16, buf(0, A), net.partials, (const float2*)nullptr, d, h, w, tY, tX);
-            DLV_LAUNCH_CHECK(ctx, "stem_mfma_kernel<1>");
-            DLV_TRY(net.stats(nblk, 0, dm[0]));
+            if (!stem_shared) {
+                hipLaunchKernelGGL((stem_mfma_kernel<P, 1>), grid, dim3(256), 0, ctx->stream, vol, Yp, Xp, starts_dev, flip_dim, wst,
+                                   L.bias16, buf(0, A), net.partials, (const float2*)nullptr, d, h, w, tY, tX, 0);
+                DLV_LAUNCH_CHECK(ctx, "stem_mfma_kernel<1>");
+                DLV_TRY(net.stats(nblk, 0, dm[0]));
+            }
+            if (ctx->stem.capture) {
+                hipLaunchKernelGGL(stem_capture_kernel, dim3(B), dim3(64), 0, ctx->stream, (const float2*)net.ss_of(0), ctx->stem.capture_idx,
+                                   ctx->stem.capture);
+                DLV_LAUNCH_CHECK(ctx, "stem_capture_kernel");
+                pr.end();
+                return DLV_OK;
+            }
             hipLaunchKernelGGL((stem_mfma_kernel<P, 2>), grid, dim3(256), 0, ctx->stream, vol, Yp, Xp, starts_dev, flip_dim, wst,
-                               L.bias16, buf(0, A), net.partials, (const float2*)net.ss_of(0), d, h, w, tY, tX);
+                               L.bias16, buf(0, A), net.partials, (const float2*)net.ss_of(0), d, h, w, tY, tX, 0);
             two_pass_stem = true;
         } else if (vol)
             hipLaunchKernelGGL((stem_conv_kernel<P, true>), grid, dim3(256), 0, ctx->stream, nullptr, vol, Yp, Xp, starts_dev,
@@ -541,15 +567,15 @@
         const uint16_t* vol = reinterpret_cast<const uint16_t*>(a.vol);
         if (kind == 2)
             hipLaunchKernelGGL((stem_mfma_kernel<P, 0>), grid, dim3(256), 0, ctx->stream, vol, H, W, starts, a.flip_dim, wst,
-                               L.bias16, o, net.partials, (const float2*)nullptr, D, H, W, tY, tX);
+                               L.bias16, o, net.partials, (const float2*)nullptr, D, H, W, tY, tX, 0);
         else
             hipLaunchKernelGGL((stem_mfma_kernel<P, 1>), grid, dim3(256), 0, ctx->stream, vol, H, W, starts, a.flip_dim, wst,
-                               L.bias16, o, net.partials, (const float2*)nullptr, D, H, W, tY, tX);
+                               L.bias16, o, net.partials, (const float2*)nullptr, D, H, W, tY, tX, 0);
         DLV_LAUNCH_CHECK(ctx, "debug stem_mfma_kernel");
         DLV_TRY(net.stats((int)grid.x, 0, d));
         if (kind == 0) {
             hipLaunchKernelGGL((stem_mfma_kernel<P, 2>), grid, dim3(256), 0, ctx->stream, vol, H, W, starts, a.flip_dim, wst,
-                               L.bias16, o, net.partials, (const float2*)net.ss_of(0), D, H, W, tY, tX);
+                               L.bias16, o, net.partials, (const float2*)net.ss_of(0), D, H, W, tY, tX, 0);
             DLV_LAUNCH_CHECK(ctx, "debug stem_mfma_kernel<2>");
             final_written = true;
         }
@@ -580,6 +606,40 @@
     return DLV_OK;
 }
 
+}
+
+static int stem_cell_blocks(const int cell[3]) { return dlv_cdiv(cell[0], SM_TZ * SM_ZC) * dlv_cdiv(cell[1], SM_TY) * dlv_cdiv(cell[2], SM_TX); }
+static int stem_cell_chunk(int ncells, const int cell[3]) {
+    const long long per_cell = (long long)stem_cell_blocks(cell) * 64 * sizeof(float);
+    return (int)std::max<long long>(1, std::min<long long>(std::min<long long>(ncells, 32768), (16ll << 20) / per_cell));
+}
+size_t dlv_stem_cell_scratch_floats(int ncells, const int cell[3]) { return (size_t)stem_cell_chunk(ncells, cell) * stem_cell_blocks(cell) * 64; }
+
+int dlv_stem_cell_stats(dlv_ctx* ctx, const uint16_t* vol, int Zv, int Yp, int Xp, const int* origins_dev, int ncells, const int cell[3],
+                        int flip_dim, int fmt16, float* scratch, size_t scratch_floats, double* sums_dev) {
+    const int D = cell[0], H = cell[1], W = cell[2];
+    const int tY = dlv_cdiv(H, SM_TY), tX = dlv_cdiv(W, SM_TX), nblk = stem_cell_blocks(cell);
+    const int chunk = stem_cell_chunk(ncells, cell);
+    if ((size_t)chunk * nblk * 64 > scratch_floats) return dlv_fail(ctx, DLV_ESTATE, "scratch too small (stem cell sums)");
+    const DlvConvLayer& L = ctx->conv[0];
+    DlvProf pr(ctx, "stem_cell_stats_u16", 2.0 * 27 * 32 * (double)D * H * W * ncells, 2.0 * (double)D * H * W * ncells);
+    for (int c0 = 0; c0 < ncells; c0 += chunk) {
+        const int nc = std::min(chunk, ncells - c0);
+        const dim3 grid(nblk, 1, nc);
+        if (fmt16 != 0)
+            hipLaunchKernelGGL((stem_mfma_kernel<PF16, 3>), grid, dim3(256), 0, ctx->stream, vol, Yp, Xp, origins_dev + 3 * (size_t)c0, flip_dim,
+                               reinterpret_cast<const uint4*>(wpack<PF16>(L)), L.bias16, (uint4*)nullptr, scratch, (const float2*)nullptr, D, H, W,
+                               tY, tX, Zv);
+        else
+            hipLaunchKernelGGL((stem_mfma_kernel<PBf16, 3>), grid, dim3(256), 0, ctx->stream, vol, Yp, Xp, origins_dev + 3 * (size_t)c0, flip_dim,
+                               reinterpret_cast<const uint4*>(wpack<PBf16>(L)), L.bias16, (uint4*)nullptr, scratch, (const float2*)nullptr, D, H, W,
+                               tY, tX, Zv);
+        DLV_LAUNCH_CHECK(ctx, "stem_mfma_kernel<3>");
+        hipLaunchKernelGGL(stem_cell_reduce_kernel, dim3(nc), dim3(64), 0, ctx->stream, (const float*)scratch, nblk, sums_dev + (size_t)c0 * 64);
+        DLV_LAUNCH_CHECK(ctx, "stem_cell_reduce_kernel");
+    }
+    pr.end();
+    return DLV_OK;
 }
 
 int dlv_pack_weights_bf16(dlv_ctx* ctx) {
diff --git a/delivr_cfos_amd/engine.py b/delivr_cfos_amd/engine.py
--- a/delivr_cfos_amd/engine.py
+++ b/delivr_cfos_amd/engine.py
@@ -135,14 +135,18 @@
     return eng
 
 
-def layer_plan(window, switches=None, precision="fp16", batch=1, features=(32, 32, 64, 128, 256, 32)):
+def layer_plan(window, switches=None, precision="fp16", batch=1, features=(32, 32, 64, 128, 256, 32), volume=None, overlap=0.5):
     lib = _lib.load()
     sw = dict(switches or {})
     names = (C.c_char_p * max(1, len(sw)))(*[k.encode() for k in sw])
     values = (C.c_int * max(1, len(sw)))(*[int(v) for v in sw.values()])
     out = _lib.LayerPlan()
-    rc = lib.dlv_diag_plan((C.c_int * 6)(*features), names, values, len(sw), {"bf16_all": 0, "fp16": 1, "bf16": 2}[precision], int(batch),
-                           *(int(v) for v in window), C.byref(out))
+    fmt16 = {"bf16_all": 0, "fp16": 1, "bf16": 2}[precision]
+    if volume is None:
+        rc = lib.dlv_diag_plan((C.c_int * 6)(*features), names, values, len(sw), fmt16, int(batch), *(int(v) for v in window), C.byref(out))
+    else:
+        rc = lib.dlv_diag_plan_sw((C.c_int * 6)(*features), names, values, len(sw), fmt16, int(batch), (C.c_int * 3)(*(int(v) for v in window)),
+                                  (C.c_int * 3)(*(int(v) for v in volume)), float(overlap), C.byref(out))
     if rc != 0:
         raise DelivrHipError(rc, f"dlv_diag_plan: window {tuple(window)}, switches {sw}")
 
@@ -154,6 +158,7 @@
     return {"conv": [fields(c, _lib.PLAN_CONV_KERNELS) for c in out.conv],
             "deconv": [fields(c, _lib.PLAN_DECONV_KERNELS) for c in out.deconv],
             "pool": [{name: getattr(p, name) for name, _ in p._fields_} for p in out.pool],
+            "stem_stats_pass": out.stem_stats_pass,
             "labels": [(out.labels[i].value.decode(), out.flops[i], out.bytes[i]) for i in range(out.n_labels)]}
 
 
@@ -452,6 +457,16 @@
         self._leave()
         return {"n_windows": st.n_windows, "n_skipped": st.n_skipped, "n_forward_launches": st.n_forward_launches}
 
+    def debug_sw_stem_stats(self, params, vol, n_windows):
+        torch = self.torch
+        out = torch.zeros((int(n_windows), 32, 2), dtype=torch.float32, device=self.device)
+        shared = C.c_int(0)
+        self._enter()
+        self._check(self.lib.dlv_debug_sw_stem_stats(self.ctx, C.byref(params), self._dev(vol, torch.uint16, "vol"),
+                                                     self._dev(out, torch.float32, "out"), C.byref(shared)))
+        self._leave()
+        return out, bool(shared.value)
+
     def finalize(self, acc, cnt, raw, stack_shape, threshold=0.5, erode_iters=30, zblock=0, want_prob=False, out=None):
         torch = self.torch
         Z, Y, X = (int(v) for v in stack_shape)
diff --git a/include/delivr_hip_diag.h b/include/delivr_hip_diag.h
--- a/include/delivr_hip_diag.h
+++ b/include/delivr_hip_diag.h
@@ -77,9 +77,14 @@
     int n_labels;
     char labels[DLV_PLAN_MAX_LABELS][48];
     double flops[DLV_PLAN_MAX_LABELS], bytes[DLV_PLAN_MAX_LABELS];
+    int stem_stats_pass;
 } dlv_layer_plan;
 int dlv_diag_plan(const int features[6], const char* const* names, const int* values, int n, int fmt16, int B, int d, int h, int w,
                   dlv_layer_plan* out);
+int dlv_diag_plan_sw(const int features[6], const char* const* names, const int* values, int n, int fmt16, int B, const int roi[3],
+                     const int volume[3], float overlap, dlv_layer_plan* out);
+
+int dlv_debug_sw_stem_stats(dlv_ctx* ctx, const dlv_sw_params* p, const unsigned short* vol_dev, float* ss_dev, int* shared_out);
 
 #ifdef __cplusplus
 }
```

Result: no change. 825.0 million voxels/s, median of 6 (+0.7%).
